# adobe-research/DiffusionHandles

Hardware: AMD Instinct MI355X
Metric: guided-denoise steps/sec at 512x512 (SD2-depth) (higher is better)
Workload: dtype f16; 1 GPU; single 512x512 edit per GPU, SD2-depth (865.9M params, seeded random weights), guided phase: 3 x (fwd + energy + bwd-to-latent) + CFG fwd (B=2) + DDIM step; resolution=512, edits_per_gpu=1, correspondences=24906, parallelism=independent edits, one process per GPU, no collectives

## Files before the change

### diffusionhandles_amd/_lib.py

```python
import ctypes
import os

import torch

_HERE = os.path.dirname(os.path.abspath(__file__))
LIB_PATH = os.environ.get("DIFFHANDLES_LIB") or os.path.join(_HERE, "libdiffhandles_hip.so")
_LIB = None

c_p = ctypes.c_void_p
c_i = ctypes.c_int
c_f = ctypes.c_float
c_d = ctypes.c_double
c_sz = ctypes.c_size_t


class UNetConfig(ctypes.Structure):
    _fields_ = [("in_channels", c_i), ("out_channels", c_i), ("n_levels", c_i),
                ("block_out_channels", c_i * 4), ("layers_per_block", c_i), ("heads", c_i * 4),
                ("cross_attention_dim", c_i), ("norm_groups", c_i), ("sample_size", c_i),
                ("text_len", c_i), ("max_batch", c_i), ("dtype", c_i), ("max_diff_batch", c_i)]


class VAEConfig(ctypes.Structure):
    _fields_ = [("latent_channels", c_i), ("out_channels", c_i), ("block_out_channels", c_i * 4),
# ... 40 lines not shown
    "dh_energy_fwd_bwd_planned": (c_i, [c_p, c_p, c_i, c_i, c_i, c_p, c_sz, c_i, c_p, c_i, c_p, c_i, c_f, c_f, c_f,
                                        c_p, c_p, c_i, c_p, c_sz, c_p]),
    "dh_energy_planned_batch_workspace_bytes": (c_i, [c_i, c_i, c_i, ctypes.POINTER(c_sz)]),
    "dh_energy_fwd_bwd_planned_batch": (c_i, [ctypes.POINTER(EnergyItem), c_i, c_i, c_i, c_i, c_i, c_p, c_sz, c_p]),
    "dh_energy_plan_objects_bytes": (c_i, [c_i, c_i, ctypes.POINTER(c_sz)]),
    "dh_energy_plan_build_objects": (c_i, [c_p, c_p, c_i, c_p, c_i, c_i, c_i, ctypes.POINTER(c_f), ctypes.POINTER(ctypes.c_int32),
                                           c_p, c_sz, c_p]),
    "dh_energy_fwd_bwd_planned_objects": (c_i, [c_p, c_p, c_i, c_i, c_i, c_p, c_sz, c_i, c_p, c_i, c_p, c_i, c_f, c_f, c_f,
                                                c_p, c_p, c_i, c_p, c_sz, c_p]),
    "dh_energy_planned_objects_batch_workspace_bytes": (c_i, [c_i, c_i, c_i, ctypes.POINTER(c_sz)]),
    "dh_energy_fwd_bwd_planned_objects_batch": (c_i, [ctypes.POINTER(EnergyItem), c_i, c_i, c_i, c_i, c_i, c_p, c_sz, c_p]),
    "dh_energy_fwd_bwd_planned_mixed_batch": (c_i, [ctypes.POINTER(EnergyItem), ctypes.POINTER(ctypes.c_uint8), c_i, c_i, c_i, c_i, c_i,
                                              c_p, c_sz, c_p]),
    "dh_unet_create": (c_i, [ctypes.POINTER(UNetConfig), ctypes.POINTER(c_p)]),
    "dh_unet_create_shared": (c_i, [c_p, c_i, c_p, ctypes.POINTER(c_p)]),
    "dh_unet_destroy": (None, [c_p]),
    "dh_unet_num_params": (c_i, [c_p]),
    "dh_unet_param_info": (c_i, [c_p, c_i, ctypes.POINTER(ctypes.c_char_p), ctypes.POINTER(c_i),
                                 ctypes.POINTER(ctypes.c_int64)]),
    "dh_unet_load_param": (c_i, [c_p, c_i, c_p, c_p]),
    "dh_unet_weight_bytes": (c_sz, [c_p]),
    "dh_unet_workspace_bytes": (c_sz, [c_p]),
    "dh_unet_forward": (c_i, [c_p, c_p, c_f, c_p, c_i, c_i, c_p, ctypes.POINTER(c_p), c_p]),
    "dh_unet_backward": (c_i, [c_p, ctypes.POINTER(c_p), c_p, c_p, c_p, c_p]),
    "dh_unet_set_text_key": (c_i, [c_p, ctypes.c_ulonglong]),
    "dh_unet_stats": (c_i, [c_p, ctypes.POINTER(c_d), ctypes.POINTER(c_d), ctypes.POINTER(ctypes.c_int64)]),
    "dh_vae_decoder_create": (c_i, [c_p, ctypes.POINTER(c_p)]),
    "dh_vae_decoder_destroy": (None, [c_p]),
    "dh_vae_decoder_num_params": (c_i, [c_p]),
    "dh_vae_decoder_param_info": (c_i, [c_p, c_i, ctypes.POINTER(ctypes.c_char_p), ctypes.POINTER(c_i),
                                        ctypes.POINTER(ctypes.c_int64)]),
    "dh_vae_decoder_load_param": (c_i, [c_p, c_i, c_p, c_p]),
    "dh_vae_decoder_bytes": (c_sz, [c_p]),
    "dh_vae_decoder_decode": (c_i, [c_p, c_p, c_i, c_p, c_p]),
    "dh_vae_encoder_create": (c_i, [c_p, ctypes.POINTER(c_p)]),
    "dh_vae_encoder_encode": (c_i, [c_p, c_p, c_i, c_p, c_p]),
    "dh_text_encoder_create": (c_i, [c_p, ctypes.POINTER(c_p)]),
    "dh_text_encoder_destroy": (None, [c_p]),
    "dh_text_encoder_num_params": (c_i, [c_p]),
    "dh_text_encoder_param_info": (c_i, [c_p, c_i, ctypes.POINTER(ctypes.c_char_p), ctypes.POINTER(c_i),
                                         ctypes.POINTER(ctypes.c_int64)]),
    "dh_text_encoder_load_param": (c_i, [c_p, c_i, c_p, c_p]),
    "dh_text_encoder_bytes": (c_sz, [c_p]),
    "dh_text_encoder_encode": (c_i, [c_p, c_p, c_i, c_i, c_p, c_p]),
    "dh_gemm_profile_begin": (c_i, []),
    "dh_gemm_profile_end": (c_i, [ctypes.POINTER(c_d), ctypes.POINTER(ctypes.c_int64), ctypes.POINTER(c_d)]),
    "dh_gemm_profile_bytes": (c_i, [ctypes.POINTER(c_d)]),
    "dh_ddim_cfg_step": (c_i, [c_p, c_p, c_p, c_p, c_f, c_f, c_f, c_i, c_p]),
    "dh_latent_update": (c_i, [c_p, c_p, c_p, c_f, c_f, c_i, c_p]),
    "dh_adam_step": (c_i, [c_p, c_p, c_p, c_p, c_f, c_f, c_f, c_f, c_i, c_i, c_p]),
    "dh_mse_fwd_bwd": (c_i, [c_p, c_p, c_i, c_p, c_p, c_p]),
    "dh_latent_update_strided": (c_i, [c_p, c_p, c_p, c_i, c_i, c_f, c_f, c_i, c_p]),
    "dh_pack_sample": (c_i, [c_p, c_p, c_i, c_i, c_p, c_i, c_i, c_i, c_i, c_p]),
    "dh_unet_io_ptr": (c_i, [c_p, c_i, c_i, ctypes.POINTER(c_p), ctypes.POINTER(c_sz)]),
    "dh_mse_cotangent": (c_i, [c_p, c_p, c_i, c_f, c_f, c_p, c_p, c_p, c_p]),
    "dh_adam_step_scaled": (c_i, [c_p, c_p, c_p, c_p, c_p, c_f, c_f, c_f, c_f, c_i, c_i, c_p]),
    "dh_mse_cotangent_batch": (c_i, [c_p, c_p, c_i, c_i, c_f, c_f, c_d, c_p, c_p, c_p, c_p, c_p, c_p]),
    "dh_adam_step_scaled_batch": (c_i, [c_p, c_p, c_p, c_p, c_p, c_p, c_f, c_f, c_f, c_f, c_i, c_i, c_i, c_p]),
    "dh_latent_update_guarded": (c_i, [c_p, c_p, c_p, c_i, c_i, c_f, c_i, c_i, c_p, c_i, c_i, c_p, c_p, c_i, c_i, c_p]),
    "dh_ddim_cfg_step_flagged": (c_i, [c_p, c_p, c_p, c_p, c_f, c_f, c_f, c_i, c_i, c_p, c_i, c_i, c_p]),
}

c_l = ctypes.c_long
DEBUG_SIGNATURES = {
    "dh_dbg_gemm": (c_i, [c_i, c_p, c_l, c_p, c_i, c_i, c_i, c_i, c_i, c_i, c_i, c_i, c_i, c_i, c_i, c_p, c_p, c_i, c_i,
                          c_p, c_l, c_p, c_l, c_i, c_p, c_sz, c_p]),
    "dh_dbg_gemm_groupnorm": (c_i, [c_i, c_p, c_l, c_p, c_i, c_i, c_i, c_i, c_i, c_i, c_i, c_p, c_p, c_p, c_sz, c_i, c_i, c_p, c_p, c_f, c_i,
                                    c_p, c_p, c_p, ctypes.POINTER(c_i), c_p]),
    "dh_dbg_gemm_groupnorm_bwd": (c_i, [c_i, c_p, c_l, c_p, c_i, c_i, c_i, c_i, c_i, c_i, c_i, c_p, c_p, c_sz, c_i, c_i, c_p, c_p, c_p, c_p, c_i,
                                        c_p, c_p, ctypes.POINTER(c_i), c_p]),
    "dh_dbg_gemm_groupnorm_res": (c_i, [c_i, c_p, c_l, c_p, c_i, c_i, c_i, c_i, c_i, c_i, c_i, c_p, c_p, c_l, c_p, c_p, c_sz, c_i, c_i, c_p, c_p,
                                    c_f, c_i, c_p, c_p, c_p, ctypes.POINTER(c_i), c_p]),
    "dh_dbg_gemm_groupnorm_bwd_res": (c_i, [c_i, c_p, c_l, c_p, c_i, c_i, c_i, c_i, c_i, c_i, c_i, c_p, c_l, c_p, c_p, c_sz, c_i, c_i, c_p, c_p, c_p,
                                        c_p, c_i, c_p, c_p, ctypes.POINTER(c_i), c_p]),
    "dh_dbg_concat_groupnorm": (c_i, [c_i, c_p, c_i, c_p, c_i, c_p, c_i, c_i, c_i, c_p, c_p, c_f, c_i, c_p, c_p, c_p, c_p]),
    "dh_dbg_gemm_last_tile": (c_i, [ctypes.POINTER(c_i)]),
    "dh_dbg_unet_concat_ops": (c_i, [ctypes.POINTER(UNetConfig), ctypes.POINTER(c_i), c_i, ctypes.POINTER(c_i)]),
    "dh_dbg_gemm_lnfold": (c_i, [c_i, c_p, c_l, c_p, c_i, c_i, c_i, c_p, c_p, c_p, c_f, c_p, c_l, c_p]),
    "dh_dbg_gemm_glu": (c_i, [c_i, c_i, c_p, c_l, c_p, c_i, c_i, c_i, c_p, c_p, c_p, c_p, c_p, c_p]),
    "dh_dbg_gemm_glub_split": (c_i, [c_i, c_p, c_l, c_p, c_i, c_i, c_i, c_i, c_p, c_l, c_i, c_p, c_p, ctypes.POINTER(c_i), c_p]),
    "dh_dbg_unet_ff_fold": (c_i, [c_p, c_i, ctypes.POINTER(c_i), ctypes.POINTER(c_i), c_p, c_p, c_p]),
    "dh_dbg_gemm_family": (c_i, [c_i]),
    "dh_dbg_gemm_stage": (c_i, [c_i]),
    "dh_dbg_gemm_pp_variant": (c_i, [c_i, c_p]),
    "dh_dbg_gemm_pp_ablate": (c_i, [c_i]),
    "dh_dbg_gemm_pp_persist": (c_i, [c_i]),
    "dh_dbg_gemm_pp_glu": (c_i, [c_i]),
    "dh_dbg_gemm_pp_plan": (c_i, [c_i, c_i, c_i, c_i, c_i, c_i, c_sz, ctypes.POINTER(c_i), ctypes.POINTER(c_i), ctypes.POINTER(c_i)]),
    "dh_dbg_touch_tiled": (c_i, [c_sz, c_p]),
    "dh_dbg_groupnorm": (c_i, [c_i, c_p, c_p, c_p, c_p, c_p, c_p, c_p, c_p, c_i, c_i, c_i, c_i, c_f, c_i, c_i, c_p]),
    "dh_dbg_layernorm": (c_i, [c_i, c_p, c_p, c_p, c_p, c_p, c_p, c_p, c_p, c_i, c_i, c_f, c_p]),
    "dh_dbg_geglu": (c_i, [c_i, c_p, c_p, c_p, c_p, c_i, c_i, c_p]),
    "dh_dbg_attention": (c_i, [c_i, c_p, c_l, c_p, c_p, c_l, c_p, c_l, c_p, c_p, c_p, c_p, c_p, c_p, c_i, c_i, c_i, c_i, c_p]),
    "dh_dbg_attention_bwd_pair": (c_i, [c_i, c_p, c_l, c_p, c_p, c_l, c_p, c_l, c_p, c_p, c_p, c_p, c_p, c_p, c_i, c_i, c_i, c_i, c_p, c_p]),
    "dh_dbg_pool2x2": (c_i, [c_i, c_p, c_p, c_i, c_i, c_i, c_i, c_i, c_p]),
    "dh_dbg_ellipse_offsets": (c_i, [c_i, ctypes.POINTER(ctypes.c_int32), c_i, ctypes.POINTER(c_i)]),
    "dh_dbg_lane_ops": (c_i, [c_p, c_p, c_p, c_p]),
}


def lib():
    global _LIB
    if _LIB is None:
        if not os.path.exists(LIB_PATH):
            raise RuntimeError(
                f"native HIP library not found at {LIB_PATH}; build it with "
                "`python -c 'import __graft_entry__ as g; g.build()'` (there is no CPU fallback)")
        handle = ctypes.CDLL(LIB_PATH)
        missing = []
        for name, (res, args) in list(SIGNATURES.items()) + list(DEBUG_SIGNATURES.items()):
            try:
                fn = getattr(handle, name)
            except AttributeError:
                missing.append(name)
                continue
            fn.restype = res
            fn.argtypes = args
        handle.dh_missing_symbols = missing
        for env, fn in (("DH_GEMM_FAMILY", "dh_dbg_gemm_family"), ("DH_PP_GLU", "dh_dbg_gemm_pp_glu"),
                        ("DH_PP_PERSIST", "dh_dbg_gemm_pp_persist"), ("DH_GEMM_STAGE", "dh_dbg_gemm_stage")):
            if os.environ.get(env) and fn not in missing:
                getattr(handle, fn)(int(os.environ[env]))
        _LIB = handle
    return _LIB


def check(rc, what=""):
    if rc != 0:
        raise RuntimeError(f"{what} failed ({rc}): {lib().dh_last_error().decode()}")


def require_gpu(t=None):
    if not torch.cuda.is_available():
        raise RuntimeError("diffusionhandles_amd needs a HIP device (MI355X); there is no CPU fallback")
    if t is not None and not t.is_cuda:
        raise RuntimeError("expected a device tensor")


def ptr(t):
    return c_p(t.data_ptr()) if t is not None else c_p(0)


def stream_ptr():
    return c_p(torch.cuda.current_stream().cuda_stream)


DTYPE_CODE = {torch.float16: 0, torch.bfloat16: 1, torch.float32: 2}
CODE_DTYPE = {v: k for k, v in DTYPE_CODE.items()}
```

### diffusionhandles_amd/csrc/attention.hip

```cpp
#include "unet_kernels.h"

namespace dh {

typedef _Float16 v8h __attribute__((ext_vector_type(8)));
typedef __bf16 v8b __attribute__((ext_vector_type(8)));
typedef float v16f __attribute__((ext_vector_type(16)));
typedef short v4s __attribute__((ext_vector_type(4)));

template <class T> struct Mma;
template <> struct Mma<f16> {
  static __device__ __forceinline__ v16f run(uint4 a, uint4 b, v16f c) {
    return __builtin_amdgcn_mfma_f32_32x32x16_f16(__builtin_bit_cast(v8h, a), __builtin_bit_cast(v8h, b), c, 0, 0, 0);
  }
};
template <> struct Mma<bf16> {
  static __device__ __forceinline__ v16f run(uint4 a, uint4 b, v16f c) {
    return __builtin_amdgcn_mfma_f32_32x32x16_bf16(__builtin_bit_cast(v8b, a), __builtin_bit_cast(v8b, b), c, 0, 0, 0);
  }
};

constexpr int HD = 64;
constexpr int TLD = 72;
constexpr int TILE = 64 * TLD;
constexpr float LOG2E = 1.4426950408889634f;
constexpr float LN2 = 0.6931471805599453f;
constexpr float SCALE = 0.125f;
constexpr float CEXP = SCALE * LOG2E;

__device__ __forceinline__ v16f zero16() {
  v16f z;
#pragma unroll
  for (int i = 0; i < 16; ++i) z[i] = 0.f;
  return z;
}
__device__ __forceinline__ float fast_exp2(float x) { return __builtin_amdgcn_exp2f(x); }
#ifndef DH_ATTN_ABL
#define DH_ATTN_ABL 0
#endif

template <class T>
__device__ __forceinline__ void load_row_frags(const T* base, long ld, long row, bool ok, int col0, int hi, uint4 (&f)[4]) {
#pragma unroll
  for (int kk = 0; kk < 4; ++kk)
    f[kk] = ok ? *reinterpret_cast<const uint4*>(base + row * ld + col0 + 16 * kk + 8 * hi) : make_uint4(0, 0, 0, 0);
}

typedef unsigned u4v __attribute__((ext_vector_type(4)));
template <int GT> struct TileRegs { u4v v[(512 + GT - 1) / GT]; };
template <class T, int GT>
__device__ __forceinline__ void fetch_tile(const T* base , long ld, long row0, long rows_total,
                                           TileRegs<GT>& t, int tid) {
#pragma unroll
  for (int j = 0; j < (512 + GT - 1) / GT; ++j) {
    int idx = tid + j * GT;
    idx = idx < 512 ? idx : 511;
    long r = row0 + (idx >> 3);
    r = r < rows_total ? r : rows_total - 1;
    const T* ptr = base + r * ld + (idx & 7) * 8;
    asm volatile("global_load_dwordx4 %0, %1, off" : "=&v"(t.v[j]) : "v"(ptr) : "memory");
  }
}
__device__ __forceinline__ void frags_ready(uint4 (&f)[4]) {
#pragma unroll
  for (int kk = 0; kk < 4; ++kk) asm volatile("" : "+v"(f[kk].x), "+v"(f[kk].y), "+v"(f[kk].z), "+v"(f[kk].w));
}
template <int GT>
__device__ __forceinline__ void tile_wait(TileRegs<GT>& a, TileRegs<GT>& b) {
  asm volatile("s_waitcnt vmcnt(0)" ::: "memory");
#pragma unroll
  for (int j = 0; j < (512 + GT - 1) / GT; ++j) { asm volatile("" : "+v"(a.v[j])); asm volatile("" : "+v"(b.v[j])); }
}
template <int GT>
__device__ __forceinline__ void commit_tile(const TileRegs<GT>& t, unsigned short* rm, int tid) {
#pragma unroll
  for (int j = 0; j < (512 + GT - 1) / GT; ++j) {
    const int idx = tid + j * GT;
    if (512 % GT == 0 || idx < 512) *reinterpret_cast<u4v*>(&rm[(idx >> 3) * TLD + (idx & 7) * 8]) = t.v[j];
  }
}

template <class T>
__device__ __forceinline__ v16f tile_times_frags(const unsigned short* tile, int rowbase, int ln, int hi, const uint4 (&f)[4]) {
  v16f acc = zero16();
#pragma unroll
  for (int kk = 0; kk < 4; ++kk) {
    const uint4 a = *reinterpret_cast<const uint4*>(&tile[(rowbase + ln) * TLD + 16 * kk + 8 * hi]);
    acc = Mma<T>::run(a, f[kk], acc);
  }
  return acc;
}

__device__ __forceinline__ uint4 tr_frag(const unsigned short* tptr, int cbase, int r0) {
  typedef __attribute__((address_space(3))) v4s* lp;
  const unsigned short* a = tptr + r0 * TLD + cbase;
  const v4s lo = __builtin_amdgcn_ds_read_tr16_b64_v4i16((lp)(a));
  const v4s up = __builtin_amdgcn_ds_read_tr16_b64_v4i16((lp)(a + 8 * TLD));
  const uint2 l2 = __builtin_bit_cast(uint2, lo), u2 = __builtin_bit_cast(uint2, up);
  return make_uint4(l2.x, l2.y, u2.x, u2.y);
}

constexpr int DTILE = 64 * 64;
__device__ uint4 g_attn_zero_page[8];
#ifdef DH_ATTN_STAMP
__device__ unsigned long long g_attn_ts_dkv[16];
#define DKV_STAMP(i) do { if (blockIdx.x == 0 && blockIdx.y == 0 && blockIdx.z == 0 && threadIdx.x == 0) g_attn_ts_dkv[i] = __builtin_amdgcn_s_memtime(); } while (0)
__device__ unsigned long long g_attn_ts[8];
#define ATTN_STAMP(i) do { if (blockIdx.x == 0 && blockIdx.y == 0 && blockIdx.z == 0 && threadIdx.x == 0) g_attn_ts[i] = __builtin_amdgcn_s_memtime(); } while (0)
#else
#define ATTN_STAMP(i) do { } while (0)
#define DKV_STAMP(i) do { } while (0)
#endif
#ifdef DH_ATTN_STAMP_DQ
#undef DKV_STAMP
#define DKV_STAMP(i) do { } while (0)
#define DQ_STAMP(i) do { if (blockIdx.x == 0 && blockIdx.y == 0 && blockIdx.z == 0 && threadIdx.x == 0) g_attn_ts_dkv[i] = __builtin_amdgcn_s_memtime(); } while (0)
#else
#define DQ_STAMP(i) do { } while (0)
#endif
__device__ __forceinline__ int dswz(int r) {
  const int y = r >> 1;
  return ((y & 1) << 2) | (y & 2) | ((y >> 2) & 1);
}
__device__ __forceinline__ void attn_dma16(const void* gsrc, unsigned lds_dst) {
  unsigned keep;
  asm volatile("s_mov_b32 %0, m0\n\ts_mov_b32 m0, %2\n\ts_nop 0\n\tglobal_load_lds_dwordx4 %1, off\n\ts_mov_b32 m0, %0"
               : "=&s"(keep) : "v"(gsrc), "s"(lds_dst) : "memory");
}
template <int QW> struct DmaPieces { unsigned voff[(16 + QW - 1) / QW]; };
template <int QW>
__device__ __forceinline__ void dma_pieces_init(DmaPieces<QW>& d, int wave_u, int lane, long ld_a, long ld_b) {
  const int d_row = lane >> 3;
  const int d_c0 = (lane & 7) ^ ((((lane >> 4) >> 1) & 1) << 1 | ((lane >> 4) & 1) << 2);
#pragma unroll
  for (int j = 0; j < (16 + QW - 1) / QW; ++j) {
    const int p = wave_u + j * QW, pp = p & 7;
    d.voff[j] = (unsigned)(((long)(8 * pp + d_row) * (p < 8 ? ld_a : ld_b) + ((d_c0 ^ (pp & 1)) << 3)) * 2);
  }
}
__device__ __forceinline__ void attn_dma16_s(const void* base, unsigned voff, unsigned lds) {
  const unsigned long long b64 = (unsigned long long)base;
  const unsigned long long sbase = (unsigned long long)(unsigned)__builtin_amdgcn_readfirstlane((int)(unsigned)b64) |
                                   ((unsigned long long)(unsigned)__builtin_amdgcn_readfirstlane((int)(unsigned)(b64 >> 32)) << 32);
  const unsigned lds_dst = (unsigned)__builtin_amdgcn_readfirstlane((int)lds);
  unsigned keep;
  asm volatile("s_mov_b32 %0, m0\n\ts_mov_b32 m0, %3\n\ts_nop 0\n\tglobal_load_lds_dwordx4 %2, %1\n\ts_mov_b32 m0, %0"
               : "=&s"(keep) : "s"(sbase), "v"(voff), "s"(lds_dst) : "memory");
}
template <int QW>
__device__ __forceinline__ void dma_tile_full(const DmaPieces<QW>& d, int wave_u, const void* base_a, const void* base_b,
                                              unsigned lds_tile) {
#pragma unroll
  for (int j = 0; j < (16 + QW - 1) / QW; ++j) {
    const int p = wave_u + j * QW;
    if (p < 16) attn_dma16_s(p < 8 ? base_a : base_b, d.voff[j], lds_tile + (unsigned)(p * 1024));
  }
}
template <class T>
__device__ __forceinline__ v16f dtile_times_frags(const unsigned short* tile, int rowbase, int ln, int xk, const uint4 (&f)[4]) {
  v16f acc = zero16();
#pragma unroll
  for (int kk = 0; kk < 4; ++kk) {
    const uint4 a = *reinterpret_cast<const uint4*>(&tile[(rowbase + ln) * 64 + ((xk ^ (2 * kk)) << 3)]);
    acc = Mma<T>::run(a, f[kk], acc);
  }
  return acc;
}
__device__ __forceinline__ uint4 dtr_frag(const unsigned short* trow, int lo_c, int up_c, int within, int dt, int r0) {
  typedef __attribute__((address_space(3))) v4s* lp;
  const unsigned short* a = trow + r0 * 64 + within;
  const v4s lo = __builtin_amdgcn_ds_read_tr16_b64_v4i16((lp)(a + ((lo_c ^ (4 * dt)) << 3)));
  const v4s up = __builtin_amdgcn_ds_read_tr16_b64_v4i16((lp)(a + 8 * 64 + ((up_c ^ (4 * dt)) << 3)));
  const uint2 l2 = __builtin_bit_cast(uint2, lo), u2 = __builtin_bit_cast(uint2, up);
  return make_uint4(l2.x, l2.y, u2.x, u2.y);
}

template <class T>
__device__ __forceinline__ uint4 pack8(const v16f& p, int s);
template <>
__device__ __forceinline__ uint4 pack8<f16>(const v16f& p, int s) {
  uint4 o;
  o.x = __builtin_bit_cast(unsigned, __builtin_amdgcn_cvt_pkrtz(p[8 * s + 0], p[8 * s + 1]));
  o.y = __builtin_bit_cast(unsigned, __builtin_amdgcn_cvt_pkrtz(p[8 * s + 2], p[8 * s + 3]));
  o.z = __builtin_bit_cast(unsigned, __builtin_amdgcn_cvt_pkrtz(p[8 * s + 4], p[8 * s + 5]));
  o.w = __builtin_bit_cast(unsigned, __builtin_amdgcn_cvt_pkrtz(p[8 * s + 6], p[8 * s + 7]));
  return o;
}
template <>
__device__ __forceinline__ uint4 pack8<bf16>(const v16f& p, int s) {
  bf16 o[8];
#pragma unroll
  for (int j = 0; j < 8; ++j) o[j] = (bf16)p[8 * s + j];
  return *reinterpret_cast<uint4*>(o);
}

template <class T>
__device__ __forceinline__ void store_rows_t(T* base, long ld, long row, int col0, int hi, const v16f (&acc)[2], float mul) {
#pragma unroll
  for (int dt = 0; dt < 2; ++dt) {
    uint2 w[4];
#pragma unroll
    for (int g = 0; g < 4; ++g) {
      T o[4];
#pragma unroll
      for (int i = 0; i < 4; ++i) o[i] = from_f32<T>(acc[dt][4 * g + i] * mul);
      w[g] = *reinterpret_cast<uint2*>(o);
    }
    const uint4 ca = half_exchange(w[0], w[1]), cb = half_exchange(w[2], w[3]);
    T* out = base + row * ld + col0 + dt * 32 + 8 * hi;
    *reinterpret_cast<uint4*>(out) = ca;
    *reinterpret_cast<uint4*>(out + 16) = cb;
  }
}

__device__ __forceinline__ int acc_row(int r, int hi) { return (r & 3) + 8 * (r >> 2) + 4 * hi; }

__device__ __forceinline__ void lds_barrier() {
  asm volatile("s_waitcnt lgkmcnt(0)" ::: "memory");
  __builtin_amdgcn_s_barrier();
  asm volatile("" ::: "memory");
}

template <class T, int KS, int QW, bool DB>
__global__ void __launch_bounds__(64 * QW * KS) k_attn_fwd(const T* q, long ldq, const T* k, const T* v, long ldk, T* o, long ldo,
                                                       float* lse, int H, int Nq, int Nk, int causal) {
  ATTN_STAMP(0);
  constexpr int NBUF = DB ? 2 : 1;
  constexpr int TSZ = DB ? DTILE : TILE;
  __shared__ __attribute__((aligned(1024))) unsigned short smem[KS * NBUF * 2 * TSZ];
  constexpr int GT = 64 * QW;
  const int ks = threadIdx.x / GT, tid = threadIdx.x - ks * GT;
  const int lane = tid & 63, wave = tid >> 6, ln = lane & 31, hi = lane >> 5, t16 = lane & 15;
  const int h = blockIdx.y, b = blockIdx.z;
  unsigned short* sK0 = smem + ks * NBUF * 2 * TSZ;
  const long qrow = (long)blockIdx.x * (32 * QW) + wave * 32 + ln;
  const bool qok = qrow < Nq;
  uint4 qf[4];
  load_row_frags<T>(q + (long)b * Nq * ldq, ldq, qrow, qok, h * HD, hi, qf);
  frags_ready(qf);
  v16f oacc[2] = {zero16(), zero16()};
  float m_run = -INFINITY, l_run = 0.f;
  const T* kp = k + (long)b * Nk * ldk + h * HD;
  const T* vp = v + (long)b * Nk * ldk + h * HD;
  const int vt_off = (4 * hi + (t16 >> 2)) * TLD + 16 * ((lane >> 4) & 1) + 4 * (t16 & 3);
  const int tiles = (Nk + 63) >> 6, tps = (tiles + KS - 1) / KS;
  const int t_begin = ks * tps, t_end = min(t_begin + tps, tiles);
  TileRegs<GT> rk, rv;
  const unsigned lds_grp = DB ? (unsigned)(size_t)((__attribute__((address_space(3))) unsigned char*)smem) + ks * NBUF * 2 * TSZ * 2 : 0u;
  const int d_row = lane >> 3;
  const int d_c0 = (lane & 7) ^ ((((lane >> 4) >> 1) & 1) << 1 | ((lane >> 4) & 1) << 2);
  const T* d_zero = reinterpret_cast<const T*>(g_attn_zero_page) + (lane & 7) * 8;
  const int wave_u = __builtin_amdgcn_readfirstlane(wave);
  DmaPieces<QW> dpc;
  if (DB) dma_pieces_init<QW>(dpc, wave_u, lane, ldk, ldk);
  auto dma_tile = [&](int key0, int buf) {
    if (key0 + 64 <= Nk) {
      dma_tile_full<QW>(dpc, wave_u, kp + (long)key0 * ldk, vp + (long)key0 * ldk, lds_grp + (unsigned)(buf * 2 * TSZ * 2));
      return;
    }
#pragma unroll
    for (int j = 0; j < (16 + QW - 1) / QW; ++j) {
      const int p = wave_u + j * QW;
      if (p < 16) {
        const int pp = p & 7;
        const long r = (long)key0 + 8 * pp + d_row;
        const T* src = (p < 8 ? kp : vp) + r * ldk + ((d_c0 ^ (pp & 1)) << 3);
        attn_dma16(r < Nk ? src : d_zero, __builtin_amdgcn_readfirstlane(lds_grp + (unsigned)(buf * 2 * TSZ * 2 + p * 1024)));
      }
    }
  };
  if (t_begin < t_end) {
    if (DB) {
      dma_tile(t_begin * 64, 0);
    } else {
      fetch_tile<T, GT>(kp, ldk, t_begin * 64, Nk, rk, tid);
      fetch_tile<T, GT>(vp, ldk, t_begin * 64, Nk, rv, tid);
    }
  }
  const int xk = hi ^ dswz(ln);
  const int d_rl = 4 * hi + (t16 >> 2), d_cl = 2 * ((lane >> 4) & 1) + ((t16 & 3) >> 1);
  const int d_lo = d_cl ^ dswz(d_rl), d_up = d_cl ^ dswz(d_rl + 8), d_within = 4 * (t16 & 1);
  ATTN_STAMP(1);
  for (int it = 0; it < tps; ++it) {
    if (it == 1) ATTN_STAMP(2);
    const int k0 = (t_begin + it) * 64;
    const bool act = t_begin + it < t_end;
    if (DB) {
      asm volatile("s_waitcnt vmcnt(0)" ::: "memory");
      __syncthreads();
    } else {
      lds_barrier();
    }
    if (DB && act && t_begin + it + 1 < t_end) dma_tile(k0 + 64, (it + 1) & 1);
    if (!DB) {
      if (act) {
        tile_wait<GT>(rk, rv);
        commit_tile<GT>(rk, sK0, tid);
        commit_tile<GT>(rv, sK0 + TILE, tid);
// ... 712 lines not shown
```

### diffusionhandles_amd/csrc/debug_api.cpp

```cpp
#include <stdlib.h>

#include "unet_kernels.h"
using namespace dh;

static void* g_dbg_tiled = nullptr;

__global__ void k_dbg_touch(const uint4* p, size_t n16, unsigned* sink) {
  unsigned acc = 0;
  for (size_t i = (size_t)blockIdx.x * blockDim.x + threadIdx.x; i < n16; i += (size_t)gridDim.x * blockDim.x) { const uint4 v = p[i]; acc ^= v.x ^ v.y ^ v.z ^ v.w; }
  if (acc == 0x9e3779b9u && sink) sink[0] = acc;
}
extern "C" int dh_dbg_touch_tiled(size_t bytes, void* stream) {
  DH_REQUIRE(g_dbg_tiled != nullptr, "no tiled weights yet (call dh_dbg_gemm first)");
  hipLaunchKernelGGL(k_dbg_touch, dim3(512), dim3(256), 0, (hipStream_t)stream, (const uint4*)g_dbg_tiled, bytes / 16, (unsigned*)nullptr);
  DH_LAUNCH_CHECK();
  return DH_OK;
}

extern "C" int dh_dbg_gemm(int dtype, const void* A, long lda, const void* W, int M, int N, int K, int mode, int Hin,
                           int Win, int Cin, int Hout, int Wout, int stride, int up, const float* bias,
                           const float* rowvec, int rowvec_ld, int rows_per_batch, const void* R, long ldr, void* C,
                           long ldc, int act_silu, float* partial, size_t partial_elems, void* stream) {
  DH_REQUIRE(A && W && C && K % 64 == 0 && N % 64 == 0, "bad arguments (N, K must be multiples of 64)");
  void*& tiled = g_dbg_tiled;
// ... 32 lines not shown
    cap = need;
  }
  launch_tile_weights(dtype, W, tiled, N, K, (hipStream_t)stream, mode != 0 ? Cin : 0);
  GemmArgs g;
  g.A = A; g.lda = lda; g.W = tiled; g.M = M; g.N = N; g.K = K; g.mode = mode; g.Hin = Hin; g.Win = Win; g.Cin = Cin;
  g.Hout = Hin; g.Wout = Win; g.stride = 1; g.up = 0; g.bias = bias; g.R = R; g.ldr = ldr; g.C = C; g.ldc = N;
  g.partial = partial; g.partial_elems = partial_elems;
  int have = 0;
  g.gn_part = scratch; g.gn_HW = HW; g.gn_G = G; g.gn_done = &have;
  launch_gemm(dtype, g, (hipStream_t)stream);
  launch_groupnorm_fwd(dtype, C, gamma, beta, Y, stats, scratch, M / HW, HW, N, G, eps, silu, (hipStream_t)stream, have);
  if (have_out) *have_out = have;
  DH_LAUNCH_CHECK();
  return DH_OK;
}
extern "C" int dh_dbg_gemm_groupnorm(int dtype, const void* A, long lda, const void* W, int M, int N, int K, int mode, int Hin, int Win,
                                     int Cin, const float* bias, void* C, float* partial, size_t partial_elems, int HW, int G,
                                     const float* gamma, const float* beta, float eps, int silu, void* Y, float* stats, float* scratch,
                                     int* have_out, void* stream) {
  return dh_dbg_gemm_groupnorm_res(dtype, A, lda, W, M, N, K, mode, Hin, Win, Cin, bias, nullptr, N, C, partial, partial_elems, HW, G,
                                   gamma, beta, eps, silu, Y, stats, scratch, have_out, stream);
}
extern "C" int dh_dbg_gemm_groupnorm_bwd_res(int dtype, const void* A, long lda, const void* W, int M, int N, int K, int mode, int Hin,
                                         int Win, int Cin, const void* R, long ldr, void* C, float* partial, size_t partial_elems, int HW, int G, const void* x,
                                         const float* gamma, const float* beta, const float* stats, int silu, void* dx,
                                         float* scratch, int* have_out, void* stream) {
  DH_REQUIRE(A && W && C && x && dx && stats && scratch && gamma && beta && K % 64 == 0 && N % 64 == 0 && HW > 0 && M % HW == 0, "bad arguments");
  static void* tiled = nullptr;
  static size_t cap = 0;
  const size_t need = (size_t)N * K * 2;
  if (need > cap) {
    if (tiled) (void)hipFree(tiled);
    DH_CHECK_HIP(hipMalloc(&tiled, need));
    cap = need;
  }
  launch_tile_weights(dtype, W, tiled, N, K, (hipStream_t)stream, mode != 0 ? Cin : 0);
  GemmArgs g;
  g.A = A; g.lda = lda; g.W = tiled; g.M = M; g.N = N; g.K = K; g.mode = mode; g.Hin = Hin; g.Win = Win; g.Cin = Cin;
  g.Hout = Hin; g.Wout = Win; g.stride = 1; g.up = 0; g.R = R; g.ldr = ldr; g.C = C; g.ldc = N;
  g.partial = partial; g.partial_elems = partial_elems;
  int have = 0;
  g.gnb_x = x; g.gnb_ldx = N; g.gnb_gamma = gamma; g.gnb_beta = beta; g.gnb_stats = stats; g.gnb_silu = silu;
  g.gn_part = scratch; g.gn_HW = HW; g.gn_G = G; g.gn_done = &have;
  launch_gemm(dtype, g, (hipStream_t)stream);
  launch_groupnorm_bwd(dtype, x, C, gamma, beta, stats, dx, scratch, M / HW, HW, N, G, silu, 0, (hipStream_t)stream, have, GnBwdSplit());
  if (have_out) *have_out = have;
  DH_LAUNCH_CHECK();
  return DH_OK;
}
extern "C" int dh_dbg_gemm_groupnorm_bwd(int dtype, const void* A, long lda, const void* W, int M, int N, int K, int mode, int Hin,
                                         int Win, int Cin, void* C, float* partial, size_t partial_elems, int HW, int G, const void* x,
                                         const float* gamma, const float* beta, const float* stats, int silu, void* dx,
                                         float* scratch, int* have_out, void* stream) {
  return dh_dbg_gemm_groupnorm_bwd_res(dtype, A, lda, W, M, N, K, mode, Hin, Win, Cin, nullptr, N, C, partial, partial_elems, HW, G, x,
                                       gamma, beta, stats, silu, dx, scratch, have_out, stream);
}
extern "C" int dh_dbg_concat_groupnorm(int dtype, const void* a, int Ca, const void* b, int Cb, void* out, int B, int HW, int G,
                                       const float* gamma, const float* beta, float eps, int silu, void* Y, float* stats,
                                       float* scratch, void* stream) {
  DH_REQUIRE(a && b && out && Y && stats && scratch && gamma && beta && B > 0 && HW > 0 && G > 0, "bad arguments");
  DH_REQUIRE(Ca % 8 == 0 && Cb % 8 == 0 && (Ca + Cb) % G == 0 && (GN_GB * ((Ca + Cb) / G)) % 8 == 0 && GN_GB * ((Ca + Cb) / G) <= 2048,
             "shape the fused concatenation does not take");
  launch_concat_gn(dtype, a, Ca, b, Cb, out, scratch, B, HW, G, (hipStream_t)stream);
  launch_groupnorm_fwd(dtype, out, gamma, beta, Y, stats, scratch, B, HW, Ca + Cb, G, eps, silu, (hipStream_t)stream, 1);
  DH_LAUNCH_CHECK();
  return DH_OK;
}
extern "C" int dh_dbg_gemm_lnfold(int dtype, const void* A, long lda, const void* W, int M, int N, int K, const float* ln_s,
                                  const float* ln_t, float* ln_stats, float ln_eps, void* C, long ldc, void* stream) {
  DH_REQUIRE(A && W && C && ln_s && ln_t && ln_stats && K % 64 == 0 && N % 64 == 0, "bad arguments (N, K must be multiples of 64)");
  static void* tiled = nullptr;
  static size_t tiled_cap = 0;
  const size_t need = (size_t)N * K * 2;
  if (need > tiled_cap) {
    if (tiled) (void)hipFree(tiled);
    DH_CHECK_HIP(hipMalloc(&tiled, need));
    tiled_cap = need;
  }
  launch_tile_weights(dtype, W, tiled, N, K, (hipStream_t)stream);
  GemmArgs g;
  g.A = A; g.lda = lda; g.W = tiled; g.M = M; g.N = N; g.K = K; g.mode = A_DENSE; g.C = C; g.ldc = ldc;
  g.ln_s = ln_s; g.ln_t = ln_t; g.ln_stats = ln_stats; g.ln_eps = ln_eps;
  launch_gemm(dtype, g, (hipStream_t)stream);
  DH_LAUNCH_CHECK();
  return DH_OK;
}
extern "C" int dh_dbg_gemm_glu(int dtype, int bwd, const void* A, long lda, const void* W, int M, int N, int K, const float* bias,
                               void* C, void* y, const void* x, void* dx, void* stream) {
  DH_REQUIRE(A && W && K % 64 == 0 && N % 128 == 0, "bad arguments (K % 64, N % 128)");
  DH_REQUIRE(bwd ? (x && dx) : (y != nullptr), "missing output");
  static void* tiled = nullptr;
  static size_t tiled_cap = 0;
  const size_t need = (size_t)N * K * 2;
  if (need > tiled_cap) {
    if (tiled) (void)hipFree(tiled);
    DH_CHECK_HIP(hipMalloc(&tiled, need));
    tiled_cap = need;
  }
  launch_tile_weights(dtype, W, tiled, N, K, (hipStream_t)stream);
  GemmArgs g;
  g.A = A; g.lda = lda; g.W = tiled; g.M = M; g.N = N; g.K = K; g.mode = A_DENSE; g.bias = bias;
  if (bwd) { g.glub_x = x; g.glub_dx = dx; }
  else { g.C = C; g.ldc = N; g.glu_y = y; g.glu_ldy = N / 2; }
  launch_gemm(dtype, g, (hipStream_t)stream);
  DH_LAUNCH_CHECK();
  return DH_OK;
}
extern "C" int dh_dbg_gemm_last_tile(int* out);
extern "C" int dh_dbg_gemm_glub_split(int dtype, const void* A, long lda, const void* W, int M, int N, int K, int F, void* C,
                                      long ldc, int accumulate, const void* x, void* dx, int* tile, void* stream) {
  DH_REQUIRE(A && W && C && x && dx && K % 64 == 0 && N % 64 == 0 && F % 64 == 0 && F > 0 && F < N, "bad arguments (K, N, F % 64; 0 < F < N)");
  static void* tiled = nullptr;
  static size_t tiled_cap = 0;
  const int Np = (int)align_up((size_t)N, 128);
  const size_t need = (size_t)Np * K * 2;
  if (need > tiled_cap) {
    if (tiled) (void)hipFree(tiled);
    DH_CHECK_HIP(hipMalloc(&tiled, need));
    tiled_cap = need;
  }
  DH_CHECK_HIP(hipMemsetAsync(tiled, 0, need, (hipStream_t)stream));
  launch_tile_weights(dtype, W, tiled, N, K, (hipStream_t)stream);
  GemmArgs g;
  g.A = A; g.lda = lda; g.W = tiled; g.M = M; g.N = N; g.K = K; g.mode = A_DENSE;
  g.glub_x = x; g.glub_dx = dx; g.glub_f = F;
  g.C = C; g.ldc = ldc;
  if (accumulate) { g.R = C; g.ldr = ldc; }
  launch_gemm(dtype, g, (hipStream_t)stream);
  if (tile) dh_dbg_gemm_last_tile(tile);
  DH_LAUNCH_CHECK();
  return DH_OK;
}
extern "C" int dh_dbg_groupnorm(int dtype, const void* x, const float* gamma, const float* beta, void* y, float* stats,
                                const void* dy, void* dx, float* scratch, int B, int HW, int C, int G, float eps,
                                int silu, int accumulate, void* stream) {
  launch_groupnorm_fwd(dtype, x, gamma, beta, y, stats, scratch, B, HW, C, G, eps, silu, (hipStream_t)stream);
  if (dy && dx)
    launch_groupnorm_bwd(dtype, x, dy, gamma, beta, stats, dx, scratch, B, HW, C, G, silu, accumulate, (hipStream_t)stream);
  DH_LAUNCH_CHECK();
  return DH_OK;
}
extern "C" int dh_dbg_layernorm(int dtype, const void* x, const float* gamma, const float* beta, void* y, float* stats,
                                const void* dy, const void* add, void* dx, int rows, int C, float eps, void* stream) {
  launch_layernorm_fwd(dtype, x, gamma, beta, y, stats, rows, C, eps, (hipStream_t)stream);
  if (dy && dx) launch_layernorm_bwd(dtype, x, dy, gamma, stats, add, dx, rows, C, (hipStream_t)stream);
  DH_LAUNCH_CHECK();
  return DH_OK;
}
extern "C" int dh_dbg_geglu(int dtype, const void* x, void* y, const void* dy, void* dx, int rows, int F, void* stream) {
  launch_geglu_fwd(dtype, x, y, rows, F, (hipStream_t)stream);
  if (dy && dx) launch_geglu_bwd(dtype, x, dy, dx, rows, F, (hipStream_t)stream);
  DH_LAUNCH_CHECK();
  return DH_OK;
}
extern "C" int dh_dbg_attention(int dtype, const void* q, long ldq, const void* k, const void* v, long ldk, void* o,
                                long ldo, float* lse, const void* d_o, float* delta, void* dq, void* dk, void* dv,
                                int B, int H, int Nq, int Nk, void* stream) {
  hipStream_t st = (hipStream_t)stream;
  launch_attention_fwd(dtype, q, ldq, k, v, ldk, o, ldo, lse, B, H, Nq, Nk, st);
  if (d_o) {
    if (dq) launch_attention_bwd_dq(dtype, q, ldq, k, v, ldk, o, ldo, d_o, ldo, lse, delta, dq, ldq, B, H, Nq, Nk, st);
    else launch_attention_delta(dtype, o, ldo, d_o, ldo, delta, B, H, Nq, st);
    if (dk && dv) {
      static float* scratch = nullptr;
      constexpr size_t kScratch = (size_t)16 << 20;
      if (!scratch && hipMalloc((void**)&scratch, kScratch * sizeof(float)) != hipSuccess) scratch = nullptr;
// ... 39 lines not shown
```

### diffusionhandles_amd/csrc/gemm.hip

```cpp
#include <stdlib.h>

#include <vector>

#include <hip/hip_ext.h>

#include "gemm_k.h"

namespace dh {

struct GemmProf {
  bool on = false;
  std::vector<hipEvent_t> ev;
  size_t used = 0;
  double flops = 0;
  double bytes = 0;
  hipEvent_t e0 = nullptr, e1 = nullptr;
};
static GemmProf g_prof;
static int g_buf_stage = 1;
static int g_pp_force = 0;
struct GemmTileReport {
  int bm, bn, kg, stages, mw, splits, pp, gn_epi, reduce_gn;
};
static thread_local GemmTileReport g_last_tile;
#ifdef DH_TUNING
static unsigned long long* g_gemm_ts = nullptr;
#endif
bool gemm_profiling_on() { return g_prof.on; }

constexpr int BK = 64;
#ifdef DH_EXP_SETPRIO
#define DH_PRIO(x) __builtin_amdgcn_s_setprio(x)
#else
#define DH_PRIO(x) do { } while (0)
#endif


template <class T>
__device__ __forceinline__ uint2 epilogue_pack(const GemmK& p, int m, int n, float v0, float v1, float v2, float v3,
                                               bool have_r, uint2 rpre, bool have_b, float4 bpre) {
  float v[4] = {v0, v1, v2, v3};
  if (p.bias) {
    float4 b = bpre;
    if (!have_b) b = *reinterpret_cast<const float4*>(p.bias + n);
    v[0] += b.x; v[1] += b.y; v[2] += b.z; v[3] += b.w;
  }
  if (p.rowvec) {
    const float4 b = *reinterpret_cast<const float4*>(p.rowvec + (size_t)div_small(m, p.inv_rows_per_batch) * p.rowvec_ld + n);
    v[0] += b.x; v[1] += b.y; v[2] += b.z; v[3] += b.w;
  }
  if (p.act_silu) {
#pragma unroll
    for (int i = 0; i < 4; ++i) v[i] = v[i] / (1.f + __expf(-v[i]));
  }
  typedef T T4 __attribute__((ext_vector_type(4)));
  if (p.R) {
    const T* r = reinterpret_cast<const T*>(p.R) + (size_t)m * p.ldr + n;
    uint2 raw = rpre;
    if (!have_r) raw = *reinterpret_cast<const uint2*>(r);
    const T4 rv = __builtin_bit_cast(T4, raw);
#pragma unroll
    for (int i = 0; i < 4; ++i) v[i] += to_f32<T>(rv[i]);
  }
  T4 o;
#pragma unroll
  for (int i = 0; i < 4; ++i) o[i] = from_f32<T>(v[i]);
  return __builtin_bit_cast(uint2, o);
}
template <class T>
__device__ __forceinline__ void epilogue_store(const GemmK& p, int m, int n, float v0, float v1, float v2, float v3,
                                               bool have_r = false, uint2 rpre = make_uint2(0, 0), bool have_b = false,
                                               float4 bpre = make_float4(0.f, 0.f, 0.f, 0.f)) {
  *reinterpret_cast<uint2*>(reinterpret_cast<T*>(p.C) + (size_t)m * p.ldc + n) =
      epilogue_pack<T>(p, m, n, v0, v1, v2, v3, have_r, rpre, have_b, bpre);
}

template <class T>
__device__ __forceinline__ float epilogue_scalar(const GemmK& p, int m, int n, float v) {
  if (p.bias) v += p.bias[n];
  if (p.rowvec) v += p.rowvec[(size_t)div_small(m, p.inv_rows_per_batch) * p.rowvec_ld + n];
  if (p.act_silu) v = v / (1.f + __expf(-v));
  if (p.R) v += to_f32<T>(reinterpret_cast<const T*>(p.R)[(size_t)m * p.ldr + n]);
  return to_f32<T>(from_f32<T>(v));
}

__device__ uint4 g_zero_page[8];

__device__ __forceinline__ void dma16(const void* gsrc, unsigned lds_dst) {
  unsigned keep;
  asm volatile("s_mov_b32 %0, m0\n\ts_mov_b32 m0, %2\n\ts_nop 0\n\tglobal_load_lds_dwordx4 %1, off\n\ts_mov_b32 m0, %0"
               : "=&s"(keep) : "v"(gsrc), "s"(lds_dst) : "memory");
}

__device__ __forceinline__ void dma16_nt(const void* gsrc, unsigned lds_dst) {
  unsigned keep;
  asm volatile("s_mov_b32 %0, m0\n\ts_mov_b32 m0, %2\n\ts_nop 0\n\tglobal_load_lds_dwordx4 %1, off nt\n\ts_mov_b32 m0, %0"
               : "=&s"(keep) : "v"(gsrc), "s"(lds_dst) : "memory");
}

typedef int buf_v4i __attribute__((ext_vector_type(4)));
__device__ __forceinline__ void buf_dma16(unsigned voff, buf_v4i rsrc, unsigned soff, unsigned lds_dst) {
  unsigned tmp;
  soff = __builtin_amdgcn_readfirstlane(soff);
  lds_dst = __builtin_amdgcn_readfirstlane(lds_dst);
  asm volatile("s_mov_b32 m0, %4\n\ts_mov_b32 %0, %3\n\tbuffer_load_dwordx4 %1, %2, %0 offen lds"
               : "=&s"(tmp) : "v"(voff), "s"(rsrc), "s"(soff), "s"(lds_dst) : "memory");
}
// ... 235 lines not shown
      bs_sh = 31u - (unsigned)tap;
      return;
    }
    if (MODE != GM_DENSE) { if (++tap == 9) { tap = 0; c0 += BK; } }
  };
  auto issue = [&](int kt, int stage) {
#pragma unroll
    for (int q = 0; q < NP; ++q) issue_piece(kt, stage, q);
    next_tile();
  };

  v16f acc[TM][TN];
#pragma unroll
  for (int i = 0; i < TM; ++i)
#pragma unroll
    for (int j = 0; j < TN; ++j)
#pragma unroll
      for (int r = 0; r < 16; ++r) acc[i][j][r] = 0.f;

  const int wn_u = __builtin_amdgcn_readfirstlane(wn);
  float ln1[TM], ln2[TM];
#pragma unroll
  for (int i = 0; i < TM; ++i) { ln1[i] = 0.f; ln2[i] = 0.f; }

#pragma unroll
  for (int s = 0; s < ST - 1; ++s)
    if (s < ntiles) issue(s, s);
  DH_STAMP(1);

  constexpr bool PRE = TM * TN <= 8;
  const bool pre_r = PRE && p.R != nullptr && p.pre_r && p.splits == 1 && (WG == 1 || grp == 0) && (KG == 1 || kg == 0) &&
                     (GLU != 2 || !glub_tile_is_glu(n0, p.glub_f));
  constexpr bool PRE_B = PRE && !(MW == 2 && BN == 320) && WNS == 2;
  const bool pre_b = PRE_B && p.bias != nullptr && p.pre_r && p.splits == 1;
  float4 bpre[PRE_B ? TN : 1][4];
  if (pre_b) {
#pragma unroll
    for (int j = 0; j < TN; ++j)
#pragma unroll
      for (int g = 0; g < 4; ++g) {
        const int n = n0 + wn * CPW + j * 32 + 8 * g + 4 * hi;
        bpre[PRE_B ? j : 0][g] = n < p.N ? *reinterpret_cast<const float4*>(p.bias + n) : make_float4(0.f, 0.f, 0.f, 0.f);
      }
  }
  constexpr bool PRE_LN = LNF && PRE && !(MW == 2 && BM == 256);
  float4 lsp[PRE_LN ? TN : 1][4], ltp[PRE_LN ? TN : 1][4];
  if (PRE_LN) {
#pragma unroll
    for (int j = 0; j < TN; ++j)
#pragma unroll
      for (int g = 0; g < 4; ++g) {
        const int n = n0 + wn * CPW + j * 32 + 8 * g + 4 * hi;
        lsp[PRE_LN ? j : 0][g] = n < p.N ? *reinterpret_cast<const float4*>(p.ln_s + n) : make_float4(0.f, 0.f, 0.f, 0.f);
        ltp[PRE_LN ? j : 0][g] = n < p.N ? *reinterpret_cast<const float4*>(p.ln_t + n) : make_float4(0.f, 0.f, 0.f, 0.f);
      }
  }
  constexpr bool GNB = gn_epi_bwd_tile(BM, BN, WG, GLU, LNF);
  static_assert(!GNB || (PRE && WNS == 2), "the backward form carries the GroupNorm input tile in the residual's prefetch registers");
  const bool gnb = GNB && p.gn_epi == 2 && p.splits == 1;
  const bool pre_x = gnb && (KG == 1 || kg == 0);
  float4 gnb_col = make_float4(0.f, 0.f, 0.f, 0.f);
  if (GNB && pre_x && tid < BN) {
    const int n = n0 + tid, grp_n = (int)(((float)n + 0.5f) / (float)p.gn_cpg);
    const float2 st2 = *reinterpret_cast<const float2*>(p.gnb_stats + 2 * ((m0 / p.gn_HW) * p.gn_G + grp_n));
    gnb_col = make_float4(p.gnb_gamma[n], p.gnb_beta[n], st2.x, st2.y);
  }
  uint2 rpre[TM][TN][4];
  if (pre_r || pre_x) {
    const T* rsrc = reinterpret_cast<const T*>(pre_x ? p.gnb_x : p.R);
    const long rld = pre_x ? p.gnb_ldx : p.ldr;
#pragma unroll
    for (int i = 0; i < TM; ++i) {
      const int m = m0 + wm * RPW + i * 32 + ln;
#pragma unroll
      for (int j = 0; j < TN; ++j)
#pragma unroll
        for (int g = 0; g < 4; ++g) {
          const int n = n0 + wn * CPW + j * 32 + 8 * g + 4 * hi;
          rpre[i][j][g] = (m < p.M && n < p.N) ? *reinterpret_cast<const uint2*>(rsrc + (size_t)m * rld + n) : make_uint2(0, 0);
        }
    }
  }

  constexpr int KK = BK / 16 / WG;
  const int kk0 = grp * KK;
  unsigned fa_off[BK / 16], fb_off[BK / 16];
#pragma unroll
  for (int kk = 0; kk < BK / 16; ++kk) {
    const unsigned pc = (unsigned)(((2 * kk + hi) ^ ((ln >> 1) & 7)) << 4);
    fa_off[kk] = (unsigned)((wm * RPW + ln) * 128) + pc;
    fb_off[kk] = (unsigned)(BM * 128 + (wn * CPW + ln) * 128) + pc;
  }
  int stg = 0;
  DH_STAMP(2);
  for (int kt = 0; kt < loop_tiles; ++kt) {
    DH_STAMP_T(kt, 0);
    if (ntiles - 1 - kt >= ST - 2) wait_vmcnt<NP * (ST - 2)>(); else wait_vmcnt<0>();
    __builtin_amdgcn_s_barrier();
    DH_STAMP_T(kt, 1);
    if (kt == 0) DH_STAMP(3);
    if (KG > 1 && kt >= ntiles) continue;
    const bool more = ABL != 2 && kt + ST - 1 < ntiles;
    const int cur = __builtin_amdgcn_readfirstlane(stg);
    const int nkt = kt + ST - 1, nstage = cur == 0 ? ST - 1 : cur - 1;
    stg = cur + 1 == ST ? 0 : cur + 1;
    if (ABL == 1) { if (more) issue(nkt, nstage); continue; }
    const unsigned char* st_base = smem + cur * STAGE;
    uint4 fw[2][TN], fx[2][TM];
    auto load_frags = [&](int kk, int buf) {
      const unsigned char* pb = st_base + fb_off[kk];
      const unsigned char* pa = st_base + fa_off[kk];
#pragma unroll
      for (int j = 0; j < TN; ++j) fw[buf][j] = *reinterpret_cast<const uint4*>(pb + j * (32 * 128));
#pragma unroll
      for (int i = 0; i < TM; ++i) fx[buf][i] = *reinterpret_cast<const uint4*>(pa + i * (32 * 128));
    };
    load_frags(kk0, 0);
#pragma unroll
    for (int kk = 0; kk < KK; ++kk) {
      if (kk + 1 < KK) load_frags(kk0 + kk + 1, (kk + 1) & 1);
      DH_PRIO(1);
#pragma unroll
      for (int i = 0; i < TM; ++i)
#pragma unroll
        for (int j = 0; j < TN; ++j) acc[i][j] = Mfma<T>::run(fw[kk & 1][j], fx[kk & 1][i], acc[i][j]);
      DH_PRIO(0);
      if (LNF && (kk & 1) == wn_u LNF_ABL(1)) {
#pragma unroll
        for (int i = 0; i < TM; ++i) frag_sums<T>(fx[kk & 1][i], ln1[i], ln2[i]);
      }
      if (more) {
        constexpr int EK = ST == 2 ? 2 : KK;
        if (kk < EK) {
#pragma unroll
          for (int q = kk * NP / EK; q < (kk + 1) * NP / EK; ++q) issue_piece(nkt, nstage, q);
        }
      }
    }
    if (more) next_tile();
    DH_STAMP_T(kt, 2);
  }
  DH_STAMP(4);

  if (LNF LNF_ABL(2)) {
    float* xb = reinterpret_cast<float*>(smem_all);
    const int wid = tid >> 6;
    __syncthreads();
#pragma unroll
    for (int i = 0; i < TM; ++i) { xb[(wid * 2 * TM + 2 * i) * 64 + lane] = ln1[i]; xb[(wid * 2 * TM + 2 * i + 1) * 64 + lane] = ln2[i]; }
    __syncthreads();
#pragma unroll
    for (int i = 0; i < TM; ++i) {
      ln1[i] += xb[((wid ^ 1) * 2 * TM + 2 * i) * 64 + lane];
      ln2[i] += xb[((wid ^ 1) * 2 * TM + 2 * i + 1) * 64 + lane];
    }
  }

  if (WG > 1 || KG > 1) {
    constexpr int NG = WG * KG;
    constexpr int SLOT = (TM * TN * 16 + (LNF ? 2 * TM : 0)) * 64;
    static_assert((NG - 1) * 4 * SLOT * 4 <= KG * ST * STAGE, "merge buffer does not fit the stage rings");
    const int g = WG > 1 ? grp : kg;
    float* cb = reinterpret_cast<float*>(smem_all);
    __syncthreads();
    if (g > 0) {
      float* slot = cb + ((g - 1) * 4 + wave) * SLOT + lane;
#pragma unroll
      for (int i = 0; i < TM; ++i)
#pragma unroll
        for (int j = 0; j < TN; ++j)
#pragma unroll
          for (int r = 0; r < 16; ++r) slot[((i * TN + j) * 16 + r) * 64] = acc[i][j][r];
      if (LNF) {
#pragma unroll
        for (int i = 0; i < TM; ++i) { slot[(TM * TN * 16 + 2 * i) * 64] = ln1[i]; slot[(TM * TN * 16 + 2 * i + 1) * 64] = ln2[i]; }
      }
    }
    __syncthreads();
    if (g > 0) return;
#pragma unroll
    for (int og = 1; og < NG; ++og) {
      const float* slot = cb + ((og - 1) * 4 + wave) * SLOT + lane;
#pragma unroll
      for (int i = 0; i < TM; ++i)
#pragma unroll
        for (int j = 0; j < TN; ++j)
#pragma unroll
          for (int r = 0; r < 16; ++r) acc[i][j][r] += slot[((i * TN + j) * 16 + r) * 64];
      if (LNF) {
#pragma unroll
        for (int i = 0; i < TM; ++i) { ln1[i] += slot[(TM * TN * 16 + 2 * i) * 64]; ln2[i] += slot[(TM * TN * 16 + 2 * i + 1) * 64]; }
      }
    }
  }

  if (LNF LNF_ABL(4)) {
    const float inv_k = 1.f / (float)p.K;
#pragma unroll
    for (int i = 0; i < TM; ++i) {
      const float a = xor32_sum(ln1[i]), q = xor32_sum(ln2[i]);
      const float mean = a * inv_k;
      float var = q * inv_k - mean * mean;
      var = var > 0.f ? var : 0.f;
      const float rstd = rsqrtf(var + p.ln_eps);
      const int m = m0 + wm * RPW + i * 32 + ln;
      if (blockIdx.y == 0 && wn == 0 && hi == 0 && m < p.M) { p.ln_stats[2 * (size_t)m] = mean; p.ln_stats[2 * (size_t)m + 1] = rstd; }
#pragma unroll
      for (int j = 0; j < TN; ++j)
#pragma unroll
        for (int g = 0; g < 4; ++g) {
          const int n = n0 + wn * CPW + j * 32 + 8 * g + 4 * hi;
          if (n >= p.N) continue;
          float4 sv, tv;
          if (PRE_LN) { sv = lsp[PRE_LN ? j : 0][g]; tv = ltp[PRE_LN ? j : 0][g]; }
          else { sv = *reinterpret_cast<const float4*>(p.ln_s + n); tv = *reinterpret_cast<const float4*>(p.ln_t + n); }
          acc[i][j][4 * g] = rstd * (acc[i][j][4 * g] - mean * sv.x) + tv.x;
          acc[i][j][4 * g + 1] = rstd * (acc[i][j][4 * g + 1] - mean * sv.y) + tv.y;
          acc[i][j][4 * g + 2] = rstd * (acc[i][j][4 * g + 2] - mean * sv.z) + tv.z;
          acc[i][j][4 * g + 3] = rstd * (acc[i][j][4 * g + 3] - mean * sv.w) + tv.w;
        }
    }
  }


  if constexpr (GLU == 1) {
    typedef T T4 __attribute__((ext_vector_type(4)));
    const bool hb = p.bias != nullptr;
    T* Y = reinterpret_cast<T*>(p.glu_y);
#pragma unroll
    for (int i = 0; i < TM; ++i) {
      const int m = m0 + wm * RPW + i * 32 + ln;
      if (m >= p.M) continue;
#pragma unroll
      for (int j = 0; j < TN; ++j) {
        const int nb = n0 + wn * CPW + j * 32;
        if (nb >= p.N) continue;
        uint2 w[4];
        float pv[4][4];
#pragma unroll
        for (int g = 0; g < 4; ++g) {
          float v0 = acc[i][j][4 * g], v1 = acc[i][j][4 * g + 1], v2 = acc[i][j][4 * g + 2], v3 = acc[i][j][4 * g + 3];
          if (hb) {
            float4 b = bpre[PRE_B ? j : 0][g];
            if (!pre_b) b = *reinterpret_cast<const float4*>(p.bias + nb + 8 * g + 4 * hi);
            v0 += b.x; v1 += b.y; v2 += b.z; v3 += b.w;
          }
          T4 o;
          o[0] = from_f32<T>(v0); o[1] = from_f32<T>(v1); o[2] = from_f32<T>(v2); o[3] = from_f32<T>(v3);
          w[g] = __builtin_bit_cast(uint2, o);
#pragma unroll
          for (int c = 0; c < 4; ++c) pv[g][c] = to_f32<T>(o[c]);
        }
        if (p.C) {
          T* out = reinterpret_cast<T*>(p.C) + (size_t)m * p.ldc + nb + 8 * hi;
          *reinterpret_cast<uint4*>(out) = half_exchange(w[0], w[1]);
          *reinterpret_cast<uint4*>(out + 16) = half_exchange(w[2], w[3]);
        }
        uint2 y[2];
#pragma unroll
        for (int q = 0; q < 2; ++q) {
          T4 o;
#pragma unroll
          for (int c = 0; c < 4; ++c) o[c] = from_f32<T>(pv[q][c] * gelu_f(pv[q + 2][c]));
          y[q] = __builtin_bit_cast(uint2, o);
        }
        *reinterpret_cast<uint4*>(Y + (size_t)m * p.glu_ldy + (nb >> 1) + 8 * hi) = half_exchange(y[0], y[1]);
      }
    }
    return;
  }
  if (GLU == 2 && glub_tile_is_glu(n0, p.glub_f)) {
    typedef T T4 __attribute__((ext_vector_type(4)));
    const T* X = reinterpret_cast<const T*>(p.glub_x);
    T* DX = reinterpret_cast<T*>(p.glub_dx);
    const size_t ldx = 2 * (size_t)p.glub_f;
    uint4 Hc[TM][TN][2], Gc[TM][TN][2];
#pragma unroll
    for (int i = 0; i < TM; ++i) {
      const int m = m0 + wm * RPW + i * 32 + ln;
      const int mc = m < p.M ? m : p.M - 1;
#pragma unroll
      for (int j = 0; j < TN; ++j) {
        int nb = n0 + wn * CPW + j * 32;
        if (nb >= p.glub_f) nb = 0;
#pragma unroll
        for (int q = 0; q < 2; ++q) {
          const T* src = X + (size_t)mc * ldx + 2 * nb + 32 * q + 8 * hi;
          Hc[i][j][q] = *reinterpret_cast<const uint4*>(src);
          Gc[i][j][q] = *reinterpret_cast<const uint4*>(src + 16);
        }
      }
    }
#pragma unroll
    for (int i = 0; i < TM; ++i) {
      const int m = m0 + wm * RPW + i * 32 + ln;
      if (m >= p.M) continue;
#pragma unroll
      for (int j = 0; j < TN; ++j) {
        const int nb = n0 + wn * CPW + j * 32;
        if (nb >= p.glub_f) continue;
#pragma unroll
        for (int q = 0; q < 2; ++q) {
          const uint4 hc = Hc[i][j][q], gc = Gc[i][j][q];
          const uint4 hx = half_exchange(make_uint2(hc.x, hc.y), make_uint2(hc.z, hc.w));
          const uint4 gx = half_exchange(make_uint2(gc.x, gc.y), make_uint2(gc.z, gc.w));
          uint2 dh[2], dg[2];
// ... 381 lines not shown
      const uint4 rawx = *reinterpret_cast<const uint4*>(reinterpret_cast<const T*>(p.gnb_x) + (size_t)m * p.gnb_ldx + n);
      const T* xv = reinterpret_cast<const T*>(&rawx);
#pragma unroll
      for (int i = 0; i < 8; ++i) {
        o[i] = from_f32<T>(v[i]);
        const float xh = (to_f32<T>(xv[i]) - mu[i]) * rs[i];
        float d = to_f32<T>(o[i]);
        if (p.gnb_silu) d *= silu_grad(xh * gm[i] + bt[i]);
        d *= gm[i];
        av[i] += d; qv[i] += d * xh;
      }
    }
    *reinterpret_cast<uint4*>(reinterpret_cast<T*>(p.C) + (size_t)m * p.ldc + n) = *reinterpret_cast<uint4*>(o);
  };
  auto acc = [&](const float* f) {
#pragma unroll
    for (int i = 0; i < 8; ++i) { const float d = f[i] - pv[i]; av[i] += d; qv[i] += d * d; }
  };
  float f[8];
  if (BWD) {
    if (live)
      for (int r = r0 + rr; r < r1; r += RP) row(r, f);
  } else {
    const bool first = live && r0 + rr < r1;
    if (first) row(r0 + rr, f);
    if (first && rr == 0) {
#pragma unroll
      for (int i = 0; i < 8; ++i)
        if (ch * 8 + i == gi[i] * cpg) sm_piv[gi[i]] = f[i];
    }
    __syncthreads();
#pragma unroll
    for (int i = 0; i < 8; ++i) pv[i] = g0 + gi[i] < G ? sm_piv[gi[i]] : 0.f;
    if (first) {
      acc(f);
      for (int r = r0 + rr + RP; r < r1; r += RP) { row(r, f); acc(f); }
    }
  }
  if (live) {
#pragma unroll
    for (int i = 0; i < 8; ++i)
#pragma unroll
      for (int gl = 0; gl < GN_GB; ++gl) {
        ga[gl] += gi[i] == gl ? av[i] : 0.f;
        gq[gl] += gi[i] == gl ? qv[i] : 0.f;
      }
  }
#pragma unroll
  for (int gl = 0; gl < GN_GB; ++gl) { ga[gl] = wave_sum(ga[gl]); gq[gl] = wave_sum(gq[gl]); }
  if ((threadIdx.x & 63) == 0) {
#pragma unroll
    for (int gl = 0; gl < GN_GB; ++gl) { sm_red[threadIdx.x >> 6][2 * gl] = ga[gl]; sm_red[threadIdx.x >> 6][2 * gl + 1] = gq[gl]; }
  }
  __syncthreads();
  if ((int)threadIdx.x < GN_GB && g0 + (int)threadIdx.x < G) {
    const int gl = threadIdx.x, g = g0 + gl;
    float sa = 0.f, sq = 0.f;
    for (int w = 0; w < 4; ++w) { sa += sm_red[w][2 * gl]; sq += sm_red[w][2 * gl + 1]; }
    if (BWD) {
      p.gn_part[((size_t)(b * G + g) * S + s) * 2] = sa;
      p.gn_part[((size_t)(b * G + g) * S + s) * 2 + 1] = sq;
    } else {
      const float cnt = (float)(r1 - r0) * (float)cpg;
      float* o = p.gn_part + ((size_t)(b * G + g) * 3) * S + s;
      o[0] = cnt; o[S] = sm_piv[gl] + sa / cnt; o[2 * S] = sq - sa * sa / cnt;
    }
  }
}

#define DH_GEMM_LAUNCH(KERNEL)                                                                              \
  do {                                                                                                      \
    if (g_prof.e0) hipExtLaunchKernelGGL(KERNEL, grid, dim3(TH), 0, st, g_prof.e0, g_prof.e1, 0, k);        \
    else hipLaunchKernelGGL(KERNEL, grid, dim3(TH), 0, st, k);                                              \
  } while (0)
template <class T, int BM, int BN, int ST, int WG, int KG, int MW, bool BUF>
static void launch_tile_b(int gm, bool lnf, dim3 grid, hipStream_t st, const GemmK& k, int glu) {
  constexpr int TH = 256 * WG * KG * MW;
  constexpr bool GLUOK = WG == 1 && KG == 1 && ((BM == 256 && BN == 128 && MW == 2) || (BM == 128 && BN == 128 && MW == 2 && ST == 4) || (BM == 64 && BN == 64));
  if constexpr (GLUOK) {
    if (glu == 1 && lnf) { DH_GEMM_LAUNCH((k_gemm_dma<T, BM, BN, ST, GM_DENSE, 0, WG, KG, MW, true, 1, BUF>)); return; }
    if (glu == 1) { DH_GEMM_LAUNCH((k_gemm_dma<T, BM, BN, ST, GM_DENSE, 0, WG, KG, MW, false, 1, BUF>)); return; }
    if (glu == 2) { DH_GEMM_LAUNCH((k_gemm_dma<T, BM, BN, ST, GM_DENSE, 0, WG, KG, MW, false, 2, BUF>)); return; }
  }
  if (gm == GM_DENSE) {
    if constexpr (WG == 1 && BN != 320 && BN != 160) {
      if (lnf) { DH_GEMM_LAUNCH((k_gemm_dma<T, BM, BN, ST, GM_DENSE, 0, WG, KG, MW, true, 0, BUF>)); return; }
    }
    DH_GEMM_LAUNCH((k_gemm_dma<T, BM, BN, ST, GM_DENSE, 0, WG, KG, MW, false, 0, BUF>));
  } else if (gm == GM_CONV_S1) {
    DH_GEMM_LAUNCH((k_gemm_dma<T, BM, BN, ST, GM_CONV_S1, 0, WG, KG, MW, false, 0, BUF>));
  } else {
    DH_GEMM_LAUNCH((k_gemm_dma<T, BM, BN, ST, GM_GENERIC, 0, WG, KG, MW>));
  }
}
template <class T, int BM, int BN, int ST, int WG, int KG, int MW>
static void launch_tile(int gm, bool lnf, dim3 grid, hipStream_t st, const GemmK& k, int glu = 0) {
  g_last_tile.bm = BM; g_last_tile.bn = BN; g_last_tile.kg = KG; g_last_tile.stages = ST; g_last_tile.mw = MW;
  if (k.pp_a_bytes != 0 && gm != GM_GENERIC) launch_tile_b<T, BM, BN, ST, WG, KG, MW, true>(gm, lnf, grid, st, k, glu);
  else launch_tile_b<T, BM, BN, ST, WG, KG, MW, false>(gm, lnf, grid, st, k, glu);
}
#undef DH_GEMM_LAUNCH

#ifdef DH_TUNING
#define DH_KNOB(name, env, dflt) static const int name = getenv(env) ? atoi(getenv(env)) : (dflt)
#else
#define DH_KNOB(name, env, dflt) constexpr int name = (dflt)
#endif

template <class T>
static void gemm_dispatch(GemmK k, size_t partial_elems, hipStream_t st, int* gn_done, int* lnb_done, int dtype) {
  DH_KNOB(kSplitTiles, "DH_SPLITK_TILES", 200);
  DH_KNOB(kSplitMinK, "DH_SPLITK_MINKT", 32);
  DH_KNOB(kSplitTarget, "DH_SPLITK_TARGET", 256);
  DH_KNOB(kBigTiles, "DH_BIG_TILES", 128);
  DH_KNOB(kNarrowTiles, "DH_NARROW_TILES", 40);
  DH_KNOB(kN320, "DH_GEMM_N320", 224);
  DH_KNOB(kMwBlocks, "DH_GEMM_MW", 64);
  DH_KNOB(kKg2MinKt, "DH_KG2_MINKT", 4);
  DH_KNOB(kManyBlocks, "DH_GEMM_MANY", 512);
  DH_KNOB(kMw128, "DH_GEMM_MW128", 1);
  DH_KNOB(kTwoPerCu, "DH_GEMM_TWO_PER_CU", 1);
#ifdef DH_TUNING
  DH_KNOB(kWnt, "DH_W_NT", 0);
#endif
  const bool lnf = k.ln_s != nullptr;
  g_last_tile = GemmTileReport{};
  int BM = 128, BN = (k.N % 128 == 0) ? 128 : 64;
  const int ktiles = k.K / BK;
  PpPlan pp;
  const bool use_pp = gemm_pp_plan(k, partial_elems, g_pp_force, &pp);
  if (BN == 128 && ktiles >= 16 && cdiv(k.M, 128) * cdiv(k.N, 128) <= kNarrowTiles) BN = 64;
  if (k.M <= 64 || (cdiv(k.M, 128) * cdiv(k.N, BN) < kBigTiles && ktiles < kSplitMinK)) { BM = 64; BN = 64; }
  const bool n320 = kN320 > 0 && k.N % 320 == 0 && k.N <= 960 && !lnf && BM == 128 && BN == 64 && cdiv(k.M, 128) >= kN320;
  if (n320) BN = 320;
  DH_KNOB(kMwShortK, "DH_GEMM_MW_SHORTK", 128);
  const long tiles256 = (long)cdiv(k.M, 256) * cdiv(k.N, 128);
  const bool mw2 = kMwBlocks > 0 && k.N % 128 == 0 && tiles256 >= kMwBlocks &&
                   !(k.M <= 256 && k.M > 128 && cdiv(k.N, 128) < 128) && (tiles256 >= kMwShortK || ktiles >= kSplitMinK);
  if (mw2) { BM = 256; BN = 128; }
  const int glu = k.glu_y ? 1 : (k.glub_x ? 2 : 0);
  if (glu && !(BM == 64 && BN == 64)) { BM = mw2 ? 256 : 128; BN = 128; }
  if (glu == 2 && !glub_split_ok(BN, k.glub_f)) { BM = 64; BN = 64; }
  DH_KNOB(kT160, "DH_GEMM_T160", 224);
  const long tiles160 = (long)cdiv(k.M, 128) * (k.N / 160);
  const bool t160 = kT160 > 0 && k.N % 160 == 0 && !lnf && !glu && !n320 && BM != 64 && tiles160 >= kT160 && tiles160 <= 256;
  if (t160) { BM = 128; BN = 160; }
  if (use_pp) { BM = pp.bm; BN = pp.bn; }
  const int tm = cdiv(k.M, BM), tn = cdiv(k.N, BN), tiles = tm * tn;
  int splits = 1;
  if (use_pp) splits = pp.splits;
  else if (k.partial && !lnf && !glu && tiles < kSplitTiles && ktiles >= kSplitMinK) {
    splits = kSplitTarget / tiles;
    if (splits > ktiles / 4) splits = ktiles / 4;
    if (splits > 32) splits = 32;
    const size_t fit = partial_elems / ((size_t)k.M * k.N);
    if ((size_t)splits > fit) splits = (int)fit;
    if (splits < 1) splits = 1;
  }
#ifdef DH_TUNING
  static const int kLog = getenv("DH_GEMM_LOG") ? atoi(getenv("DH_GEMM_LOG")) : 0;
  const int kForceTile = getenv("DH_FORCE_TILE") ? atoi(getenv("DH_FORCE_TILE")) : 0;
  const int kForceSplits = getenv("DH_FORCE_SPLITS") ? atoi(getenv("DH_FORCE_SPLITS")) : 0;
  int force_tile = 0;
  if (kForceTile && !use_pp && !(k.glu_y || k.glub_x)) {
    const int fbm = kForceTile == 1 ? 64 : (kForceTile == 6 ? 256 : 128), fbn = kForceTile == 7 ? 160 : ((kForceTile <= 3) ? 64 : 128);
    if ((k.N % fbn == 0 || fbn == 64) && !(fbn == 160 && lnf)) { BM = fbm; BN = fbn; force_tile = kForceTile; }
  }
  if (kForceSplits && !use_pp && k.partial && !lnf) {
    splits = kForceSplits;
    if (splits > ktiles / 2) splits = ktiles / 2 > 0 ? ktiles / 2 : 1;
    const size_t fit = partial_elems / ((size_t)k.M * k.N);
    if ((size_t)splits > fit) splits = (int)fit;
    if (splits < 1) splits = 1;
  }
  if (kLog) fprintf(stderr, "GEMMLOG M=%d N=%d K=%d mode=%d lnf=%d gn=%d gnb=%d bias=%d R=%d rowvec=%d | pp=%d BM=%d BN=%d splits=%d\n", k.M, k.N, k.K,
                    k.mode == A_DENSE ? 0 : (k.mode == A_CONV3 && k.stride == 1 && k.up == 0 ? 1 : 2), (int)lnf, k.gn_part != nullptr,
                    k.gnb_x != nullptr, k.bias != nullptr, k.R != nullptr, k.rowvec != nullptr, (int)use_pp, BM, BN, splits);
#endif
  const int tiles_per_split = cdiv(ktiles, splits);
  splits = cdiv(ktiles, tiles_per_split);
  k.splits = splits;
  k.k_per_split = tiles_per_split * BK;
  k.gn_epi = 0; k.gn_cpg = 0;
  if ((g_buf_stage & 4) == 0 && splits == 1 && !use_pp && gn_epi_fwd_tile(BN, glu, lnf) && k.gn_part && !k.gnb_x && gn_done && k.gn_G > 0 &&
      k.gn_HW > 0 && k.C && k.wide_store && k.M % k.gn_HW == 0 && k.gn_HW % BM == 0 && k.N % k.gn_G == 0 && k.N % BN == 0) {
    const int cpg = k.N / k.gn_G, sx = 2 * (k.gn_HW / BM);
    if (cpg >= 8 && cpg <= BN && sx <= 64) { k.gn_epi = 1; k.gn_cpg = cpg; k.gn_S = sx; }
  }
  if ((g_buf_stage & 8) == 0 && splits == 1 && !use_pp && gn_epi_bwd_tile(BM, BN, 1, glu, lnf) && k.gn_part && k.gnb_x && gn_done && k.gn_G > 0 &&
      k.gn_HW > 0 && k.C && k.wide_store && k.pre_r && !k.R && !k.bias && !k.rowvec && !k.act_silu && k.M % k.gn_HW == 0 && k.gn_HW % BM == 0 &&
      k.N % k.gn_G == 0 && k.N % BN == 0 && (((size_t)k.gnb_x | (size_t)(k.gnb_ldx * 2)) & 7) == 0) {
    const int cpg = k.N / k.gn_G, sx = 2 * (k.gn_HW / BM);
    if (cpg >= 8 && cpg <= BN && sx <= 64) { k.gn_epi = 2; k.gn_cpg = cpg; k.gn_S = sx; }
  }
#ifdef DH_TUNING
  k.w_nt = kWnt > 0 && tm <= kWnt;
  static const int kLnfAbl = getenv("DH_LNF_ABL") ? atoi(getenv("DH_LNF_ABL")) : 0;
  k.lnf_abl = kLnfAbl;
  k.ts = g_gemm_ts;
#endif
#ifdef DH_TUNING
  dim3 grid(force_tile ? cdiv(k.M, BM) : tm, force_tile ? cdiv(k.N, BN) : tn, splits);
#else
  dim3 grid(tm, tn, splits);
#endif
  hipEvent_t e0 = nullptr, e1 = nullptr;
  if (g_prof.on) {
    if (g_prof.used + 2 > g_prof.ev.size()) {
      const size_t old = g_prof.ev.size();
      g_prof.ev.resize(old + 4096);
      for (size_t i = old; i < g_prof.ev.size(); ++i) (void)hipEventCreate(&g_prof.ev[i]);
    }
    e0 = g_prof.ev[g_prof.used++];
    e1 = g_prof.ev[g_prof.used++];
    g_prof.flops += 2.0 * (double)k.M * (double)k.N * (double)k.K;
    const double esz = 2.0;
    double a_elems = (double)k.M * k.K;
    if (k.mode != A_DENSE && k.Hout > 0 && k.Wout > 0) a_elems = (double)k.M / ((double)k.Hout * k.Wout) * k.Hin * k.Win * k.Cin;
    double c_elems = (double)k.M * k.N * (k.C ? 1.0 : 0.0) + (k.R ? (double)k.M * k.N : 0.0);
    if (k.glu_y) c_elems += 0.5 * (double)k.M * k.N;
    if (k.glub_x) c_elems += 4.0 * (double)k.M * k.glub_f - (k.C ? (double)k.M * k.glub_f : 0.0);
    if (k.gn_epi == 2) c_elems += (double)k.M * k.N;
    g_prof.bytes += esz * (a_elems + (double)k.N * k.K + c_elems);
    g_prof.e0 = e0; g_prof.e1 = e1;
  }
  int gm = GM_GENERIC;
  if (k.mode == A_DENSE) gm = GM_DENSE;
  else if (k.mode == A_CONV3 && k.stride == 1 && k.up == 0 && k.pad == 1) gm = GM_CONV_S1;
  if (!use_pp) {
    k.pp_a_bytes = 0; k.pp_w_bytes = 0;
    size_t ab = 0;
    if (k.mode == A_DENSE) ab = ((size_t)(k.M - 1) * k.lda + k.K) * 2;
    else if (k.Hout > 0 && k.Wout > 0 && k.M % (k.Hout * k.Wout) == 0)
      ab = (size_t)(k.M / (k.Hout * k.Wout)) * k.Hin * k.Win * (size_t)k.lda * 2;
    const size_t wb = (size_t)align_up((size_t)k.N, 64) * k.K * 2;
    const bool conv_ok = k.mode == A_DENSE || (k.Cin % 64 == 0 && k.K == 9 * k.Cin);
    if ((g_buf_stage & 1) && ab > 0 && conv_ok && ab + (size_t)(k.Win + 1) * k.lda * 2 < 0x7ff00000ull && wb < 0x7ff00000ull && k.lda % 8 == 0 &&
        ((size_t)k.A & 15) == 0 && ((size_t)k.W & 15) == 0) {
      k.pp_a_bytes = (unsigned)ab; k.pp_w_bytes = (unsigned)wb;
    }
  }
#ifdef DH_TUNING
  static const int kAbl = getenv("DH_GEMM_ABLATE") ? atoi(getenv("DH_GEMM_ABLATE")) : 0;
  if (kAbl == 1 && BM == 128 && BN == 128) { hipLaunchKernelGGL((k_gemm_dma<T, 128, 128, 4, GM_CONV_S1, 1>), grid, dim3(256), 0, st, k); }
  else if (kAbl == 2 && BM == 128 && BN == 128) { hipLaunchKernelGGL((k_gemm_dma<T, 128, 128, 4, GM_CONV_S1, 2>), grid, dim3(256), 0, st, k); }
  else if (kAbl == 3 && BM == 128 && BN == 128) { hipLaunchKernelGGL((k_gemm_dma<T, 128, 128, 4, GM_DENSE, 1>), grid, dim3(256), 0, st, k); }
  else if (kAbl == 1 && mw2 && gm == GM_CONV_S1) { hipLaunchKernelGGL((k_gemm_dma<T, 256, 128, 3, GM_CONV_S1, 1, 1, 1, 2>), grid, dim3(512), 0, st, k); }
  else if (kAbl == 2 && mw2 && gm == GM_CONV_S1) { hipLaunchKernelGGL((k_gemm_dma<T, 256, 128, 3, GM_CONV_S1, 2, 1, 1, 2>), grid, dim3(512), 0, st, k); }
  else if (kAbl == 1 && mw2 && gm == GM_DENSE && !lnf) { hipLaunchKernelGGL((k_gemm_dma<T, 256, 128, 3, GM_DENSE, 1, 1, 1, 2>), grid, dim3(512), 0, st, k); }
  else if (kAbl == 2 && mw2 && gm == GM_DENSE && !lnf) { hipLaunchKernelGGL((k_gemm_dma<T, 256, 128, 3, GM_DENSE, 2, 1, 1, 2>), grid, dim3(512), 0, st, k); }
  else if (force_tile == 1) launch_tile<T, 64, 64, 4, 1, 1, 1>(gm, lnf, grid, st, k);
  else if (force_tile == 2) launch_tile<T, 128, 64, 3, 1, 2, 1>(gm, lnf, grid, st, k);
  else if (force_tile == 3) launch_tile<T, 128, 64, 5, 1, 1, 1>(gm, lnf, grid, st, k);
  else if (force_tile == 4) launch_tile<T, 128, 128, 4, 1, 1, 2>(gm, lnf, grid, st, k);
  else if (force_tile == 5) launch_tile<T, 128, 128, 4, 1, 1, 1>(gm, lnf, grid, st, k);
  else if (force_tile == 6) launch_tile<T, 256, 128, 3, 1, 1, 2>(gm, lnf, grid, st, k);
  else if (force_tile == 7) launch_tile<T, 128, 160, 4, 1, 1, 1>(gm, false, grid, st, k);
  else
#endif
  if (use_pp) { pp.splits = splits; g_last_tile.bm = pp.bm; g_last_tile.bn = pp.bn; launch_gemm_pp(dtype, k, pp, st, g_prof.e0, g_prof.e1); }
  else if (t160) launch_tile<T, 128, 160, 4, 1, 1, 1>(gm, false, grid, st, k);
  else if (mw2) launch_tile<T, 256, 128, 3, 1, 1, 2>(gm, lnf, grid, st, k, glu);
  else if (BM == 128 && BN == 128 && (glu || (kMw128 && tiles_per_split >= kMw128))) launch_tile<T, 128, 128, 4, 1, 1, 2>(gm, lnf, grid, st, k, glu);
  else if (kTwoPerCu && BM == 128 && BN == 64 && tiles * splits > 256 && tiles * splits <= 512)
    launch_tile<T, 128, 64, 3, 1, 1, 1>(gm, lnf, grid, st, k);
  else if (BM == 128 && BN == 64 && tiles_per_split >= kKg2MinKt) launch_tile<T, 128, 64, 3, 1, 2, 1>(gm, lnf, grid, st, k);
  else if (BN == 320) launch_tile<T, 128, 320, 2, 1, 1, 2>(gm, false, grid, st, k);
  else if (BM == 64) launch_tile<T, 64, 64, 4, 1, 1, 1>(gm, lnf, grid, st, k, glu);
  else if (BN == 128 && kManyBlocks > 0 && tiles * splits >= kManyBlocks) launch_tile<T, 128, 128, 2, 1, 1, 1>(gm, lnf, grid, st, k);
  else if (BN == 128) launch_tile<T, 128, 128, 4, 1, 1, 1>(gm, lnf, grid, st, k);
  else launch_tile<T, 128, 64, 5, 1, 1, 1>(gm, lnf, grid, st, k);
  g_prof.e0 = g_prof.e1 = nullptr;
  g_last_tile.splits = splits; g_last_tile.pp = use_pp ? 1 : 0; g_last_tile.gn_epi = k.gn_epi;
  if (k.gn_epi) *gn_done = k.gn_S;
  if (splits > 1) {
    if (k.gn_part && k.gn_G > 0 && k.gn_HW > 0 && k.N % k.gn_G == 0 && (GN_GB * (k.N / k.gn_G)) % 8 == 0 &&
        GN_GB * (k.N / k.gn_G) <= 2048 && k.M % k.gn_HW == 0) {
      k.gn_S = gn_slices(k.gn_HW, k.M / k.gn_HW);
      if (k.gnb_x) hipLaunchKernelGGL((k_splitk_reduce_gn<T, true>), dim3(k.gn_S, cdiv(k.gn_G, GN_GB), k.M / k.gn_HW), dim3(256), 0, st, k);
      else hipLaunchKernelGGL((k_splitk_reduce_gn<T, false>), dim3(k.gn_S, cdiv(k.gn_G, GN_GB), k.M / k.gn_HW), dim3(256), 0, st, k);
      g_last_tile.reduce_gn = 1;
      if (gn_done) *gn_done = 1;
    } else if (k.lnb_x && lnb_done && !k.bias && !k.rowvec && !k.R && !k.act_silu && k.N % 8 == 0 && k.ldc == k.N) {
      launch_splitk_reduce_ln_bwd(dtype, k.partial, splits, k.lnb_x, k.lnb_gamma, k.lnb_stats, k.lnb_add, k.lnb_dx, k.M, k.N, st, k.lnb_ldx);
      *lnb_done = 1;
    } else {
      const size_t groups = (size_t)k.M * k.N / 4;
      hipLaunchKernelGGL((k_splitk_reduce<T>), dim3((unsigned)((groups + 255) / 256)), dim3(256), 0, st, k);
    }
  }
}
#undef DH_KNOB

double launch_gemm(int dtype, const GemmArgs& a, hipStream_t st) {
  GemmK k;
  k.A = a.A; k.lda = a.lda; k.W = a.W; k.M = a.M; k.N = a.N; k.K = a.K;
  k.mode = a.mode; k.Hin = a.Hin; k.Win = a.Win; k.Cin = a.Cin; k.Hout = a.Hout; k.Wout = a.Wout;
  k.stride = a.stride; k.up = a.up; k.pad = a.pad;
  k.bias = a.bias; k.rowvec = a.rowvec; k.rowvec_ld = a.rowvec_ld;
  k.rows_per_batch = a.rows_per_batch > 0 ? a.rows_per_batch : 1;
  k.inv_rows_per_batch = 1.f / (float)k.rows_per_batch;
  k.R = a.R; k.ldr = a.ldr; k.C = a.C; k.ldc = a.ldc; k.act_silu = a.act_silu;
  k.partial = a.partial; k.splits = 1; k.k_per_split = a.K;
  k.pre_r = 1;
  k.wide_store = a.N % 32 == 0 && a.ldc % 8 == 0 && ((size_t)a.C & 15) == 0;
  k.ln_s = a.ln_s; k.ln_t = a.ln_t; k.ln_stats = a.ln_stats; k.ln_eps = a.ln_eps;
  k.gn_part = a.gn_part; k.gn_HW = a.gn_HW; k.gn_G = a.gn_G; k.gn_S = 0;
  k.gnb_x = a.gnb_x; k.gnb_ldx = a.gnb_ldx; k.gnb_gamma = a.gnb_gamma; k.gnb_beta = a.gnb_beta; k.gnb_stats = a.gnb_stats;
  k.gnb_silu = a.gnb_silu;
  k.lnb_x = a.lnb_x; k.lnb_ldx = a.lnb_ldx > 0 ? a.lnb_ldx : a.N;
  k.lnb_gamma = a.lnb_gamma; k.lnb_stats = a.lnb_stats; k.lnb_add = a.lnb_add; k.lnb_dx = a.lnb_dx;
  k.glu_y = a.glu_y; k.glu_ldy = a.glu_ldy; k.glub_x = a.glub_x; k.glub_dx = a.glub_dx;
  k.glub_f = a.glub_x && a.glub_f > 0 && a.glub_f < a.N ? a.glub_f : a.N;
  if (k.glub_f < a.N) {
    if (k.C) k.C = reinterpret_cast<unsigned short*>(k.C) - k.glub_f;
    if (k.R) k.R = reinterpret_cast<const unsigned short*>(k.R) - k.glub_f;
  } else if (a.glub_x) {
    k.C = nullptr;
  }
  if (a.gn_done) *a.gn_done = 0;
  if (a.lnb_done) *a.lnb_done = 0;
  if (dtype == DH_DTYPE_F16) gemm_dispatch<f16>(k, a.partial_elems, st, a.gn_done, a.lnb_done, dtype);
  else gemm_dispatch<bf16>(k, a.partial_elems, st, a.gn_done, a.lnb_done, dtype);
  return 2.0 * (double)a.M * (double)a.N * (double)a.K;
}

}

#ifdef DH_TUNING
extern "C" int dh_dbg_gemm_timeline(unsigned long long* ts) { dh::g_gemm_ts = ts; return DH_OK; }
#endif

extern "C" int dh_dbg_gemm_family(int force) {
  DH_REQUIRE(force >= 0 && force <= 2, "family: 0 policy, 1 k_gemm_dma, 2 k_gemm_pp");
  dh::g_pp_force = force;
  return DH_OK;
}

extern "C" int dh_dbg_gemm_stage(int buf) {
  dh::g_buf_stage = buf;
  return DH_OK;
}

extern "C" int dh_dbg_gemm_last_tile(int* out) {
  DH_REQUIRE(out != nullptr, "null pointer");
  const dh::GemmTileReport& r = dh::g_last_tile;
  const int v[9] = {r.bm, r.bn, r.kg, r.stages, r.mw, r.splits, r.pp, r.gn_epi, r.reduce_gn};
  for (int i = 0; i < 9; ++i) out[i] = v[i];
  return DH_OK;
}

extern "C" int dh_gemm_profile_begin(void) {
  dh::g_prof.on = true;
  dh::g_prof.used = 0;
  dh::g_prof.flops = 0;
  dh::g_prof.bytes = 0;
  return DH_OK;
}
extern "C" int dh_gemm_profile_bytes(double* bytes) {
  if (bytes) *bytes = dh::g_prof.bytes;
  return DH_OK;
}
extern "C" int dh_gemm_profile_end(double* ms_total, int64_t* launches, double* flops) {
  using namespace dh;
  g_prof.on = false;
  double ms = 0;
  if (g_prof.used >= 2) DH_CHECK_HIP(hipEventSynchronize(g_prof.ev[g_prof.used - 1]));
  for (size_t i = 0; i + 1 < g_prof.used; i += 2) {
    float t = 0;
    DH_CHECK_HIP(hipEventElapsedTime(&t, g_prof.ev[i], g_prof.ev[i + 1]));
    ms += t;
  }
  if (ms_total) *ms_total = ms;
  if (launches) *launches = (int64_t)(g_prof.used / 2);
  if (flops) *flops = g_prof.flops;
  return DH_OK;
}
```

### diffusionhandles_amd/csrc/gemm_k.h

```cpp
#pragma once
#include "unet_kernels.h"

namespace dh {

typedef _Float16 v8h __attribute__((ext_vector_type(8)));
typedef __bf16 v8b __attribute__((ext_vector_type(8)));
typedef float v16f __attribute__((ext_vector_type(16)));

template <class T> struct Mfma;
template <> struct Mfma<f16> {
  static __device__ __forceinline__ v16f run(uint4 a, uint4 b, v16f c) {
    return __builtin_amdgcn_mfma_f32_32x32x16_f16(__builtin_bit_cast(v8h, a), __builtin_bit_cast(v8h, b), c, 0, 0, 0);
  }
};
template <> struct Mfma<bf16> {
  static __device__ __forceinline__ v16f run(uint4 a, uint4 b, v16f c) {
    return __builtin_amdgcn_mfma_f32_32x32x16_bf16(__builtin_bit_cast(v8b, a), __builtin_bit_cast(v8b, b), c, 0, 0, 0);
  }
};

struct GemmK {
  const void* A; long lda;
  const void* W;
  int M, N, K;
  int mode, Hin, Win, Cin, Hout, Wout, stride, up, pad;
  const float* bias;
  const float* rowvec; int rowvec_ld; int rows_per_batch; float inv_rows_per_batch;
  const void* R; long ldr;
  void* C; long ldc;
  int act_silu;
  int pre_r;
  int wide_store;
#ifdef DH_TUNING
  int w_nt;
  unsigned long long* ts;
  int lnf_abl;
#endif
  const float* ln_s; const float* ln_t; float* ln_stats; float ln_eps;
  float* partial;
  int splits, k_per_split;
  float* gn_part; int gn_HW, gn_G, gn_S;
  int gn_epi, gn_cpg;
  const void* gnb_x; long gnb_ldx; const float *gnb_gamma, *gnb_beta, *gnb_stats; int gnb_silu;
  const void* lnb_x; long lnb_ldx; const float *lnb_gamma, *lnb_stats; const void* lnb_add; void* lnb_dx;
  void* glu_y; long glu_ldy; const void* glub_x; void* glub_dx;
  int glub_f;
  int pp_tm, pp_tn, pp_order, pp_nwork; unsigned pp_a_bytes, pp_w_bytes;
  unsigned long long* pp_ts;
};


__host__ __device__ constexpr bool glub_tile_is_glu(int n0, int glub_f) { return n0 < glub_f; }
__host__ __device__ constexpr bool glub_split_ok(int BN, int glub_f) { return BN > 0 && glub_f % BN == 0; }

struct PpPlan { int bm = 0, bn = 0, splits = 1; };
bool gemm_pp_plan(const GemmK& k, size_t partial_elems, int force, PpPlan* plan);
void launch_gemm_pp(int dtype, const GemmK& k, const PpPlan& plan, hipStream_t st, hipEvent_t e0, hipEvent_t e1);

}
```

### diffusionhandles_amd/csrc/unet_engine.cpp

```cpp
#include <stdlib.h>

#include <algorithm>
#include <map>
#include <numeric>
#include <vector>

#include "unet_kernels.h"

namespace dh {

enum OpType { OP_CONV_IN, OP_CONV_OUT, OP_GEMM, OP_GN, OP_LN, OP_ATTN, OP_GEGLU, OP_CONCAT, OP_TIMESTEP, OP_T2F };
enum ParamKind { PK_F32, PK_MAT };

struct Ten {
  size_t off = 0, goff = 0;
  size_t off_fo = 0;
  int rows = 0, C = 0;
  int ld = 0;
  int view = -1, col = 0;
  bool req_grad = true;
  bool persistent = false;
};

struct Wt {
  size_t fwd_off = 0, bwd_off = 0;
  int N = 0, K = 0, taps = 1;
  bool has_bwd = true, f32 = false;
  int glu_F = 0;
};

struct ParamInfo {
  std::string name;
  int ndim = 0;
  int64_t shape[4] = {0, 0, 0, 0};
  int kind = PK_F32;
  size_t f32_off = 0;
  int wt = -1;
  int row_off = 0;
  int glu_F = 0;
};

struct Op {
  int type = OP_GEMM;
  int in0 = -1, in1 = -1, out = -1, res = -1;
  int wt = -1;
  long bias_off = -1;
  long gamma_off = -1, beta_off = -1;
  int mode = A_DENSE, Hin = 0, Win = 0, Cin = 0, Hout = 0, Wout = 0, stride = 1, up = 0;
  int in_col = 0, in_cols = 0;
  long rowvec_off = -1; int rowvec_ld = 0;
  int act_silu = 0;
  float eps = 1e-5f; int silu = 0; int groups = 32; size_t stats_off = 0;
  int heads = 0, Nq = 0, Nk = 0, cross = 0, kv_col = 0; size_t lse_off = 0;
  int gn_next = -1;
  int ln_fold = -1, folded = 0;
  long ln_s_off = -1, ln_t_off = -1;
  int glu_op = -1, glub_op = -1;
};

struct FfFold {
  int wt_po = -1, wt_ffo = -1, wt = -1;
  long b_po = -1, b_ffo = -1, bias = -1;
};

}

using namespace dh;

struct dh_unet {
  dh_unet_config cfg;
  int dtype = DH_DTYPE_F16;
  std::vector<Ten> tens;
  std::vector<Wt> wts;
  std::vector<ParamInfo> params;
  std::vector<Op> ops;
  std::vector<FfFold> ffolds;
  std::map<std::string, int> pindex;
  size_t w16_elems = 0, pf_elems = 0, act_elems = 0, grad_elems = 0, f32_elems = 0;
  size_t fo_elems = 0;
  size_t partial_elems = 0, scratch_elems = 0, small_elems = 0;
  unsigned short *w16 = nullptr, *act = nullptr, *grad = nullptr, *scratch = nullptr;
  float *pf = nullptr, *f32a = nullptr, *partial = nullptr, *small = nullptr;
  int t_text = -1, t_kv = -1, t_conv_in_out = -1, t_final = -1, act_ids[3] = {-1, -1, -1};
  int act_op_end[3] = {0, 0, 0};
  int first_cross_op = 0;
  int saved_ops = 0;
  int temb_ops = 0, temb_rows = 0;
  float temb_t = 0.f;
  hipStream_t temb_stream = nullptr;
  uint64_t text_key = 0, kv_key = 0;
  int kv_rows = 0;
  hipStream_t kv_stream = nullptr;
  long temb_f32_off = -1;
  int temb_total = 0, kv_total = 0;
  float *in_sample = nullptr, *in_text = nullptr, *io_eps = nullptr, *out_dsample = nullptr, *out_dtext = nullptr, *t_dev = nullptr;
  std::map<uint64_t, hipGraphExec_t> graphs;
  std::map<uint64_t, double> graph_flops;
  bool use_graphs = true;
  long ones_off = -1, zeros_off = -1;
  bool fold_dirty = true;
  bool owns_weights = true;
  int n_shared = 0;
  int saved_batch = 0;
  const float* saved_sample = nullptr;
  std::vector<char> gready;
  double flops_fwd = 0, flops_bwd = 0;
  int64_t launches = 0;

  bool fo_mode = false;
  unsigned short* aptr(int t, int B_unused = 0) { return act + (fo_mode && !tens[t].persistent ? tens[t].off_fo : tens[t].off); }
  std::vector<int> galias;
  unsigned short* gptr(int t) {
    while (galias[t] != t) t = galias[t];
    return grad + tens[t].goff;
  }
};

namespace {

struct Builder {
  dh_unet& u;
  int maxB, maxBd;
  explicit Builder(dh_unet& uu) : u(uu), maxB(uu.cfg.max_batch), maxBd(uu.cfg.max_diff_batch) {}

  int tensor(int rows, int C, bool req_grad = true) {
    Ten t;
    t.rows = rows; t.C = C; t.ld = C; t.req_grad = req_grad;
    u.tens.push_back(t);
    return (int)u.tens.size() - 1;
  }
  void set_view(int t, int root, int col) {
    Ten& tt = u.tens[t];
    tt.view = root; tt.col = col; tt.ld = u.tens[root].C;
  }
  size_t f32_slot(size_t n) { size_t o = u.f32_elems; u.f32_elems += align_up(n, 64); return o; }

  long param_f32(const std::string& name, int n) {
    ParamInfo p;
    p.name = name; p.ndim = 1; p.shape[0] = n; p.kind = PK_F32;
    p.f32_off = u.pf_elems;
// ... 72 lines not shown
               bool req_grad = true) {
    const Ten tx = u.tens[x];
    Op o;
    o.type = OP_GEMM; o.mode = A_DENSE; o.in0 = x; o.res = res; o.wt = wt; o.bias_off = bias_off;
    o.in_col = in_col; o.in_cols = in_cols ? in_cols : tx.C; o.act_silu = silu;
    o.out = tensor(tx.rows, u.wts[wt].N, req_grad);
    u.ops.push_back(o);
    return o.out;
  }
  int linear(int x, const std::string& pre, int N, bool bias, int res, bool as_conv1x1 = false) {
    const int K = u.tens[x].C;
    const int wt = weight(N, K);
    if (as_conv1x1) bind_conv1x1(pre + ".weight", wt, N, K); else bind_mat(pre + ".weight", wt, N, 0, K, 1);
    const long b = bias ? param_f32(pre + ".bias", N) : -1;
    return linear_w(x, wt, b, res);
  }
  int concat(int a, int b) {
    Op o;
    o.type = OP_CONCAT; o.in0 = a; o.in1 = b;
    o.out = tensor(u.tens[a].rows, u.tens[a].C + u.tens[b].C);
    u.ops.push_back(o);
    return o.out;
  }

  void fold_ln_into_last_gemm() {
    const int gi = (int)u.ops.size() - 1, li = gi - 1;
    Op& g = u.ops[gi];
    Op& l = u.ops[li];
    if (g.type != OP_GEMM || l.type != OP_LN || g.in0 != l.out || g.mode != A_DENSE || g.in_col != 0) return;
    const int N = u.wts[g.wt].N;
    g.ln_fold = li; l.folded = 1;
    g.ln_s_off = (long)u.pf_elems; u.pf_elems += align_up((size_t)N, 64);
    g.ln_t_off = (long)u.pf_elems; u.pf_elems += align_up((size_t)N, 64);
  }

  int temb_cursor = 0, kv_cursor = 0;
  int wt_temb = -1, wt_kv = -1;
  size_t temb_bias_off = 0;

  int resnet(int x, const std::string& pre, int Cout, int H) {
    const int Cin = u.tens[x].C;
    int h = gn(x, pre + ".norm1", 1e-5f, true);
    bind_mat(pre + ".time_emb_proj.weight", wt_temb, Cout, temb_cursor, u.cfg.block_out_channels[0] * 4, 1);
    param_f32_at(pre + ".time_emb_proj.bias", Cout, temb_bias_off + temb_cursor);
    const long toff = temb_cursor;
    temb_cursor += Cout;
    h = conv3(h, pre + ".conv1", Cout, H, 1, 0, toff, -1);
    h = gn(h, pre + ".norm2", 1e-5f, true);
    int sc = x;
    if (Cin != Cout) sc = linear(x, pre + ".conv_shortcut", Cout, true, -1, true);
    return conv3(h, pre + ".conv2", Cout, H, 1, 0, -1, sc);
  }

  int transformer(int x, const std::string& pre, int heads, int H) {
    const int C = u.tens[x].C, N = H * H;
    int h = gn(x, pre + ".norm", 1e-6f, false);
    int t0 = linear(h, pre + ".proj_in", C, true, -1);
    const std::string b = pre + ".transformer_blocks.0";
    int n1 = ln(t0, b + ".norm1");
    const int wqkv = weight(3 * C, C);
    bind_mat(b + ".attn1.to_q.weight", wqkv, C, 0, C, 1);
    bind_mat(b + ".attn1.to_k.weight", wqkv, C, C, C, 1);
    bind_mat(b + ".attn1.to_v.weight", wqkv, C, 2 * C, C, 1);
    int qkv = linear_w(n1, wqkv, -1, -1);
    fold_ln_into_last_gemm();
    Op a;
    a.type = OP_ATTN; a.in0 = qkv; a.heads = heads; a.Nq = N; a.Nk = N; a.cross = 0;
    a.out = tensor(N, C);
    a.lse_off = f32_slot((size_t)maxB * heads * N);
    u.ops.push_back(a);
    int t1 = linear(a.out, b + ".attn1.to_out.0", C, true, t0);
    int n2 = ln(t1, b + ".norm2");
    int q2 = linear(n2, b + ".attn2.to_q", C, false, -1);
    fold_ln_into_last_gemm();
    bind_mat(b + ".attn2.to_k.weight", wt_kv, C, kv_cursor, u.cfg.cross_attention_dim, 1);
    bind_mat(b + ".attn2.to_v.weight", wt_kv, C, kv_cursor + C, u.cfg.cross_attention_dim, 1);
    Op c;
    c.type = OP_ATTN; c.in0 = q2; c.in1 = u.t_kv; c.heads = heads; c.Nq = N; c.Nk = u.cfg.text_len; c.cross = 1;
    c.kv_col = kv_cursor;
    kv_cursor += 2 * C;
    c.out = tensor(N, C);
    c.lse_off = f32_slot((size_t)maxB * heads * N);
    u.ops.push_back(c);
    const int tg = tensor(N, 5 * C, false);
    int t2 = linear(c.out, b + ".attn2.to_out.0", C, true, t1);
    set_view(t2, tg, 4 * C);
    int n3 = ln(t2, b + ".norm3");
    int gg = linear(n3, b + ".ff.net.0.proj", 8 * C, true, -1);
    fold_ln_into_last_gemm();
    const int ff1 = (int)u.ops.size() - 1;
    u.wts[u.ops[ff1].wt].glu_F = 4 * C;
    u.params[u.pindex[b + ".ff.net.0.proj.weight"]].glu_F = 4 * C;
    u.params[u.pindex[b + ".ff.net.0.proj.bias"]].glu_F = 4 * C;
    Op g;
    g.type = OP_GEGLU; g.in0 = gg; g.out = tensor(N, 4 * C);
    set_view(g.out, tg, 0);
    u.ops.push_back(g);
    u.ops[ff1].glu_op = (int)u.ops.size() - 1;
    FfFold f;
    f.wt_ffo = weight(C, 4 * C);
    bind_mat(b + ".ff.net.2.weight", f.wt_ffo, C, 0, 4 * C, 1);
    f.b_ffo = param_f32(b + ".ff.net.2.bias", C);
    f.wt_po = weight(C, C, 1, false);
    bind_mat(pre + ".proj_out.weight", f.wt_po, C, 0, C, 1);
    f.b_po = param_f32(pre + ".proj_out.bias", C);
    f.wt = weight(C, 5 * C, 1, true, false, true);
    f.bias = (long)u.pf_elems; u.pf_elems += align_up((size_t)C, 64);
    u.ffolds.push_back(f);
    const int out = linear_w(tg, f.wt, f.bias, x);
    u.ops.back().glub_op = u.ops[ff1].glu_op;
    u.ops.back().in1 = t2;
    return out;
  }
};

void count_fused(const dh_unet_config& c, int& temb_total, int& kv_total) {
  const int L = c.n_levels, n = c.layers_per_block;
  temb_total = 0; kv_total = 0;
  for (int i = 0; i < L; ++i) {
    temb_total += n * c.block_out_channels[i];
    if (i < L - 1) kv_total += n * 2 * c.block_out_channels[i];
  }
  temb_total += 2 * c.block_out_channels[L - 1];
  kv_total += 2 * c.block_out_channels[L - 1];
  for (int i = 0; i < L; ++i) {
    const int ch = c.block_out_channels[L - 1 - i];
    temb_total += (n + 1) * ch;
    if (i > 0) kv_total += (n + 1) * 2 * ch;
  }
}

static void layout_tensors(dh_unet& u);
static size_t ff_fold_scratch(int C);

int build(dh_unet& u) {
  const dh_unet_config& c = u.cfg;
  Builder b(u);
  const int L = c.n_levels, n = c.layers_per_block, S = c.sample_size;
  const int* ch = c.block_out_channels;
  const int temb_dim = ch[0] * 4;
  count_fused(c, u.temb_total, u.kv_total);

  int t_sin = b.tensor(1, ch[0], false);
  { Op o; o.type = OP_TIMESTEP; o.out = t_sin; u.ops.push_back(o); }
  const int w1 = b.weight(temb_dim, ch[0], 1, false);
  b.bind_mat("time_embedding.linear_1.weight", w1, temb_dim, 0, ch[0], 1);
  int e1 = b.linear_w(t_sin, w1, b.param_f32("time_embedding.linear_1.bias", temb_dim), -1, 0, 0, true, false);
  const int w2 = b.weight(temb_dim, temb_dim, 1, false);
  b.bind_mat("time_embedding.linear_2.weight", w2, temb_dim, 0, temb_dim, 1);
  int e2 = b.linear_w(e1, w2, b.param_f32("time_embedding.linear_2.bias", temb_dim), -1, 0, 0, true, false);
  b.wt_temb = b.weight(u.temb_total, temb_dim, 1, false);
  b.temb_bias_off = u.pf_elems;
  u.pf_elems += align_up((size_t)u.temb_total, 64);
  int t_temb = b.linear_w(e2, b.wt_temb, (long)b.temb_bias_off, -1, 0, 0, false, false);
  u.temb_f32_off = (long)b.f32_slot((size_t)c.max_batch * u.temb_total);
  { Op o; o.type = OP_T2F; o.in0 = t_temb; u.ops.push_back(o); }
  u.temb_ops = (int)u.ops.size();

  u.t_text = b.tensor(c.text_len, c.cross_attention_dim, true);
  b.wt_kv = b.weight(u.kv_total, c.cross_attention_dim);
  u.t_kv = b.linear_w(u.t_text, b.wt_kv, -1, -1);

  { Op o;
    o.type = OP_CONV_IN;
    o.wt = b.weight(ch[0], 9 * c.in_channels, 9, true, true);
    b.bind_mat("conv_in.weight", o.wt, ch[0], 0, c.in_channels, 9);
    o.bias_off = b.param_f32("conv_in.bias", ch[0]);
    o.Hin = S; o.Cin = c.in_channels;
// ... 13 lines not shown
    }
    if (down) {
      x = b.conv3(x, pre + ".downsamplers.0.conv", ch[i], H, 2, 0, -1, -1);
      H /= 2;
      skips.push_back(x);
    }
  }
  x = b.resnet(x, "mid_block.resnets.0", ch[L - 1], H);
  x = b.transformer(x, "mid_block.attentions.0", c.heads[L - 1], H);
  x = b.resnet(x, "mid_block.resnets.1", ch[L - 1], H);
  int n_act = 0;
  for (int i = 0; i < L; ++i) {
    const std::string pre = "up_blocks." + std::to_string(i);
    const int co = ch[L - 1 - i];
    const bool attn = i > 0, up = i < L - 1;
    for (int j = 0; j < n + 1; ++j) {
      const int sk = skips.back();
      skips.pop_back();
      x = b.concat(x, sk);
      x = b.resnet(x, pre + ".resnets." + std::to_string(j), co, H);
      if (attn) x = b.transformer(x, pre + ".attentions." + std::to_string(j), c.heads[L - 1 - i], H);
    }
    if (up) {
      x = b.conv3(x, pre + ".upsamplers.0.conv", co, H, 1, 1, -1, -1);
      H *= 2;
    }
    if (attn && n_act < 3) {
      u.act_op_end[n_act] = (int)u.ops.size();
      u.act_ids[n_act++] = x;
    }
  }
  x = b.gn(x, "conv_norm_out", 1e-5f, true);
  u.t_final = x;
  { Op o;
    o.type = OP_CONV_OUT; o.in0 = x;
    o.wt = b.weight(c.out_channels, 9 * ch[0], 9, true, true);
    b.bind_mat("conv_out.weight", o.wt, c.out_channels, 0, ch[0], 9);
    o.bias_off = b.param_f32("conv_out.bias", c.out_channels);
    o.Hin = S; o.Cin = ch[0];
    u.ops.push_back(o); }
  if (b.temb_cursor != u.temb_total || b.kv_cursor != u.kv_total) {
    set_error("internal: fused projection sizes do not match");
    return DH_ERR_STATE;
  }
  u.first_cross_op = 0;
  for (size_t i = 0; i < u.ops.size(); ++i)
    if (u.ops[i].type == OP_ATTN && u.ops[i].cross) { u.first_cross_op = (int)i; break; }
  for (size_t i = 0; i + 1 < u.ops.size(); ++i) {
    Op& o = u.ops[i];
    const Op& nx = u.ops[i + 1];
    if (nx.type == OP_GN && nx.in0 == o.out && (o.type == OP_GEMM || o.type == OP_CONCAT)) o.gn_next = (int)(i + 1);
  }
  { int cmax = 0;
    for (const Op& o : u.ops) if (o.type == OP_LN) cmax = std::max(cmax, u.tens[o.in0].C);
    u.ones_off = (long)u.pf_elems; u.pf_elems += align_up((size_t)cmax, 64);
    u.zeros_off = (long)u.pf_elems; u.pf_elems += align_up((size_t)cmax, 64); }
  layout_tensors(u);
  size_t biggest = 0;
  for (const Ten& t : u.tens) biggest = std::max(biggest, (size_t)t.rows * t.C * c.max_diff_batch);
  u.scratch_elems = biggest * 4 + 1024;
  for (const FfFold& f : u.ffolds) u.scratch_elems = std::max(u.scratch_elems, ff_fold_scratch(u.wts[f.wt_po].N));
  u.partial_elems = std::max<size_t>((size_t)48 << 20, biggest * 2);
  u.small_elems = (size_t)c.max_batch * 64 * 4096 + (size_t)c.max_batch * c.norm_groups * 4 + 4096;
  return DH_OK;
}


static void layout_tensors(dh_unet& u) {
  const size_t maxB = (size_t)u.cfg.max_batch, maxBd = (size_t)u.cfg.max_diff_batch;
  const int nt = (int)u.tens.size(), nops = (int)u.ops.size();
  u.tens[u.t_text].persistent = true;
  u.tens[u.t_kv].persistent = true;
  for (int i = 0; i < 3; ++i)
    if (u.act_ids[i] >= 0) u.tens[u.act_ids[i]].persistent = true;
  auto root = [&](int t) { return t >= 0 && u.tens[t].view >= 0 ? u.tens[t].view : t; };
  std::vector<int> first(nt, nops), last(nt, -1);
  auto rd = [&](int t, int oi) { t = root(t); if (t >= 0) { last[t] = std::max(last[t], oi); first[t] = std::min(first[t], oi); } };
  auto wr = [&](int t, int oi) { t = root(t); if (t >= 0) { first[t] = std::min(first[t], oi); last[t] = std::max(last[t], oi); } };
  for (int oi = 0; oi < nops; ++oi) {
    const Op& o = u.ops[oi];
    rd(o.in0, oi); rd(o.in1, oi); rd(o.res, oi); wr(o.out, oi);
    if (o.ln_fold >= 0) rd(u.ops[o.ln_fold].in0, oi);
    if (o.glu_op >= 0) wr(u.ops[o.glu_op].out, oi);
  }
  std::vector<char> written(nt, 0);
  for (const Op& o : u.ops) { if (o.out >= 0) written[root(o.out)] = 1; if (o.glu_op >= 0) written[root(u.ops[o.glu_op].out)] = 1; }
  for (int t = 0; t < nt; ++t)
    if (u.tens[t].view < 0 && (!written[t] || t == u.t_final)) {
      first[t] = 0; last[t] = nops; u.tens[t].persistent = u.tens[t].persistent || !written[t];
    }
  u.act_elems = 0; u.grad_elems = 0;
  for (Ten& t : u.tens) {
    if (t.view < 0) {
      t.off = u.act_elems;
      u.act_elems += align_up((size_t)t.rows * t.C * (t.persistent ? maxB : maxBd), 128);
    }
    if (t.req_grad) { t.goff = u.grad_elems; u.grad_elems += align_up((size_t)t.rows * t.C * maxBd, 128); }
  }
  struct Live { size_t off, end; int last; };
  std::vector<Live> live;
  for (const Ten& t : u.tens)
    if (t.persistent) live.push_back({t.off, t.off + align_up((size_t)t.rows * t.C * maxB, 128), nops + 1});
  std::vector<int> order(nt);
  std::iota(order.begin(), order.end(), 0);
  std::stable_sort(order.begin(), order.end(), [&](int a, int b) { return first[a] < first[b]; });
  size_t fo_end = 0;
  for (const Live& l : live) fo_end = std::max(fo_end, l.end);
  for (int t : order) {
    Ten& tt = u.tens[t];
    if (tt.view >= 0) continue;
    if (tt.persistent) { tt.off_fo = tt.off; continue; }
    if (last[t] < 0) { tt.off_fo = 0; continue; }
    const size_t size = align_up((size_t)tt.rows * tt.C * maxB, 128);
    live.erase(std::remove_if(live.begin(), live.end(), [&](const Live& l) { return l.last < first[t]; }), live.end());
    std::sort(live.begin(), live.end(), [](const Live& a, const Live& b) { return a.off < b.off; });
    size_t pos = 0;
    for (const Live& l : live) {
      if (pos + size <= l.off) break;
      pos = std::max(pos, l.end);
    }
    tt.off_fo = pos;
    live.push_back({pos, pos + size, last[t]});
    fo_end = std::max(fo_end, pos + size);
  }
  u.fo_elems = fo_end;
  u.act_elems = std::max(u.act_elems, fo_end);
  for (Ten& t : u.tens)
    if (t.view >= 0) {
      const Ten& r = u.tens[t.view];
      t.off = r.off + t.col; t.off_fo = r.off_fo + t.col; t.persistent = r.persistent;
    }
}

template <class D, bool TILED>
__global__ void k_load_weight(const float* src, int N, int C, int taps, D* fwd, long fwd_K, long row_off, D* bwd,
                              long bwd_K, long col_off, int Nb, float scale = 1.f, int glu_F = 0) {
  const size_t idx = (size_t)blockIdx.x * blockDim.x + threadIdx.x;
  if (idx >= (size_t)N * C * taps) return;
  const int tap = (int)(idx % taps);
  const int cc = (int)((idx / taps) % C);
  int nn = (int)(idx / ((size_t)taps * C));
  if (glu_F) nn = glu_col(nn >= glu_F ? nn - glu_F : nn, nn >= glu_F ? 1 : 0);
  const D v = from_f32<D>(src[idx] * scale);
  int fk = tap * C + cc, bk = (taps - 1 - tap) * Nb + (int)col_off + nn;
  if (TILED && taps == 9) { fk = conv_k_index(tap, cc); bk = conv_k_index(taps - 1 - tap, (int)col_off + nn); }
  const int fr = (int)row_off + nn;
  if (TILED) {
    fwd[wt_index(fr, fk, (int)fwd_K)] = v;
    if (bwd) bwd[wt_index(cc, bk, (int)bwd_K)] = v;
  } else {
    fwd[(size_t)fr * fwd_K + fk] = v;
    if (bwd) bwd[(size_t)cc * bwd_K + bk] = v;
  }
}

}
namespace dh {
void launch_load_weight(int dtype, const float* src, int N, int C, int taps, void* fwd, long fwd_K, long row_off, void* bwd,
                        long bwd_K, long col_off, int Nb, float scale, hipStream_t st) {
  const size_t total = (size_t)N * C * taps;
  const unsigned nb = (unsigned)((total + 255) / 256);
  if (dtype == DH_DTYPE_F32)
    hipLaunchKernelGGL((k_load_weight<float, false>), dim3(nb), dim3(256), 0, st, src, N, C, taps, (float*)fwd, fwd_K, row_off, (float*)bwd, bwd_K, col_off, Nb, scale);
  else if (dtype == DH_DTYPE_F16)
    hipLaunchKernelGGL((k_load_weight<f16, true>), dim3(nb), dim3(256), 0, st, src, N, C, taps, (f16*)fwd, fwd_K, row_off, (f16*)bwd, bwd_K, col_off, Nb, scale);
  else
// ... 230 lines not shown
}

extern "C" int dh_unet_load_param(dh_unet* u, int i, const float* src, void* stream) {
  DH_REQUIRE(u && src && i >= 0 && i < (int)u->params.size(), "bad arguments");
  if (!u->owns_weights || u->n_shared > 0) {
    set_error("dh_unet_load_param: the weights are shared (dh_unet_create_shared): load every parameter before sharing");
    return DH_ERR_STATE;
  }
  u->temb_rows = 0; u->fold_dirty = true; u->kv_key = 0;
  hipStream_t st = (hipStream_t)stream;
  const ParamInfo& p = u->params[i];
  if (p.kind == PK_F32) {
    if (p.glu_F) {
      hipLaunchKernelGGL(k_load_glu_bias, dim3(cdiv((int)p.shape[0], 256)), dim3(256), 0, st, src, u->pf + p.f32_off, p.glu_F);
      DH_LAUNCH_CHECK();
      return DH_OK;
    }
    DH_CHECK_HIP(hipMemcpyAsync(u->pf + p.f32_off, src, (size_t)p.shape[0] * 4, hipMemcpyDeviceToDevice, st));
    return DH_OK;
  }
  const Wt& w = u->wts[p.wt];
  const int N = (int)p.shape[0], C = (int)p.shape[1], taps = w.taps;
  const size_t total = (size_t)N * C * taps;
  const unsigned nb = (unsigned)((total + 255) / 256);
  const long fwd_ld = w.K;
  const long bwd_ld = (long)taps * w.N;
  if (w.f32) {
    float* f = u->pf + w.fwd_off;
    float* b = w.has_bwd ? u->pf + w.bwd_off : nullptr;
    hipLaunchKernelGGL((k_load_weight<float, false>), dim3(nb), dim3(256), 0, st, src, N, C, taps, f, fwd_ld, (long)p.row_off,
                       b, bwd_ld, (long)p.row_off, w.N);
  } else if (u->dtype == DH_DTYPE_F16) {
    f16* f = (f16*)(u->w16 + w.fwd_off);
    f16* b = w.has_bwd ? (f16*)(u->w16 + w.bwd_off) : nullptr;
    hipLaunchKernelGGL((k_load_weight<f16, true>), dim3(nb), dim3(256), 0, st, src, N, C, taps, f, fwd_ld, (long)p.row_off, b,
                       bwd_ld, (long)p.row_off, w.N, 1.f, w.glu_F);
  } else {
    bf16* f = (bf16*)(u->w16 + w.fwd_off);
    bf16* b = w.has_bwd ? (bf16*)(u->w16 + w.bwd_off) : nullptr;
    hipLaunchKernelGGL((k_load_weight<bf16, true>), dim3(nb), dim3(256), 0, st, src, N, C, taps, f, fwd_ld, (long)p.row_off, b,
                       bwd_ld, (long)p.row_off, w.N, 1.f, w.glu_F);
  }
  DH_LAUNCH_CHECK();
  return DH_OK;
}

extern "C" size_t dh_unet_weight_bytes(const dh_unet* u) { return u && u->owns_weights ? u->w16_elems * 2 + u->pf_elems * 4 : 0; }
extern "C" size_t dh_unet_workspace_bytes(const dh_unet* u) {
  return u ? (u->act_elems + u->grad_elems + u->scratch_elems) * 2 + (u->f32_elems + u->partial_elems + u->small_elems) * 4 : 0;
}

static void fill_gemm(dh_unet* u, const Op& o, int B, GemmArgs& g) {
  const Wt& w = u->wts[o.wt];
  const Ten& ti = u->tens[o.in0];
  const Ten& to = u->tens[o.out];
  g.A = u->aptr(o.in0) + o.in_col; g.lda = ti.ld;
  g.W = u->w16 + w.fwd_off;
  g.M = B * to.rows; g.N = w.N; g.K = w.K;
  g.mode = o.mode; g.Hin = o.Hin; g.Win = o.Win; g.Cin = o.Cin; g.Hout = o.Hout; g.Wout = o.Wout;
  g.stride = o.stride; g.up = o.up;
  g.bias = o.bias_off >= 0 ? u->pf + o.bias_off : nullptr;
  if (o.rowvec_off >= 0) { g.rowvec = u->f32a + o.rowvec_off; g.rowvec_ld = o.rowvec_ld; g.rows_per_batch = to.rows; }
  if (o.res >= 0) { g.R = u->aptr(o.res); g.ldr = u->tens[o.res].ld; }
  g.C = u->aptr(o.out); g.ldc = to.ld;
  g.act_silu = o.act_silu;
  g.partial = u->partial; g.partial_elems = u->partial_elems;
  if (o.ln_fold >= 0) {
    const Op& l = u->ops[o.ln_fold];
    if (use_ln_fold(u, B)) {
      g.A = u->aptr(l.in0); g.lda = u->tens[l.in0].ld;
      g.bias = nullptr;
      g.ln_s = u->pf + o.ln_s_off; g.ln_t = u->pf + o.ln_t_off; g.ln_stats = u->f32a + l.stats_off; g.ln_eps = l.eps;
    } else {
      g.bias = u->pf + o.ln_t_off;
    }
  }
}

static void forward_ops(dh_unet* u, int B, int n_ops, int first_op, bool kv_hit, bool save, hipStream_t st) {
  const int dt = u->dtype;
  const dh_unet_config& c = u->cfg;
  u->flops_fwd = 0;
  int gn_have = 0;
  if (!kv_hit) launch_f32_to_t(dt, u->in_text, u->aptr(u->t_text), (size_t)B * c.text_len * c.cross_attention_dim, st);
  for (int oi = first_op; oi < n_ops; ++oi) {
    const Op& o = u->ops[oi];
    if (kv_hit && oi == u->temb_ops) continue;
    switch (o.type) {
      case OP_TIMESTEP:
        launch_timestep_embedding(dt, u->t_dev, c.block_out_channels[0], B, u->aptr(o.out), st);
        break;
      case OP_T2F:
        launch_t_to_f32(dt, u->aptr(o.in0), u->f32a + u->temb_f32_off, (size_t)B * u->temb_total, 0, st);
        break;
      case OP_CONV_IN: {
        const Wt& w = u->wts[o.wt];
        launch_conv_small_fwd(dt, u->in_sample, 1, u->pf + w.fwd_off, u->pf + o.bias_off, u->aptr(o.out), 0, B, o.Hin, o.Hin,
                              o.Cin, w.N, st);
        u->flops_fwd += 2.0 * B * o.Hin * o.Hin * w.N * w.K;
        break;
      }
      case OP_CONV_OUT: {
        const Wt& w = u->wts[o.wt];
        launch_conv_small_fwd(dt, u->aptr(o.in0), 0, u->pf + w.fwd_off, u->pf + o.bias_off, u->io_eps, 1, B, o.Hin, o.Hin,
                              o.Cin, w.N, st);
        u->flops_fwd += 2.0 * B * o.Hin * o.Hin * w.N * w.K;
        break;
      }
      case OP_GEMM: {
        GemmArgs g;
        fill_gemm(u, o, B, g);
        gn_have = 0;
        if (o.gn_next >= 0 && oi + 1 < n_ops) {
          const Ten& to = u->tens[o.out];
          g.gn_part = u->small; g.gn_HW = to.rows; g.gn_G = u->ops[o.gn_next].groups; g.gn_done = &gn_have;
        }
        if (o.glu_op >= 0 && o.glu_op < n_ops) {
          const Op& ge = u->ops[o.glu_op];
          g.glu_y = u->aptr(ge.out); g.glu_ldy = u->tens[ge.out].ld;
          if (!save) g.C = nullptr;
        }
        u->flops_fwd += launch_gemm(dt, g, st);
        break;
      }
      case OP_GN: {
        const Ten& t = u->tens[o.in0];
        const int have = (oi > 0 && u->ops[oi - 1].gn_next == oi) ? gn_have : 0;
        launch_groupnorm_fwd(dt, u->aptr(o.in0), u->pf + o.gamma_off, u->pf + o.beta_off, u->aptr(o.out),
                             u->f32a + o.stats_off, u->small, B, t.rows, t.C, o.groups, o.eps, o.silu, st, have);
        gn_have = 0;
        break;
      }
      case OP_LN: {
        if (o.folded && use_ln_fold(u, B)) break;
        const Ten& t = u->tens[o.in0];
        launch_layernorm_fwd(dt, u->aptr(o.in0), u->pf + (o.folded ? u->ones_off : o.gamma_off),
                             u->pf + (o.folded ? u->zeros_off : o.beta_off), u->aptr(o.out),
                             u->f32a + o.stats_off, B * t.rows, t.C, o.eps, st, t.ld);
        break;
      }
      case OP_ATTN: {
        const Ten& tq = u->tens[o.in0];
        const int C = u->tens[o.out].C;
        if (!o.cross) {
          const unsigned short* qkv = u->aptr(o.in0);
          launch_attention_fwd(dt, qkv, tq.C, qkv + C, qkv + 2 * C, tq.C, u->aptr(o.out), C, u->f32a + o.lse_off, B,
                               o.heads, o.Nq, o.Nk, st);
        } else {
          const Ten& tkv = u->tens[o.in1];
          const unsigned short* kv = u->aptr(o.in1) + o.kv_col;
          launch_attention_fwd(dt, u->aptr(o.in0), tq.C, kv, kv + C, tkv.C, u->aptr(o.out), C, u->f32a + o.lse_off, B,
                               o.heads, o.Nq, o.Nk, st);
        }
        u->flops_fwd += 4.0 * B * o.heads * (double)o.Nq * o.Nk * 64;
        break;
      }
      case OP_GEGLU: {
        if (oi > 0 && u->ops[oi - 1].glu_op == oi) break;
        const Ten& t = u->tens[o.out];
        launch_geglu_fwd(dt, u->aptr(o.in0), u->aptr(o.out), B * t.rows, t.C, st);
        break;
      }
      case OP_CONCAT: {
        const Ten &a = u->tens[o.in0], &b2 = u->tens[o.in1], &t = u->tens[o.out];
        gn_have = 0;
        const int G = o.gn_next >= 0 ? u->ops[o.gn_next].groups : 0;
        if (o.gn_next >= 0 && oi + 1 < n_ops && a.C % 8 == 0 && b2.C % 8 == 0 && t.C % G == 0 &&
            (GN_GB * (t.C / G)) % 8 == 0 && GN_GB * (t.C / G) <= 2048) {
          launch_concat_gn(dt, u->aptr(o.in0), a.C, u->aptr(o.in1), b2.C, u->aptr(o.out), u->small, B, t.rows, G, st);
          gn_have = 1;
        } else {
          launch_copy_cols(dt, u->aptr(o.in0), a.C, u->aptr(o.out), t.C, B * t.rows, a.C, 0, st);
          launch_copy_cols(dt, u->aptr(o.in1), b2.C, u->aptr(o.out) + a.C, t.C, B * t.rows, b2.C, 0, st);
        }
        break;
      }
    }
  }
}

static uint64_t graph_key_fwd(int B, int n_ops, bool temb_hit, bool kv_hit, bool save) {
  return (uint64_t)B | ((uint64_t)n_ops << 12) | ((uint64_t)(temb_hit ? 1 : 0) << 34) | ((uint64_t)(kv_hit ? 1 : 0) << 36) |
         ((uint64_t)(save ? 1 : 0) << 37);
}
static uint64_t graph_key_bwd(int B, unsigned mask, bool eps, bool sample, bool text) {
  return (uint64_t)B | ((uint64_t)(mask & 7u) << 28) | ((uint64_t)(eps ? 1 : 0) << 31) | ((uint64_t)(sample ? 1 : 0) << 32) |
         ((uint64_t)(text ? 1 : 0) << 33) | (1ull << 35);
}

template <class F>
static int run_graphed(dh_unet* u, uint64_t key, hipStream_t st, double* flops_slot, F body) {
  if (!u->use_graphs || st == nullptr || gemm_profiling_on()) { body(); return DH_OK; }
  auto it = u->graphs.find(key);
  if (it == u->graphs.end()) {
    hipGraph_t graph = nullptr;
    DH_CHECK_HIP(hipStreamBeginCapture(st, hipStreamCaptureModeThreadLocal));
    body();
    DH_CHECK_HIP(hipStreamEndCapture(st, &graph));
    hipGraphExec_t exec = nullptr;
    DH_CHECK_HIP(hipGraphInstantiate(&exec, graph, nullptr, nullptr, 0));
    (void)hipGraphDestroy(graph);
    u->graphs[key] = exec;
    u->graph_flops[key] = *flops_slot;
    it = u->graphs.find(key);
  }
  *flops_slot = u->graph_flops[key];
  DH_CHECK_HIP(hipGraphLaunch(it->second, st));
  return DH_OK;
}

extern "C" int dh_unet_forward(dh_unet* u, const float* sample, float timestep, const float* text, int batch,
                               int save_for_backward, float* eps_out, void* const* act_out, void* stream) {
  DH_REQUIRE(u && sample && text, "null pointer");
  DH_REQUIRE(batch >= 1 && batch <= u->cfg.max_batch, "batch exceeds max_batch");
  DH_REQUIRE(!save_for_backward || batch <= u->cfg.max_diff_batch, "a forward saved for a backward pass exceeds max_diff_batch");
  hipStream_t st = (hipStream_t)stream;
  const int B = batch;
  const dh_unet_config& c = u->cfg;
  const size_t ns = (size_t)B * c.sample_size * c.sample_size;
  if (sample != u->in_sample) DH_CHECK_HIP(hipMemcpyAsync(u->in_sample, sample, ns * c.in_channels * 4, hipMemcpyDeviceToDevice, st));
  int n_ops = (int)u->ops.size();
  if (!eps_out) {
    n_ops = 0;
    for (int i = 0; i < 3; ++i)
      if (act_out && act_out[i]) n_ops = std::max(n_ops, u->act_op_end[i]);
    DH_REQUIRE(n_ops > 0, "nothing requested: eps_out and every act_out are null");
  }
  if (u->fold_dirty) fold_layernorms(u, st);
  const bool temb_hit = u->temb_rows >= B && u->temb_t == timestep && u->temb_stream == st;
  const bool kv_hit = u->text_key != 0 && u->text_key == u->kv_key && u->kv_rows == B && u->kv_stream == st;
  const int first_op = temb_hit ? u->temb_ops : 0;
  if (!kv_hit && text != u->in_text)
    DH_CHECK_HIP(hipMemcpyAsync(u->in_text, text, (size_t)B * c.text_len * c.cross_attention_dim * 4, hipMemcpyDeviceToDevice, st));
  if (!temb_hit) launch_set_scalar(u->t_dev, timestep, st);
  const bool save = save_for_backward != 0;
  u->fo_mode = !save;
  int rc = run_graphed(u, graph_key_fwd(B, n_ops, temb_hit, kv_hit, save), st, &u->flops_fwd,
                       [&]() { forward_ops(u, B, n_ops, first_op, kv_hit, save, st); });
  u->fo_mode = false;
  if (rc != DH_OK) { u->temb_rows = 0; u->kv_key = 0; return rc; }
  if (!temb_hit) { u->temb_t = timestep; u->temb_rows = B; u->temb_stream = st; }
  if (!kv_hit) { u->kv_key = u->text_key; u->kv_rows = B; u->kv_stream = st; }
  if (eps_out && eps_out != u->io_eps)
    DH_CHECK_HIP(hipMemcpyAsync(eps_out, u->io_eps, ns * c.out_channels * 4, hipMemcpyDeviceToDevice, st));
  if (act_out) {
    for (int i = 0; i < 3; ++i)
      if (act_out[i]) {
        DH_REQUIRE(u->act_op_end[i] <= n_ops, "activation requested beyond the truncated tape");
        const Ten& t = u->tens[u->act_ids[i]];
        if (act_out[i] != (void*)u->aptr(u->act_ids[i]))
          DH_CHECK_HIP(hipMemcpyAsync(act_out[i], u->aptr(u->act_ids[i]), (size_t)B * t.rows * t.C * 2,
                                      hipMemcpyDeviceToDevice, st));
      }
  }
  u->saved_batch = save_for_backward ? B : 0;
  u->saved_ops = n_ops;
  DH_LAUNCH_CHECK();
  return DH_OK;
}

namespace {
struct Bwd {
  dh_unet* u;
  int B, dt;
  hipStream_t st;
  bool need_text;
  void add_into(int t, const unsigned short* src, long lds_, int cols, int col_off = 0) {
    const Ten& tt = u->tens[t];
    launch_copy_cols(dt, src, lds_, u->gptr(t) + col_off, tt.C, B * tt.rows, cols, u->gready[t] ? 1 : 0, st);
  }
};
}

static void backward_ops(dh_unet* u, int B, unsigned act_mask, bool has_eps, bool want_sample, bool want_text,
                         hipStream_t st) {
  const int dt = u->dtype;
  const dh_unet_config& c = u->cfg;
  const float* d_eps = has_eps ? u->io_eps : nullptr;
  float* d_sample = want_sample ? u->out_dsample : nullptr;
  float* d_text = want_text ? u->out_dtext : nullptr;
  u->flops_bwd = 0;
  std::fill(u->gready.begin(), u->gready.end(), 0);
  for (int i = 0; i < 3; ++i)
    if (act_mask & (1u << i)) u->gready[u->act_ids[i]] = 1;
  Bwd bw{u, B, dt, st, d_text != nullptr};
  bool text_grad_written = false;
  int gnb_have = 0, gnb_for = -1;
  int lnb_have = 0, lnb_for = -1;
  int cat_done = -1;
  int glub_done = -1;
  for (int oi = (int)u->ops.size() - 1; oi >= 0; --oi) {
    const Op& o = u->ops[oi];
    if (!want_sample && oi < u->first_cross_op && o.out != u->t_kv) continue;
    switch (o.type) {
      case OP_CONV_OUT: {
        if (!d_eps) break;
        const Wt& w = u->wts[o.wt];
        launch_conv_small_bwd(dt, d_eps, 1, u->pf + w.bwd_off, u->gptr(o.in0), 0, 0, B, o.Hin, o.Hin, w.N, o.Cin, st);
        u->gready[o.in0] = 1;
        u->flops_bwd += 2.0 * B * o.Hin * o.Hin * w.N * w.K;
        break;
      }
      case OP_CONV_IN: {
        if (!d_sample || !u->gready[o.out]) break;
        const Wt& w = u->wts[o.wt];
        launch_conv_small_bwd(dt, u->gptr(o.out), 0, u->pf + w.bwd_off, d_sample, 1, 0, B, o.Hin, o.Hin, w.N, o.Cin, st);
        u->flops_bwd += 2.0 * B * o.Hin * o.Hin * w.N * w.K;
        break;
      }
      case OP_GEMM: {
        if (!u->tens[o.out].req_grad || !u->gready[o.out]) break;
        const Ten& to = u->tens[o.out];
        const Ten& ti = u->tens[o.in0];
        const Wt& w = u->wts[o.wt];
        if (o.res >= 0 && u->tens[o.res].req_grad) {
          if (u->gready[o.res]) bw.add_into(o.res, u->gptr(o.out), to.C, to.C);
          else u->galias[o.res] = o.out;
          u->gready[o.res] = 1;
        }
        if (o.glub_op >= 0 && o.in1 >= 0) {
          const Op& ge = u->ops[o.glub_op];
          const int t2 = o.in1;
          GemmArgs g;
          g.A = u->gptr(o.out); g.lda = to.C;
          g.W = u->w16 + w.bwd_off;
          g.mode = A_DENSE; g.M = B * to.rows; g.N = w.K; g.K = w.N;
          g.partial = u->partial; g.partial_elems = u->partial_elems;
          g.glub_x = u->aptr(ge.in0); g.glub_dx = u->gptr(ge.in0); g.glub_f = u->tens[ge.out].C;
          g.C = u->gptr(t2); g.ldc = u->tens[t2].C;
          if (u->gready[t2]) { g.R = g.C; g.ldr = g.ldc; }
          u->flops_bwd += launch_gemm(dt, g, st);
          u->gready[ge.in0] = 1; u->gready[ge.out] = 1; u->gready[t2] = 1;
          glub_done = o.glub_op;
          break;
        }
        if (!ti.req_grad || !w.has_bwd) break;
        if (o.in0 == u->t_text && !bw.need_text) break;
        GemmArgs g;
        g.A = u->gptr(o.out); g.lda = to.C;
        g.W = u->w16 + w.bwd_off;
        g.partial = u->partial; g.partial_elems = u->partial_elems;
        if (o.mode == A_DENSE) {
          g.mode = A_DENSE;
          g.M = B * to.rows; g.N = w.K; g.K = w.N;
          g.C = u->gptr(o.in0) + o.in_col; g.ldc = ti.C;
          if (u->gready[o.in0]) { g.R = g.C; g.ldr = ti.C; }
          lnb_have = 0;
          if (oi > 0 && u->ops[oi - 1].type == OP_LN && u->ops[oi - 1].out == o.in0 && !u->gready[o.in0] && o.in_col == 0 &&
              w.K == ti.C) {
            const Op& ln = u->ops[oi - 1];
            g.lnb_x = u->aptr(ln.in0); g.lnb_ldx = u->tens[ln.in0].ld; g.lnb_gamma = u->pf + ln.gamma_off; g.lnb_stats = u->f32a + ln.stats_off;
            g.lnb_add = u->gready[ln.in0] ? u->gptr(ln.in0) : nullptr; g.lnb_dx = u->gptr(ln.in0);
            g.lnb_done = &lnb_have;
            lnb_for = oi - 1;
          }
          if (oi > 0 && u->ops[oi - 1].type == OP_GN && u->ops[oi - 1].out == o.in0 && !u->gready[o.in0] && o.in_col == 0 &&
              w.K == ti.C) {
            const Op& gn = u->ops[oi - 1];
            const Ten& tx = u->tens[gn.in0];
            g.gnb_x = u->aptr(gn.in0); g.gnb_ldx = tx.ld;
            g.gnb_gamma = u->pf + gn.gamma_off; g.gnb_beta = u->pf + gn.beta_off; g.gnb_stats = u->f32a + gn.stats_off;
            g.gnb_silu = gn.silu;
            g.gn_part = u->small; g.gn_HW = tx.rows; g.gn_G = gn.groups; g.gn_done = &gnb_have;
            gnb_have = 0;
            gnb_for = oi - 1;
          }
          u->flops_bwd += launch_gemm(dt, g, st);
          u->gready[o.in0] = 1;
        } else if (o.up) {
          g.mode = A_CONV3; g.stride = 1; g.up = 0;
          g.Hin = o.Hout; g.Win = o.Wout; g.Cin = w.N; g.Hout = o.Hout; g.Wout = o.Wout;
          g.M = B * o.Hout * o.Wout; g.N = o.Cin; g.K = 9 * w.N;
          g.C = u->scratch; g.ldc = o.Cin;
          u->flops_bwd += launch_gemm(dt, g, st);
          launch_pool2x2_sum(dt, u->scratch, u->gptr(o.in0), B, o.Hin, o.Win, o.Cin, u->gready[o.in0] ? 1 : 0, st);
          u->gready[o.in0] = 1;
        } else {
          g.mode = o.stride == 2 ? A_CONVT2 : A_CONV3;
          g.stride = 1; g.up = 0;
          g.Hin = o.Hout; g.Win = o.Wout; g.Cin = w.N;
          g.Hout = o.Hin; g.Wout = o.Win;
          g.M = B * o.Hin * o.Win; g.N = o.Cin; g.K = 9 * w.N;
          g.C = u->gptr(o.in0); g.ldc = ti.C;
          if (u->gready[o.in0]) { g.R = g.C; g.ldr = ti.C; }
          gnb_have = 0;
          int gi = -1;
          if (oi > 0 && u->ops[oi - 1].type == OP_GN && u->ops[oi - 1].out == o.in0) gi = oi - 1;
          else if (oi > 1 && u->ops[oi - 1].type == OP_GEMM && u->ops[oi - 1].mode == A_DENSE && u->ops[oi - 1].out == o.res &&
                   u->ops[oi - 1].in0 != o.in0 && u->ops[oi - 2].type == OP_GN && u->ops[oi - 2].out == o.in0)
            gi = oi - 2;
          if (gi >= 0) {
            const Op& gn = u->ops[gi];
            const Ten& tx = u->tens[gn.in0];
            g.gnb_x = u->aptr(gn.in0); g.gnb_ldx = tx.ld;
            g.gnb_gamma = u->pf + gn.gamma_off; g.gnb_beta = u->pf + gn.beta_off; g.gnb_stats = u->f32a + gn.stats_off;
            g.gnb_silu = gn.silu;
            g.gn_part = u->small; g.gn_HW = tx.rows; g.gn_G = gn.groups; g.gn_done = &gnb_have;
            gnb_for = gi;
          }
          u->flops_bwd += launch_gemm(dt, g, st);
          u->gready[o.in0] = 1;
        }
        if (o.in0 == u->t_text) text_grad_written = true;
        break;
      }
      case OP_GN: {
        if (!u->gready[o.out]) break;
        const Ten& t = u->tens[o.in0];
        GnBwdSplit split;
        if (oi > 0 && u->ops[oi - 1].type == OP_CONCAT && u->ops[oi - 1].out == o.in0) {
          const Op& cat = u->ops[oi - 1];
          const int ca = u->tens[cat.in0].C;
          if (!u->gready[cat.in0] && !u->gready[cat.in1] && ca % 8 == 0 && ca + u->tens[cat.in1].C == t.C) {
            split.out0 = u->gptr(cat.in0); split.out1 = u->gptr(cat.in1); split.split_c = ca;
            cat_done = oi - 1;
          }
        }
        launch_groupnorm_bwd(dt, u->aptr(o.in0), u->gptr(o.out), u->pf + o.gamma_off, u->pf + o.beta_off,
                             u->f32a + o.stats_off, u->gptr(o.in0), u->small, B, t.rows, t.C, o.groups, o.silu,
                             u->gready[o.in0] ? 1 : 0, st, gnb_for == oi ? gnb_have : 0, split);
        gnb_have = 0;
        u->gready[o.in0] = 1;
        if (split.out0) { u->gready[u->ops[oi - 1].in0] = 1; u->gready[u->ops[oi - 1].in1] = 1; }
        break;
      }
      case OP_LN: {
        if (!u->gready[o.out]) break;
        if (lnb_have && lnb_for == oi) {
          lnb_have = 0;
          u->gready[o.in0] = 1;
          break;
        }
        const Ten& t = u->tens[o.in0];
        launch_layernorm_bwd(dt, u->aptr(o.in0), u->gptr(o.out), u->pf + o.gamma_off, u->f32a + o.stats_off,
                             u->gready[o.in0] ? u->gptr(o.in0) : nullptr, u->gptr(o.in0), B * t.rows, t.C, st, t.ld);
        u->gready[o.in0] = 1;
        break;
      }
      case OP_GEGLU: {
        if (!u->gready[o.out]) break;
        if (glub_done == oi) { glub_done = -1; break; }
        const Ten& t = u->tens[o.out];
        launch_geglu_bwd(dt, u->aptr(o.in0), u->gptr(o.out), u->gptr(o.in0), B * t.rows, t.C, st);
        u->gready[o.in0] = 1;
        break;
      }
      case OP_ATTN: {
        if (!u->gready[o.out]) break;
        const Ten& tq = u->tens[o.in0];
        const int C = u->tens[o.out].C;
        float* delta = u->small;
        if (!o.cross) {
          const unsigned short* qkv = u->aptr(o.in0);
          unsigned short* dqkv = u->gptr(o.in0);
          launch_attention_bwd_dq(dt, qkv, tq.C, qkv + C, qkv + 2 * C, tq.C, u->aptr(o.out), C, u->gptr(o.out), C,
                                  u->f32a + o.lse_off, delta, dqkv, tq.C, B, o.heads, o.Nq, o.Nk, st);
          launch_attention_bwd_dkv(dt, qkv, tq.C, qkv + C, qkv + 2 * C, tq.C, u->gptr(o.out), C, u->f32a + o.lse_off,
                                   delta, dqkv + C, dqkv + 2 * C, tq.C, B, o.heads, o.Nq, o.Nk, st);
          u->flops_bwd += 14.0 * B * o.heads * (double)o.Nq * o.Nk * 64;
        } else {
          const Ten& tkv = u->tens[o.in1];
          const unsigned short* kv = u->aptr(o.in1) + o.kv_col;
          launch_attention_bwd_dq(dt, u->aptr(o.in0), tq.C, kv, kv + C, tkv.C, u->aptr(o.out), C, u->gptr(o.out), C,
                                  u->f32a + o.lse_off, delta, u->gptr(o.in0), tq.C, B, o.heads, o.Nq, o.Nk, st);
          u->flops_bwd += 6.0 * B * o.heads * (double)o.Nq * o.Nk * 64;
          if (bw.need_text) {
            unsigned short* dkv = u->gptr(o.in1) + o.kv_col;
            launch_attention_bwd_dkv(dt, u->aptr(o.in0), tq.C, kv, kv + C, tkv.C, u->gptr(o.out), C,
                                     u->f32a + o.lse_off, delta, dkv, dkv + C, tkv.C, B, o.heads, o.Nq, o.Nk, st, u->partial,
                                     u->partial_elems);
            u->gready[o.in1] = 1;
            u->flops_bwd += 8.0 * B * o.heads * (double)o.Nq * o.Nk * 64;
          }
        }
        u->gready[o.in0] = 1;
        break;
      }
      case OP_CONCAT: {
        if (!u->gready[o.out]) break;
        if (cat_done == oi) { cat_done = -1; break; }
        const Ten &a = u->tens[o.in0], &b2 = u->tens[o.in1], &t = u->tens[o.out];
        launch_split_cols(dt, u->gptr(o.out), t.C, u->gptr(o.in0), a.C, a.C, u->gready[o.in0] ? 1 : 0, u->gptr(o.in1), b2.C,
                          b2.C, u->gready[o.in1] ? 1 : 0, B * t.rows, st);
        u->gready[o.in0] = 1;
        u->gready[o.in1] = 1;
        break;
      }
      default: break;
    }
  }
  if (d_text) {
    const size_t n = (size_t)B * c.text_len * c.cross_attention_dim;
    if (text_grad_written) launch_t_to_f32(dt, u->gptr(u->t_text), d_text, n, 0, st);
    else (void)hipMemsetAsync(d_text, 0, n * 4, st);
  }
}

extern "C" int dh_unet_backward(dh_unet* u, void* const* d_act, const float* d_eps, float* d_sample, float* d_text,
                                void* stream) {
  DH_REQUIRE(u, "null engine");
  DH_REQUIRE(u->saved_batch > 0, "no saved forward: call dh_unet_forward(save_for_backward=1) first");
  hipStream_t st = (hipStream_t)stream;
  const int B = u->saved_batch;
  const dh_unet_config& c = u->cfg;
  const size_t ns = (size_t)B * c.sample_size * c.sample_size;
  const size_t nt = (size_t)B * c.text_len * c.cross_attention_dim;
  unsigned mask = 0;
  std::iota(u->galias.begin(), u->galias.end(), 0);
  DH_REQUIRE(!d_eps || u->saved_ops == (int)u->ops.size(), "d_eps given but the saved forward did not compute eps");
  if (d_act)
    for (int i = 0; i < 3; ++i)
      if (d_act[i]) {
        DH_REQUIRE(u->act_op_end[i] <= u->saved_ops, "d_act given for an activation the saved forward did not compute");
        const Ten& t = u->tens[u->act_ids[i]];
        if (d_act[i] != (void*)u->gptr(u->act_ids[i]))
          DH_CHECK_HIP(hipMemcpyAsync(u->gptr(u->act_ids[i]), d_act[i], (size_t)B * t.rows * t.C * 2,
                                      hipMemcpyDeviceToDevice, st));
        mask |= 1u << i;
      }
  if (d_eps && d_eps != u->io_eps) DH_CHECK_HIP(hipMemcpyAsync(u->io_eps, d_eps, ns * c.out_channels * 4, hipMemcpyDeviceToDevice, st));
  const uint64_t key = graph_key_bwd(B, mask, d_eps != nullptr, d_sample != nullptr, d_text != nullptr);
  int rc = run_graphed(u, key, st, &u->flops_bwd,
                       [&]() { backward_ops(u, B, mask, d_eps != nullptr, d_sample != nullptr, d_text != nullptr, st); });
  if (rc != DH_OK) return rc;
  if (d_sample && d_sample != u->out_dsample)
    DH_CHECK_HIP(hipMemcpyAsync(d_sample, u->out_dsample, ns * c.in_channels * 4, hipMemcpyDeviceToDevice, st));
  if (d_text && d_text != u->out_dtext) DH_CHECK_HIP(hipMemcpyAsync(d_text, u->out_dtext, nt * 4, hipMemcpyDeviceToDevice, st));
  DH_LAUNCH_CHECK();
  return DH_OK;
}

extern "C" int dh_unet_io_ptr(dh_unet* u, int which, int index, void** ptr, size_t* bytes) {
  DH_REQUIRE(u && ptr, "null pointer");
  const dh_unet_config& c = u->cfg;
  const size_t ns = (size_t)c.max_batch * c.sample_size * c.sample_size;
  const size_t nt = (size_t)c.max_batch * c.text_len * c.cross_attention_dim;
  size_t n = 0;
  switch (which) {
    case DH_IO_SAMPLE: *ptr = u->in_sample; n = ns * c.in_channels * 4; break;
    case DH_IO_TEXT: *ptr = u->in_text; n = nt * 4; break;
    case DH_IO_EPS: *ptr = u->io_eps; n = ns * c.out_channels * 4; break;
    case DH_IO_DSAMPLE: *ptr = u->out_dsample; n = ns * c.in_channels * 4; break;
// ... 71 lines not shown
```

### diffusionhandles_amd/csrc/unet_kernels.h

```cpp
#pragma once
#include "common.h"

namespace dh {

__device__ inline float silu_grad(float z) {
  const float s = 1.f / (1.f + __expf(-z));
  return s * (1.f + z * (1.f - s));
}

struct GeluParts { float Phi, pdf; };
__device__ __forceinline__ GeluParts gelu_parts(float g) {
  const float x = fabsf(g) * 0.70710678118654752f;
  const float t = __builtin_amdgcn_rcpf(fmaf(0.3275911f, x, 1.f));
  const float e = __expf(-x * x);
  const float poly = t * (0.254829592f + t * (-0.284496736f + t * (1.421413741f + t * (-1.453152027f + t * 1.061405429f))));
  const float q = 0.5f * poly * e;
  return {g < 0.f ? q : 1.f - q, e * 0.3989422804014327f};
}
__device__ __forceinline__ float gelu_f(float g) { return g * gelu_parts(g).Phi; }
__device__ __forceinline__ float gelu_grad(float g) { const GeluParts p = gelu_parts(g); return fmaf(g, p.pdf, p.Phi); }
__host__ __device__ inline int glu_col(int o, int gate) { return 32 * (o >> 4) + 16 * gate + (o & 15); }
__host__ __device__ inline int glu_src_row(int n, int F) { return ((n >> 4) & 1) * F + 16 * (n >> 5) + (n & 15); }

enum { A_DENSE = 0, A_CONV3 = 1, A_CONVT2 = 2 };

struct GemmArgs {
  const void* A = nullptr; long lda = 0;
  const void* W = nullptr;
  int M = 0, N = 0, K = 0;
  int mode = A_DENSE;
  int Hin = 0, Win = 0, Cin = 0;
  int Hout = 0, Wout = 0;
  int stride = 1, up = 0;
  int pad = 1;
  const float* bias = nullptr;
  const float* rowvec = nullptr; int rowvec_ld = 0; int rows_per_batch = 1;
  const void* R = nullptr; long ldr = 0;
  void* C = nullptr; long ldc = 0;
  int act_silu = 0;
  float* partial = nullptr; size_t partial_elems = 0;
  float* gn_part = nullptr; int gn_HW = 0, gn_G = 0; int* gn_done = nullptr;
  const void* gnb_x = nullptr; long gnb_ldx = 0; const float *gnb_gamma = nullptr, *gnb_beta = nullptr, *gnb_stats = nullptr;
  int gnb_silu = 0;
  const float* ln_s = nullptr; const float* ln_t = nullptr; float* ln_stats = nullptr; float ln_eps = 1e-5f;
  const void* lnb_x = nullptr; long lnb_ldx = 0; const float *lnb_gamma = nullptr, *lnb_stats = nullptr; const void* lnb_add = nullptr;
  void* lnb_dx = nullptr; int* lnb_done = nullptr;
  void* glu_y = nullptr; long glu_ldy = 0;
  const void* glub_x = nullptr; void* glub_dx = nullptr; int glub_f = 0;
};
void launch_splitk_reduce_ln_bwd(int dtype, const float* partial, int splits, const void* x, const float* gamma,
                                 const float* stats, const void* add, void* dx, int rows, int C, hipStream_t st, long ldx = 0);
double launch_gemm(int dtype, const GemmArgs& a, hipStream_t st);
bool gemm_profiling_on();
void launch_tile_weights(int dtype, const void* src, void* dst, int N, int K, hipStream_t st, int conv_cin = 0);
__host__ __device__ inline size_t wt_index(int n, int k, int K) {
  const int r = n & 63, c = (k & 63) >> 3;
  return ((size_t)(n >> 6) * (K >> 6) + (k >> 6)) * 4096 + (size_t)r * 64 + (size_t)((c ^ ((r >> 1) & 7)) << 3) + (k & 7);
}

__host__ __device__ inline int conv_k_index(int tap, int c) { return (c >> 6) * 576 + tap * 64 + (c & 63); }

void launch_load_weight(int dtype, const float* src, int N, int C, int taps, void* fwd, long fwd_K, long row_off, void* bwd,
                        long bwd_K, long col_off, int Nb, float scale, hipStream_t st);

void launch_conv_small_fwd(int dtype, const void* x, int x_is_f32, const float* w, const float* bias, void* y,
                           int y_is_f32, int B, int H, int W, int Cin, int Cout, hipStream_t st);
void launch_conv_small_bwd(int dtype, const void* dy, int dy_is_f32, const float* w, void* dx, int dx_is_f32,
                           int accumulate, int B, int H, int W, int Cin, int Cout, hipStream_t st);

void launch_groupnorm_fwd(int dtype, const void* x, const float* gamma, const float* beta, void* y, float* stats,
                          float* scratch, int B, int HW, int C, int G, float eps, int silu, hipStream_t st,
                          int have_partials = 0);
int gn_slices(int HW, int B);
constexpr int GN_GB = 4;
void launch_concat_gn(int dtype, const void* a, int Ca, const void* b, int Cb, void* out, float* gn_part, int B, int HW,
                      int G, hipStream_t st);
struct GnBwdSplit { void* out0 = nullptr; void* out1 = nullptr; int split_c = 0; };
void launch_groupnorm_bwd(int dtype, const void* x, const void* dy, const float* gamma, const float* beta,
                          const float* stats, void* dx, float* scratch, int B, int HW, int C, int G, int silu,
                          int accumulate, hipStream_t st, int have_partials = 0, GnBwdSplit split = GnBwdSplit());
void launch_gelu(int dtype, const void* x, void* y, size_t n, hipStream_t st);
void launch_layernorm_fwd(int dtype, const void* x, const float* gamma, const float* beta, void* y, float* stats,
                          int rows, int C, float eps, hipStream_t st, long ldx = 0);
void launch_layernorm_bwd(int dtype, const void* x, const void* dy, const float* gamma, const float* stats,
                          const void* add, void* dx, int rows, int C, hipStream_t st, long ldx = 0);
void launch_geglu_fwd(int dtype, const void* x, void* y, int rows, int F, hipStream_t st);
void launch_geglu_bwd(int dtype, const void* x, const void* dy, void* dx, int rows, int F, hipStream_t st);
void launch_copy_cols(int dtype, const void* src, long lds, void* dst, long ldd, int rows, int cols, int accumulate,
                      hipStream_t st);
void launch_split_cols(int dtype, const void* src, long lds, void* dstA, long ldA, int colsA, int accA, void* dstB, long ldB,
                       int colsB, int accB, int rows, hipStream_t st);
void launch_lane_ops_probe(const float* in, float* out, unsigned* ex, hipStream_t st);
void launch_pool2x2_sum(int dtype, const void* src, void* dst, int B, int h, int w, int C, int accumulate,
                        hipStream_t st);
void launch_f32_to_t(int dtype, const float* src, void* dst, size_t n, hipStream_t st);
void launch_t_to_f32(int dtype, const void* src, float* dst, size_t n, int accumulate, hipStream_t st);
void launch_timestep_embedding(int dtype, const float* t_dev, int dim, int B, void* out, hipStream_t st);
void launch_set_scalar(float* p, float v, hipStream_t st);

void launch_attention_fwd(int dtype, const void* q, long ldq, const void* k, const void* v, long ldk, void* o,
                          long ldo, float* lse, int B, int H, int Nq, int Nk, hipStream_t st, int causal = 0);
void launch_attention_delta(int dtype, const void* o, long ldo, const void* d_o, long lddo, float* delta, int B,
                            int H, int Nq, hipStream_t st);
void launch_attention_bwd_dq(int dtype, const void* q, long ldq, const void* k, const void* v, long ldk, const void* o,
                             long ldo, const void* d_o, long lddo, const float* lse, float* delta, void* dq, long lddq,
                             int B, int H, int Nq, int Nk, hipStream_t st);
void launch_attention_bwd_dkv(int dtype, const void* q, long ldq, const void* k, const void* v, long ldk,
                              const void* d_o, long lddo, const float* lse, const float* delta, void* dk, void* dv,
                              long lddk, int B, int H, int Nq, int Nk, hipStream_t st, float* scratch = nullptr,
                              size_t scratch_elems = 0);

}
```

Measured before the change: 37.69 steps/s.

## Fuse cross-attention forward and dQ backward into Q-projection GEMM epilogues

```diff
diff --git a/diffusionhandles_amd/_lib.py b/diffusionhandles_amd/_lib.py
--- a/diffusionhandles_amd/_lib.py
+++ b/diffusionhandles_amd/_lib.py
@@ -146,6 +146,10 @@
     "dh_dbg_unet_ff_fold": (c_i, [c_p, c_i, ctypes.POINTER(c_i), ctypes.POINTER(c_i), c_p, c_p, c_p]),
     "dh_dbg_gemm_family": (c_i, [c_i]),
     "dh_dbg_gemm_stage": (c_i, [c_i]),
+    "dh_dbg_gemm_xattn": (c_i, [c_i, c_p, c_l, c_p, c_i, c_i, c_i, c_p, c_p, c_p, c_p, c_f, c_p, c_p, c_p, c_l, c_p, c_p, c_i, c_i, c_i,
+                                ctypes.POINTER(c_i), c_p]),
+    "dh_dbg_gemm_xattn_dq": (c_i, [c_i, c_p, c_l, c_p, c_i, c_i, c_i, c_p, c_p, c_p, c_p, c_l, c_p, c_p, c_p, c_i, c_i, ctypes.POINTER(c_i), c_p]),
+    "dh_dbg_gemm_xattn_carried": (c_i, [ctypes.POINTER(c_i), ctypes.POINTER(ctypes.c_longlong)]),
     "dh_dbg_gemm_pp_variant": (c_i, [c_i, c_p]),
     "dh_dbg_gemm_pp_ablate": (c_i, [c_i]),
     "dh_dbg_gemm_pp_persist": (c_i, [c_i]),
diff --git a/diffusionhandles_amd/csrc/attention.hip b/diffusionhandles_amd/csrc/attention.hip
--- a/diffusionhandles_amd/csrc/attention.hip
+++ b/diffusionhandles_amd/csrc/attention.hip
@@ -1,39 +1,7 @@
-#include "unet_kernels.h"
+#include "attn_tile.h"
 
 namespace dh {
 
-typedef _Float16 v8h __attribute__((ext_vector_type(8)));
-typedef __bf16 v8b __attribute__((ext_vector_type(8)));
-typedef float v16f __attribute__((ext_vector_type(16)));
-typedef short v4s __attribute__((ext_vector_type(4)));
-
-template <class T> struct Mma;
-template <> struct Mma<f16> {
-  static __device__ __forceinline__ v16f run(uint4 a, uint4 b, v16f c) {
-    return __builtin_amdgcn_mfma_f32_32x32x16_f16(__builtin_bit_cast(v8h, a), __builtin_bit_cast(v8h, b), c, 0, 0, 0);
-  }
-};
-template <> struct Mma<bf16> {
-  static __device__ __forceinline__ v16f run(uint4 a, uint4 b, v16f c) {
-    return __builtin_amdgcn_mfma_f32_32x32x16_bf16(__builtin_bit_cast(v8b, a), __builtin_bit_cast(v8b, b), c, 0, 0, 0);
-  }
-};
-
-constexpr int HD = 64;
-constexpr int TLD = 72;
-constexpr int TILE = 64 * TLD;
-constexpr float LOG2E = 1.4426950408889634f;
-constexpr float LN2 = 0.6931471805599453f;
-constexpr float SCALE = 0.125f;
-constexpr float CEXP = SCALE * LOG2E;
-
-__device__ __forceinline__ v16f zero16() {
-  v16f z;
-#pragma unroll
-  for (int i = 0; i < 16; ++i) z[i] = 0.f;
-  return z;
-}
-__device__ __forceinline__ float fast_exp2(float x) { return __builtin_amdgcn_exp2f(x); }
 #ifndef DH_ATTN_ABL
 #define DH_ATTN_ABL 0
 #endif
@@ -77,26 +45,6 @@
     const int idx = tid + j * GT;
     if (512 % GT == 0 || idx < 512) *reinterpret_cast<u4v*>(&rm[(idx >> 3) * TLD + (idx & 7) * 8]) = t.v[j];
   }
-}
-
-template <class T>
-__device__ __forceinline__ v16f tile_times_frags(const unsigned short* tile, int rowbase, int ln, int hi, const uint4 (&f)[4]) {
-  v16f acc = zero16();
-#pragma unroll
-  for (int kk = 0; kk < 4; ++kk) {
-    const uint4 a = *reinterpret_cast<const uint4*>(&tile[(rowbase + ln) * TLD + 16 * kk + 8 * hi]);
-    acc = Mma<T>::run(a, f[kk], acc);
-  }
-  return acc;
-}
-
-__device__ __forceinline__ uint4 tr_frag(const unsigned short* tptr, int cbase, int r0) {
-  typedef __attribute__((address_space(3))) v4s* lp;
-  const unsigned short* a = tptr + r0 * TLD + cbase;
-  const v4s lo = __builtin_amdgcn_ds_read_tr16_b64_v4i16((lp)(a));
-  const v4s up = __builtin_amdgcn_ds_read_tr16_b64_v4i16((lp)(a + 8 * TLD));
-  const uint2 l2 = __builtin_bit_cast(uint2, lo), u2 = __builtin_bit_cast(uint2, up);
-  return make_uint4(l2.x, l2.y, u2.x, u2.y);
 }
 
 constexpr int DTILE = 64 * 64;
@@ -175,25 +123,6 @@
 }
 
 template <class T>
-__device__ __forceinline__ uint4 pack8(const v16f& p, int s);
-template <>
-__device__ __forceinline__ uint4 pack8<f16>(const v16f& p, int s) {
-  uint4 o;
-  o.x = __builtin_bit_cast(unsigned, __builtin_amdgcn_cvt_pkrtz(p[8 * s + 0], p[8 * s + 1]));
-  o.y = __builtin_bit_cast(unsigned, __builtin_amdgcn_cvt_pkrtz(p[8 * s + 2], p[8 * s + 3]));
-  o.z = __builtin_bit_cast(unsigned, __builtin_amdgcn_cvt_pkrtz(p[8 * s + 4], p[8 * s + 5]));
-  o.w = __builtin_bit_cast(unsigned, __builtin_amdgcn_cvt_pkrtz(p[8 * s + 6], p[8 * s + 7]));
-  return o;
-}
-template <>
-__device__ __forceinline__ uint4 pack8<bf16>(const v16f& p, int s) {
-  bf16 o[8];
-#pragma unroll
-  for (int j = 0; j < 8; ++j) o[j] = (bf16)p[8 * s + j];
-  return *reinterpret_cast<uint4*>(o);
-}
-
-template <class T>
 __device__ __forceinline__ void store_rows_t(T* base, long ld, long row, int col0, int hi, const v16f (&acc)[2], float mul) {
 #pragma unroll
   for (int dt = 0; dt < 2; ++dt) {
@@ -211,8 +140,6 @@
     *reinterpret_cast<uint4*>(out + 16) = cb;
   }
 }
-
-__device__ __forceinline__ int acc_row(int r, int hi) { return (r & 3) + 8 * (r >> 2) + 4 * hi; }
 
 __device__ __forceinline__ void lds_barrier() {
   asm volatile("s_waitcnt lgkmcnt(0)" ::: "memory");
diff --git a/diffusionhandles_amd/csrc/attn_tile.h b/diffusionhandles_amd/csrc/attn_tile.h
--- /dev/null
+++ b/diffusionhandles_amd/csrc/attn_tile.h
@@ -0,0 +1,67 @@
+#pragma once
+#include "gemm_k.h"
+
+namespace dh {
+
+typedef short v4s __attribute__((ext_vector_type(4)));
+
+template <class T> using Mma = Mfma<T>;
+
+constexpr int HD = 64;
+constexpr int TLD = 72;
+constexpr int TILE = 64 * TLD;
+constexpr float LOG2E = 1.4426950408889634f;
+constexpr float LN2 = 0.6931471805599453f;
+constexpr float SCALE = 0.125f;
+constexpr float CEXP = SCALE * LOG2E;
+
+__device__ __forceinline__ v16f zero16() {
+  v16f z;
+#pragma unroll
+  for (int i = 0; i < 16; ++i) z[i] = 0.f;
+  return z;
+}
+__device__ __forceinline__ float fast_exp2(float x) { return __builtin_amdgcn_exp2f(x); }
+template <class T>
+__device__ __forceinline__ v16f tile_times_frags(const unsigned short* tile, int rowbase, int ln, int hi, const uint4 (&f)[4]) {
+  v16f acc = zero16();
+#pragma unroll
+  for (int kk = 0; kk < 4; ++kk) {
+    const uint4 a = *reinterpret_cast<const uint4*>(&tile[(rowbase + ln) * TLD + 16 * kk + 8 * hi]);
+    acc = Mma<T>::run(a, f[kk], acc);
+  }
+  return acc;
+}
+
+__device__ __forceinline__ uint4 tr_frag(const unsigned short* tptr, int cbase, int r0) {
+  typedef __attribute__((address_space(3))) v4s* lp;
+  const unsigned short* a = tptr + r0 * TLD + cbase;
+  const v4s lo = __builtin_amdgcn_ds_read_tr16_b64_v4i16((lp)(a));
+  const v4s up = __builtin_amdgcn_ds_read_tr16_b64_v4i16((lp)(a + 8 * TLD));
+  const uint2 l2 = __builtin_bit_cast(uint2, lo), u2 = __builtin_bit_cast(uint2, up);
+  return make_uint4(l2.x, l2.y, u2.x, u2.y);
+}
+
+template <class T>
+__device__ __forceinline__ uint4 pack8(const v16f& p, int s);
+template <>
+__device__ __forceinline__ uint4 pack8<f16>(const v16f& p, int s) {
+  uint4 o;
+  o.x = __builtin_bit_cast(unsigned, __builtin_amdgcn_cvt_pkrtz(p[8 * s + 0], p[8 * s + 1]));
+  o.y = __builtin_bit_cast(unsigned, __builtin_amdgcn_cvt_pkrtz(p[8 * s + 2], p[8 * s + 3]));
+  o.z = __builtin_bit_cast(unsigned, __builtin_amdgcn_cvt_pkrtz(p[8 * s + 4], p[8 * s + 5]));
+  o.w = __builtin_bit_cast(unsigned, __builtin_amdgcn_cvt_pkrtz(p[8 * s + 6], p[8 * s + 7]));
+  return o;
+}
+template <>
+__device__ __forceinline__ uint4 pack8<bf16>(const v16f& p, int s) {
+  bf16 o[8];
+#pragma unroll
+  for (int j = 0; j < 8; ++j) o[j] = (bf16)p[8 * s + j];
+  return *reinterpret_cast<uint4*>(o);
+}
+
+__device__ __forceinline__ int acc_row(int r, int hi) { return (r & 3) + 8 * (r >> 2) + 4 * hi; }
+
+
+}
diff --git a/diffusionhandles_amd/csrc/debug_api.cpp b/diffusionhandles_amd/csrc/debug_api.cpp
--- a/diffusionhandles_amd/csrc/debug_api.cpp
+++ b/diffusionhandles_amd/csrc/debug_api.cpp
@@ -138,6 +138,56 @@
   g.A = A; g.lda = lda; g.W = tiled; g.M = M; g.N = N; g.K = K; g.mode = A_DENSE; g.C = C; g.ldc = ldc;
   g.ln_s = ln_s; g.ln_t = ln_t; g.ln_stats = ln_stats; g.ln_eps = ln_eps;
   launch_gemm(dtype, g, (hipStream_t)stream);
+  DH_LAUNCH_CHECK();
+  return DH_OK;
+}
+extern "C" int dh_dbg_gemm_xattn(int dtype, const void* A, long lda, const void* W, int M, int N, int K, const float* bias,
+                                 const float* ln_s, const float* ln_t, float* ln_stats, float ln_eps, void* q, const void* k,
+                                 const void* v, long ldk, void* o, float* lse, int B, int Nk, int save, int* carried, void* stream) {
+  DH_REQUIRE(A && W && q && k && v && o && lse && K % 64 == 0 && N % 64 == 0 && B > 0 && M % B == 0 && Nk > 0, "bad arguments");
+  DH_REQUIRE(!ln_s || (ln_t && ln_stats), "the folded LayerNorm needs ln_s, ln_t and ln_stats");
+  static void* tiled = nullptr;
+  static size_t tiled_cap = 0;
+  const size_t need = (size_t)N * K * 2;
+  if (need > tiled_cap) {
+    if (tiled) (void)hipFree(tiled);
+    DH_CHECK_HIP(hipMalloc(&tiled, need));
+    tiled_cap = need;
+  }
+  launch_tile_weights(dtype, W, tiled, N, K, (hipStream_t)stream);
+  GemmArgs g;
+  g.A = A; g.lda = lda; g.W = tiled; g.M = M; g.N = N; g.K = K; g.mode = A_DENSE; g.bias = bias; g.C = q; g.ldc = N;
+  if (ln_s) { g.ln_s = ln_s; g.ln_t = ln_t; g.ln_stats = ln_stats; g.ln_eps = ln_eps; }
+  int have = 0;
+  g.xa_k = k; g.xa_v = v; g.xa_ldk = ldk; g.xa_o = o; g.xa_ldo = N; g.xa_lse = lse; g.xa_H = N / 64; g.xa_Nq = M / B; g.xa_Nk = Nk;
+  g.xa_save = save; g.xa_done = &have;
+  launch_gemm(dtype, g, (hipStream_t)stream);
+  if (!have) launch_attention_fwd(dtype, q, N, k, v, ldk, o, N, lse, B, N / 64, M / B, Nk, (hipStream_t)stream);
+  if (carried) *carried = have;
+  DH_LAUNCH_CHECK();
+  return DH_OK;
+}
+extern "C" int dh_dbg_gemm_xattn_dq(int dtype, const void* A, long lda, const void* W, int M, int N, int K, void* d_o, const void* q,
+                                    const void* k, const void* v, long ldk, const void* o, const float* lse, void* dq, int B, int Nk,
+                                    int* carried, void* stream) {
+  DH_REQUIRE(A && W && d_o && q && k && v && o && lse && dq && K % 64 == 0 && N % 64 == 0 && B > 0 && M % B == 0 && Nk > 0, "bad arguments");
+  static void* tiled = nullptr;
+  static size_t tiled_cap = 0;
+  const size_t need = (size_t)N * K * 2;
+  if (need > tiled_cap) {
+    if (tiled) (void)hipFree(tiled);
+    DH_CHECK_HIP(hipMalloc(&tiled, need));
+    tiled_cap = need;
+  }
+  launch_tile_weights(dtype, W, tiled, N, K, (hipStream_t)stream);
+  GemmArgs g;
+  g.A = A; g.lda = lda; g.W = tiled; g.M = M; g.N = N; g.K = K; g.mode = A_DENSE; g.C = d_o; g.ldc = N;
+  int have = 0;
+  g.xa_k = k; g.xa_v = v; g.xa_ldk = ldk; g.xa_o = const_cast<void*>(o); g.xa_ldo = N; g.xa_lse = const_cast<float*>(lse);
+  g.xa_H = N / 64; g.xa_Nq = M / B; g.xa_Nk = Nk; g.xa_q = q; g.xa_ldq = N; g.xa_dq = dq; g.xa_lddq = N; g.xa_done = &have;
+  launch_gemm(dtype, g, (hipStream_t)stream);
+  if (!have) launch_attention_bwd_dq(dtype, q, N, k, v, ldk, o, N, d_o, N, lse, nullptr, dq, N, B, N / 64, M / B, Nk, (hipStream_t)stream);
+  if (carried) *carried = have;
   DH_LAUNCH_CHECK();
   return DH_OK;
 }
diff --git a/diffusionhandles_amd/csrc/gemm.hip b/diffusionhandles_amd/csrc/gemm.hip
--- a/diffusionhandles_amd/csrc/gemm.hip
+++ b/diffusionhandles_amd/csrc/gemm.hip
@@ -4,6 +4,7 @@
 
 #include <hip/hip_ext.h>
 
+#include "attn_tile.h"
 #include "gemm_k.h"
 
 namespace dh {
@@ -23,6 +24,8 @@
   int bm, bn, kg, stages, mw, splits, pp, gn_epi, reduce_gn;
 };
 static thread_local GemmTileReport g_last_tile;
+static thread_local int g_last_xattn = 0;
+static thread_local long long g_xattn_total = 0;
 #ifdef DH_TUNING
 static unsigned long long* g_gemm_ts = nullptr;
 #endif
@@ -424,6 +427,47 @@
     }
   }
 
+  constexpr bool XA = GLU == EPI_XATTN || GLU == EPI_XATTN_DQ, XB = GLU == EPI_XATTN_DQ;
+  static_assert(!XB || !LNF, "the input-gradient GEMM carries no LayerNorm");
+  static_assert(!XA || xattn_epi_tile(BM, BN, WG, MW, BUF), "the cross-attention epilogue lives on the buffer-staged 64x64 / 128x64 tiles");
+  constexpr int XA_CH = XA_KEYS * 8 / 256;
+  u4v xa_kr[XA ? XA_CH : 1], xa_vr[XA ? XA_CH : 1];
+  if constexpr (XA) {
+    if (KG == 1 || kg == 0) {
+      const int b = div_small(m0, __builtin_amdgcn_rcpf((float)p.xa_Nq));
+      const size_t head = (size_t)b * p.xa_Nk * p.xa_ldk + n0;
+      const T* kp = reinterpret_cast<const T*>(p.xa_k) + head;
+      const T* vp = reinterpret_cast<const T*>(p.xa_v) + head;
+#pragma unroll
+      for (int j = 0; j < XA_CH; ++j) {
+        const int idx = tid + j * 256;
+        int r = idx >> 3;
+        r = r < p.xa_Nk ? r : p.xa_Nk - 1;
+        const size_t off = (size_t)r * p.xa_ldk + (idx & 7) * 8;
+        xa_kr[j] = *reinterpret_cast<const u4v*>(kp + off);
+        xa_vr[j] = *reinterpret_cast<const u4v*>(vp + off);
+      }
+    }
+  }
+  constexpr int XA_WPR = XA ? 4 / (BM / 32) : 1;
+  u4v xb_qf[XB ? 4 : 1], xb_of[XB ? 4 : 1];
+  float xb_lse = 0.f;
+  if constexpr (XB) {
+    if (KG == 1 || kg == 0) {
+      int m = m0 + (wave_s / XA_WPR) * 32 + ln;
+      m = m < p.M ? m : p.M - 1;
+      const T* qp = reinterpret_cast<const T*>(p.xa_q) + (size_t)m * p.xa_ldq + n0 + 8 * hi;
+      const T* op = reinterpret_cast<const T*>(p.xa_o) + (size_t)m * p.xa_ldo + n0 + 8 * hi;
+#pragma unroll
+      for (int kk = 0; kk < 4; ++kk) {
+        xb_qf[kk] = *reinterpret_cast<const u4v*>(qp + 16 * kk);
+        xb_of[kk] = *reinterpret_cast<const u4v*>(op + 16 * kk);
+      }
+      const int b = div_small(m0, __builtin_amdgcn_rcpf((float)p.xa_Nq));
+      xb_lse = p.xa_lse[((size_t)b * p.xa_H + blockIdx.y) * p.xa_Nq + (m - b * p.xa_Nq)] * LOG2E;
+    }
+  }
+
   constexpr int KK = BK / 16 / WG;
   const int kk0 = grp * KK;
   unsigned fa_off[BK / 16], fb_off[BK / 16];
@@ -564,6 +608,162 @@
     }
   }
 
+  if constexpr (XA) {
+    typedef T T4 __attribute__((ext_vector_type(4)));
+    static_assert((BM + 2 * XA_KEYS) * TLD * 2 <= KG * ST * STAGE, "q, K and V tiles fit the idle rings");
+    unsigned short* sq = reinterpret_cast<unsigned short*>(smem_all);
+    unsigned short* sk = sq + BM * TLD;
+    unsigned short* sv = sk + XA_KEYS * TLD;
+    const bool hb = p.bias != nullptr;
+    __syncthreads();
+#pragma unroll
+    for (int i = 0; i < TM; ++i) {
+      const int row = wm * RPW + i * 32 + ln, m = m0 + row;
+      uint2 w[4];
+#pragma unroll
+      for (int g = 0; g < 4; ++g) {
+        float v0 = acc[i][0][4 * g], v1 = acc[i][0][4 * g + 1], v2 = acc[i][0][4 * g + 2], v3 = acc[i][0][4 * g + 3];
+        if (hb) { const float4 b = bpre[0][g]; v0 += b.x; v1 += b.y; v2 += b.z; v3 += b.w; }
+        T4 o;
+        o[0] = from_f32<T>(v0); o[1] = from_f32<T>(v1); o[2] = from_f32<T>(v2); o[3] = from_f32<T>(v3);
+        w[g] = __builtin_bit_cast(uint2, o);
+      }
+      const uint4 ca = half_exchange(w[0], w[1]), cb = half_exchange(w[2], w[3]);
+      if (!XB && p.xa_save && m < p.M) {
+        T* orow = reinterpret_cast<T*>(p.C) + (size_t)m * p.ldc + n0 + wn * CPW + 8 * hi;
+        *reinterpret_cast<uint4*>(orow) = ca;
+        *reinterpret_cast<uint4*>(orow + 16) = cb;
+      }
+      *reinterpret_cast<uint4*>(&sq[row * TLD + wn * CPW + 8 * hi]) = ca;
+      *reinterpret_cast<uint4*>(&sq[row * TLD + wn * CPW + 8 * hi + 16]) = cb;
+    }
+#pragma unroll
+    for (int j = 0; j < XA_CH; ++j) {
+      const int idx = tid + j * 256;
+      *reinterpret_cast<u4v*>(&sk[(idx >> 3) * TLD + (idx & 7) * 8]) = xa_kr[j];
+      *reinterpret_cast<u4v*>(&sv[(idx >> 3) * TLD + (idx & 7) * 8]) = xa_vr[j];
+    }
+    __syncthreads();
+    constexpr int WPR = XA_WPR, NDT = 2 / WPR;
+    const int rb = wave_s / WPR, dt0 = (wave_s % WPR) * NDT;
+    uint4 qf[4];
+#pragma unroll
+    for (int kk = 0; kk < 4; ++kk) qf[kk] = *reinterpret_cast<const uint4*>(&sq[(rb * 32 + ln) * TLD + 16 * kk + 8 * hi]);
+    const int t16 = lane & 15;
+    const int tr_off = (4 * hi + (t16 >> 2)) * TLD + 16 * ((lane >> 4) & 1) + 4 * (t16 & 3);
+    if constexpr (XB) {
+      typedef T T8 __attribute__((ext_vector_type(8)));
+      uint4 sqf[4];
+      float del = 0.f;
+#pragma unroll
+      for (int kk = 0; kk < 4; ++kk) {
+        const T8 ov = __builtin_bit_cast(T8, xb_of[kk]), dv = __builtin_bit_cast(T8, qf[kk]);
+#pragma unroll
+        for (int c = 0; c < 8; ++c) del += to_f32<T>(ov[c]) * to_f32<T>(dv[c]);
+        sqf[kk] = __builtin_bit_cast(uint4, xb_qf[kk]);
+      }
+      del = xor32_sum(del);
+      const unsigned short* kt = sk + tr_off;
+      v16f dqa[NDT];
+#pragma unroll
+      for (int d = 0; d < NDT; ++d) dqa[d] = zero16();
+#pragma unroll
+      for (int kb = 0; kb < XA_KEYS / 32; ++kb) {
+        v16f sc = tile_times_frags<T>(sk, kb * 32, ln, hi, sqf);
+        const v16f dp = tile_times_frags<T>(sv, kb * 32, ln, hi, qf);
+#pragma unroll
+        for (int r = 0; r < 16; ++r) {
+          const float pr = kb * 32 + acc_row(r, hi) < p.xa_Nk ? fast_exp2(__builtin_fmaf(sc[r], CEXP, -xb_lse)) : 0.f;
+          sc[r] = pr * (dp[r] - del);
+        }
+#pragma unroll
+        for (int s2 = 0; s2 < 2; ++s2) {
+          const uint4 dsf = pack8<T>(sc, s2);
+#pragma unroll
+          for (int d = 0; d < NDT; ++d) dqa[d] = Mfma<T>::run(tr_frag(kt, (dt0 + d) * 32, kb * 32 + 16 * s2), dsf, dqa[d]);
+        }
+      }
+      const int m = m0 + rb * 32 + ln;
+      if (m < p.M) {
+        T* orow = reinterpret_cast<T*>(p.xa_dq) + (size_t)m * p.xa_lddq + n0 + 8 * hi;
+#pragma unroll
+        for (int d = 0; d < NDT; ++d) {
+          uint2 w[4];
+#pragma unroll
+          for (int g = 0; g < 4; ++g) {
+            T4 o;
+#pragma unroll
+            for (int c = 0; c < 4; ++c) o[c] = from_f32<T>(dqa[d][4 * g + c] * SCALE);
+            w[g] = __builtin_bit_cast(uint2, o);
+          }
+          const uint4 ca = half_exchange(w[0], w[1]), cb = half_exchange(w[2], w[3]);
+          *reinterpret_cast<uint4*>(orow + (dt0 + d) * 32) = ca;
+          *reinterpret_cast<uint4*>(orow + (dt0 + d) * 32 + 16) = cb;
+        }
+      }
+      return;
+    }
+    v16f sc[XA_KEYS / 32];
+#pragma unroll
+    for (int kb = 0; kb < XA_KEYS / 32; ++kb) {
+      sc[kb] = tile_times_frags<T>(sk, kb * 32, ln, hi, qf);
+#pragma unroll
+      for (int r = 0; r < 16; ++r)
+        if (kb * 32 + acc_row(r, hi) >= p.xa_Nk) sc[kb][r] = -INFINITY;
+    }
+    float mx = sc[0][0];
+#pragma unroll
+    for (int kb = 0; kb < XA_KEYS / 32; ++kb)
+#pragma unroll
+      for (int r = 0; r < 16; ++r) mx = fmaxf(mx, sc[kb][r]);
+    mx = xor32_max(mx);
+    const float mc = mx * CEXP;
+    float l = 0.f;
+#pragma unroll
+    for (int kb = 0; kb < XA_KEYS / 32; ++kb)
+#pragma unroll
+      for (int r = 0; r < 16; ++r) {
+        sc[kb][r] = fast_exp2(__builtin_fmaf(sc[kb][r], CEXP, -mc));
+        l += sc[kb][r];
+      }
+    l = xor32_sum(l);
+    const unsigned short* vt = sv + tr_off;
+    v16f oa[NDT];
+#pragma unroll
+    for (int d = 0; d < NDT; ++d) oa[d] = zero16();
+#pragma unroll
+    for (int kb = 0; kb < XA_KEYS / 32; ++kb)
+#pragma unroll
+      for (int s2 = 0; s2 < 2; ++s2) {
+        const uint4 pf = pack8<T>(sc[kb], s2);
+#pragma unroll
+        for (int d = 0; d < NDT; ++d) oa[d] = Mfma<T>::run(tr_frag(vt, (dt0 + d) * 32, kb * 32 + 16 * s2), pf, oa[d]);
+      }
+    const int m = m0 + rb * 32 + ln;
+    if (m < p.M) {
+      const float inv_l = 1.f / l;
+      T* orow = reinterpret_cast<T*>(p.xa_o) + (size_t)m * p.xa_ldo + n0 + 8 * hi;
+#pragma unroll
+      for (int d = 0; d < NDT; ++d) {
+        uint2 w[4];
+#pragma unroll
+        for (int g = 0; g < 4; ++g) {
+          T4 o;
+#pragma unroll
+          for (int c = 0; c < 4; ++c) o[c] = from_f32<T>(oa[d][4 * g + c] * inv_l);
+          w[g] = __builtin_bit_cast(uint2, o);
+        }
+        const uint4 ca = half_exchange(w[0], w[1]), cb = half_exchange(w[2], w[3]);
+        *reinterpret_cast<uint4*>(orow + (dt0 + d) * 32) = ca;
+        *reinterpret_cast<uint4*>(orow + (dt0 + d) * 32 + 16) = cb;
+      }
+      if (hi == 0 && dt0 == 0) {
+        const int b = div_small(m0, __builtin_amdgcn_rcpf((float)p.xa_Nq));
+        p.xa_lse[((size_t)b * p.xa_H + blockIdx.y) * p.xa_Nq + (m - b * p.xa_Nq)] = (mc + log2f(l)) * LN2;
+      }
+    }
+    return;
+  }
 
   if constexpr (GLU == 1) {
     typedef T T4 __attribute__((ext_vector_type(4)));
@@ -1111,6 +1311,11 @@
     if (glu == 1) { DH_GEMM_LAUNCH((k_gemm_dma<T, BM, BN, ST, GM_DENSE, 0, WG, KG, MW, false, 1, BUF>)); return; }
     if (glu == 2) { DH_GEMM_LAUNCH((k_gemm_dma<T, BM, BN, ST, GM_DENSE, 0, WG, KG, MW, false, 2, BUF>)); return; }
   }
+  if constexpr (xattn_epi_tile(BM, BN, WG, MW, BUF)) {
+    if (glu == EPI_XATTN && lnf) { DH_GEMM_LAUNCH((k_gemm_dma<T, BM, BN, ST, GM_DENSE, 0, WG, KG, MW, true, EPI_XATTN, BUF>)); return; }
+    if (glu == EPI_XATTN) { DH_GEMM_LAUNCH((k_gemm_dma<T, BM, BN, ST, GM_DENSE, 0, WG, KG, MW, false, EPI_XATTN, BUF>)); return; }
+    if (glu == EPI_XATTN_DQ) { DH_GEMM_LAUNCH((k_gemm_dma<T, BM, BN, ST, GM_DENSE, 0, WG, KG, MW, false, EPI_XATTN_DQ, BUF>)); return; }
+  }
   if (gm == GM_DENSE) {
     if constexpr (WG == 1 && BN != 320 && BN != 160) {
       if (lnf) { DH_GEMM_LAUNCH((k_gemm_dma<T, BM, BN, ST, GM_DENSE, 0, WG, KG, MW, true, 0, BUF>)); return; }
@@ -1137,7 +1342,7 @@
 #endif
 
 template <class T>
-static void gemm_dispatch(GemmK k, size_t partial_elems, hipStream_t st, int* gn_done, int* lnb_done, int dtype) {
+static void gemm_dispatch(GemmK k, size_t partial_elems, hipStream_t st, int* gn_done, int* lnb_done, int* xa_done, int dtype) {
   DH_KNOB(kSplitTiles, "DH_SPLITK_TILES", 200);
   DH_KNOB(kSplitMinK, "DH_SPLITK_MINKT", 32);
   DH_KNOB(kSplitTarget, "DH_SPLITK_TARGET", 256);
@@ -1233,26 +1438,6 @@
 #else
   dim3 grid(tm, tn, splits);
 #endif
-  hipEvent_t e0 = nullptr, e1 = nullptr;
-  if (g_prof.on) {
-    if (g_prof.used + 2 > g_prof.ev.size()) {
-      const size_t old = g_prof.ev.size();
-      g_prof.ev.resize(old + 4096);
-      for (size_t i = old; i < g_prof.ev.size(); ++i) (void)hipEventCreate(&g_prof.ev[i]);
-    }
-    e0 = g_prof.ev[g_prof.used++];
-    e1 = g_prof.ev[g_prof.used++];
-    g_prof.flops += 2.0 * (double)k.M * (double)k.N * (double)k.K;
-    const double esz = 2.0;
-    double a_elems = (double)k.M * k.K;
-    if (k.mode != A_DENSE && k.Hout > 0 && k.Wout > 0) a_elems = (double)k.M / ((double)k.Hout * k.Wout) * k.Hin * k.Win * k.Cin;
-    double c_elems = (double)k.M * k.N * (k.C ? 1.0 : 0.0) + (k.R ? (double)k.M * k.N : 0.0);
-    if (k.glu_y) c_elems += 0.5 * (double)k.M * k.N;
-    if (k.glub_x) c_elems += 4.0 * (double)k.M * k.glub_f - (k.C ? (double)k.M * k.glub_f : 0.0);
-    if (k.gn_epi == 2) c_elems += (double)k.M * k.N;
-    g_prof.bytes += esz * (a_elems + (double)k.N * k.K + c_elems);
-    g_prof.e0 = e0; g_prof.e1 = e1;
-  }
   int gm = GM_GENERIC;
   if (k.mode == A_DENSE) gm = GM_DENSE;
   else if (k.mode == A_CONV3 && k.stride == 1 && k.up == 0 && k.pad == 1) gm = GM_CONV_S1;
@@ -1268,6 +1453,41 @@
         ((size_t)k.A & 15) == 0 && ((size_t)k.W & 15) == 0) {
       k.pp_a_bytes = (unsigned)ab; k.pp_w_bytes = (unsigned)wb;
     }
+  }
+  k.xa = 0;
+  const bool xa_bwd = k.xa_dq != nullptr;
+  if (k.xa_o && xa_done && (g_buf_stage & (xa_bwd ? 32 : 16)) == 0 && splits == 1 && !use_pp && !glu && !t160 && !n320 && !mw2 &&
+      xattn_epi_tile(BM, BN, 1, 1, k.pp_a_bytes != 0) && gm == GM_DENSE && k.xa_Nk >= 1 && k.xa_Nk <= XA_KEYS && k.xa_Nq > 0 &&
+      k.N == 64 * k.xa_H && k.M % k.xa_Nq == 0 && k.M < (1 << 22) && (k.M == k.xa_Nq || k.xa_Nq % BM == 0) && k.C && k.wide_store && k.pre_r &&
+      !k.R && !k.rowvec && !k.act_silu && !k.gn_epi && k.xa_lse && k.xa_ldk % 8 == 0 && k.xa_ldo % 8 == 0 &&
+      (((size_t)k.xa_k | (size_t)k.xa_v | (size_t)k.xa_o) & 15) == 0 &&
+      (!xa_bwd || (!lnf && !k.bias && k.xa_q && k.xa_ldq % 8 == 0 && k.xa_lddq % 8 == 0 && (((size_t)k.xa_q | (size_t)k.xa_dq) & 15) == 0)))
+    k.xa = xa_bwd ? 2 : 1;
+#ifdef DH_TUNING
+  if (force_tile) k.xa = 0;
+#endif
+  const int epi = k.xa == 2 ? EPI_XATTN_DQ : (k.xa ? EPI_XATTN : glu);
+  hipEvent_t e0 = nullptr, e1 = nullptr;
+  if (g_prof.on) {
+    if (g_prof.used + 2 > g_prof.ev.size()) {
+      const size_t old = g_prof.ev.size();
+      g_prof.ev.resize(old + 4096);
+      for (size_t i = old; i < g_prof.ev.size(); ++i) (void)hipEventCreate(&g_prof.ev[i]);
+    }
+    e0 = g_prof.ev[g_prof.used++];
+    e1 = g_prof.ev[g_prof.used++];
+    g_prof.flops += 2.0 * (double)k.M * (double)k.N * (double)k.K;
+    const double esz = 2.0;
+    double a_elems = (double)k.M * k.K;
+    if (k.mode != A_DENSE && k.Hout > 0 && k.Wout > 0) a_elems = (double)k.M / ((double)k.Hout * k.Wout) * k.Hin * k.Win * k.Cin;
+    double c_elems = (double)k.M * k.N * (k.C ? 1.0 : 0.0) + (k.R ? (double)k.M * k.N : 0.0);
+    if (k.glu_y) c_elems += 0.5 * (double)k.M * k.N;
+    if (k.glub_x) c_elems += 4.0 * (double)k.M * k.glub_f - (k.C ? (double)k.M * k.glub_f : 0.0);
+    if (k.gn_epi == 2) c_elems += (double)k.M * k.N;
+    if (k.xa == 1) c_elems += (k.xa_save ? 1.0 : 0.0) * (double)k.M * k.N + 2.0 * (k.M / k.xa_Nq) * (double)k.xa_Nk * k.N;
+    if (k.xa == 2) c_elems += 2.0 * (double)k.M * k.N + 2.0 * (k.M / k.xa_Nq) * (double)k.xa_Nk * k.N;
+    g_prof.bytes += esz * (a_elems + (double)k.N * k.K + c_elems);
+    g_prof.e0 = e0; g_prof.e1 = e1;
   }
 #ifdef DH_TUNING
   static const int kAbl = getenv("DH_GEMM_ABLATE") ? atoi(getenv("DH_GEMM_ABLATE")) : 0;
@@ -1292,14 +1512,16 @@
   else if (mw2) launch_tile<T, 256, 128, 3, 1, 1, 2>(gm, lnf, grid, st, k, glu);
   else if (BM == 128 && BN == 128 && (glu || (kMw128 && tiles_per_split >= kMw128))) launch_tile<T, 128, 128, 4, 1, 1, 2>(gm, lnf, grid, st, k, glu);
   else if (kTwoPerCu && BM == 128 && BN == 64 && tiles * splits > 256 && tiles * splits <= 512)
-    launch_tile<T, 128, 64, 3, 1, 1, 1>(gm, lnf, grid, st, k);
-  else if (BM == 128 && BN == 64 && tiles_per_split >= kKg2MinKt) launch_tile<T, 128, 64, 3, 1, 2, 1>(gm, lnf, grid, st, k);
+    launch_tile<T, 128, 64, 3, 1, 1, 1>(gm, lnf, grid, st, k, epi);
+  else if (BM == 128 && BN == 64 && tiles_per_split >= kKg2MinKt) launch_tile<T, 128, 64, 3, 1, 2, 1>(gm, lnf, grid, st, k, epi);
   else if (BN == 320) launch_tile<T, 128, 320, 2, 1, 1, 2>(gm, false, grid, st, k);
-  else if (BM == 64) launch_tile<T, 64, 64, 4, 1, 1, 1>(gm, lnf, grid, st, k, glu);
+  else if (BM == 64) launch_tile<T, 64, 64, 4, 1, 1, 1>(gm, lnf, grid, st, k, epi);
   else if (BN == 128 && kManyBlocks > 0 && tiles * splits >= kManyBlocks) launch_tile<T, 128, 128, 2, 1, 1, 1>(gm, lnf, grid, st, k);
   else if (BN == 128) launch_tile<T, 128, 128, 4, 1, 1, 1>(gm, lnf, grid, st, k);
-  else launch_tile<T, 128, 64, 5, 1, 1, 1>(gm, lnf, grid, st, k);
+  else launch_tile<T, 128, 64, 5, 1, 1, 1>(gm, lnf, grid, st, k, epi);
   g_prof.e0 = g_prof.e1 = nullptr;
+  g_last_xattn = k.xa;
+  if (k.xa) { ++g_xattn_total; *xa_done = 1; }
   g_last_tile.splits = splits; g_last_tile.pp = use_pp ? 1 : 0; g_last_tile.gn_epi = k.gn_epi;
   if (k.gn_epi) *gn_done = k.gn_S;
   if (splits > 1) {
@@ -1347,10 +1569,14 @@
   } else if (a.glub_x) {
     k.C = nullptr;
   }
+  k.xa = 0; k.xa_k = a.xa_k; k.xa_v = a.xa_v; k.xa_ldk = a.xa_ldk; k.xa_o = a.xa_o; k.xa_ldo = a.xa_ldo; k.xa_lse = a.xa_lse;
+  k.xa_H = a.xa_H; k.xa_Nq = a.xa_Nq; k.xa_Nk = a.xa_Nk; k.xa_save = a.xa_save;
+  k.xa_q = a.xa_q; k.xa_ldq = a.xa_ldq; k.xa_dq = a.xa_dq; k.xa_lddq = a.xa_lddq;
   if (a.gn_done) *a.gn_done = 0;
   if (a.lnb_done) *a.lnb_done = 0;
-  if (dtype == DH_DTYPE_F16) gemm_dispatch<f16>(k, a.partial_elems, st, a.gn_done, a.lnb_done, dtype);
-  else gemm_dispatch<bf16>(k, a.partial_elems, st, a.gn_done, a.lnb_done, dtype);
+  if (a.xa_done) *a.xa_done = 0;
+  if (dtype == DH_DTYPE_F16) gemm_dispatch<f16>(k, a.partial_elems, st, a.gn_done, a.lnb_done, a.xa_done, dtype);
+  else gemm_dispatch<bf16>(k, a.partial_elems, st, a.gn_done, a.lnb_done, a.xa_done, dtype);
   return 2.0 * (double)a.M * (double)a.N * (double)a.K;
 }
 
@@ -1376,6 +1602,12 @@
   const dh::GemmTileReport& r = dh::g_last_tile;
   const int v[9] = {r.bm, r.bn, r.kg, r.stages, r.mw, r.splits, r.pp, r.gn_epi, r.reduce_gn};
   for (int i = 0; i < 9; ++i) out[i] = v[i];
+  return DH_OK;
+}
+
+extern "C" int dh_dbg_gemm_xattn_carried(int* last, long long* total) {
+  if (last) *last = dh::g_last_xattn;
+  if (total) *total = dh::g_xattn_total;
   return DH_OK;
 }
 
diff --git a/diffusionhandles_amd/csrc/gemm_k.h b/diffusionhandles_amd/csrc/gemm_k.h
--- a/diffusionhandles_amd/csrc/gemm_k.h
+++ b/diffusionhandles_amd/csrc/gemm_k.h
@@ -47,12 +47,21 @@
   int glub_f;
   int pp_tm, pp_tn, pp_order, pp_nwork; unsigned pp_a_bytes, pp_w_bytes;
   unsigned long long* pp_ts;
+  int xa, xa_Nq, xa_Nk, xa_H, xa_save;
+  const void *xa_k, *xa_v; long xa_ldk; void* xa_o; long xa_ldo; float* xa_lse;
+  const void* xa_q; long xa_ldq; void* xa_dq; long xa_lddq;
 };
 
 
 __host__ __device__ constexpr bool glub_tile_is_glu(int n0, int glub_f) { return n0 < glub_f; }
 __host__ __device__ constexpr bool glub_split_ok(int BN, int glub_f) { return BN > 0 && glub_f % BN == 0; }
 
+constexpr int EPI_XATTN = 3, EPI_XATTN_DQ = 4;
+constexpr int XA_KEYS = 96;
+__host__ __device__ constexpr bool xattn_epi_tile(int BM, int BN, int WG, int MW, bool BUF) {
+  return BN == 64 && (BM == 64 || BM == 128) && WG == 1 && MW == 1 && BUF;
+}
+
 struct PpPlan { int bm = 0, bn = 0, splits = 1; };
 bool gemm_pp_plan(const GemmK& k, size_t partial_elems, int force, PpPlan* plan);
 void launch_gemm_pp(int dtype, const GemmK& k, const PpPlan& plan, hipStream_t st, hipEvent_t e0, hipEvent_t e1);
diff --git a/diffusionhandles_amd/csrc/unet_engine.cpp b/diffusionhandles_amd/csrc/unet_engine.cpp
--- a/diffusionhandles_amd/csrc/unet_engine.cpp
+++ b/diffusionhandles_amd/csrc/unet_engine.cpp
@@ -56,6 +56,8 @@
   int ln_fold = -1, folded = 0;
   long ln_s_off = -1, ln_t_off = -1;
   int glu_op = -1, glub_op = -1;
+  int xattn_op = -1;
+  int xattn_bwd_op = -1;
 };
 
 struct FfFold {
@@ -294,8 +296,11 @@
     c.out = tensor(N, C);
     c.lse_off = f32_slot((size_t)maxB * heads * N);
     u.ops.push_back(c);
+    u.ops[u.ops.size() - 2].xattn_op = (int)u.ops.size() - 1;
     const int tg = tensor(N, 5 * C, false);
+    const int xop = (int)u.ops.size() - 1;
     int t2 = linear(c.out, b + ".attn2.to_out.0", C, true, t1);
+    u.ops.back().xattn_bwd_op = xop;
     set_view(t2, tg, 4 * C);
     int n3 = ln(t2, b + ".norm3");
     int gg = linear(n3, b + ".ff.net.0.proj", 8 * C, true, -1);
@@ -475,6 +480,7 @@
     rd(o.in0, oi); rd(o.in1, oi); rd(o.res, oi); wr(o.out, oi);
     if (o.ln_fold >= 0) rd(u.ops[o.ln_fold].in0, oi);
     if (o.glu_op >= 0) wr(u.ops[o.glu_op].out, oi);
+    if (o.xattn_op >= 0) wr(u.ops[o.xattn_op].out, oi);
   }
   std::vector<char> written(nt, 0);
   for (const Op& o : u.ops) { if (o.out >= 0) written[root(o.out)] = 1; if (o.glu_op >= 0) written[root(u.ops[o.glu_op].out)] = 1; }
@@ -871,6 +877,7 @@
   const dh_unet_config& c = u->cfg;
   u->flops_fwd = 0;
   int gn_have = 0;
+  int xa_have = 0;
   if (!kv_hit) launch_f32_to_t(dt, u->in_text, u->aptr(u->t_text), (size_t)B * c.text_len * c.cross_attention_dim, st);
   for (int oi = first_op; oi < n_ops; ++oi) {
     const Op& o = u->ops[oi];
@@ -909,6 +916,15 @@
           g.glu_y = u->aptr(ge.out); g.glu_ldy = u->tens[ge.out].ld;
           if (!save) g.C = nullptr;
         }
+        xa_have = 0;
+        if (o.xattn_op >= 0 && o.xattn_op < n_ops) {
+          const Op& at = u->ops[o.xattn_op];
+          const unsigned short* kv = u->aptr(at.in1) + at.kv_col;
+          const int C = u->tens[at.out].C;
+          g.xa_k = kv; g.xa_v = kv + C; g.xa_ldk = u->tens[at.in1].C; g.xa_o = u->aptr(at.out); g.xa_ldo = C;
+          g.xa_lse = u->f32a + at.lse_off; g.xa_H = at.heads; g.xa_Nq = at.Nq; g.xa_Nk = at.Nk; g.xa_save = save ? 1 : 0;
+          g.xa_done = &xa_have;
+        }
         u->flops_fwd += launch_gemm(dt, g, st);
         break;
       }
@@ -935,7 +951,7 @@
           const unsigned short* qkv = u->aptr(o.in0);
           launch_attention_fwd(dt, qkv, tq.C, qkv + C, qkv + 2 * C, tq.C, u->aptr(o.out), C, u->f32a + o.lse_off, B,
                                o.heads, o.Nq, o.Nk, st);
-        } else {
+        } else if (!(oi > 0 && u->ops[oi - 1].xattn_op == oi && xa_have)) {
           const Ten& tkv = u->tens[o.in1];
           const unsigned short* kv = u->aptr(o.in1) + o.kv_col;
           launch_attention_fwd(dt, u->aptr(o.in0), tq.C, kv, kv + C, tkv.C, u->aptr(o.out), C, u->f32a + o.lse_off, B,
@@ -1078,6 +1094,7 @@
   int lnb_have = 0, lnb_for = -1;
   int cat_done = -1;
   int glub_done = -1;
+  int xb_have = 0, xb_for = -1;
   for (int oi = (int)u->ops.size() - 1; oi >= 0; --oi) {
     const Op& o = u->ops[oi];
     if (!want_sample && oi < u->first_cross_op && o.out != u->t_kv) continue;
@@ -1154,6 +1171,17 @@
             gnb_have = 0;
             gnb_for = oi - 1;
           }
+          xb_have = 0;
+          if (o.xattn_bwd_op >= 0 && !bw.need_text && !u->gready[o.in0] && o.in0 == u->ops[o.xattn_bwd_op].out) {
+            const Op& at = u->ops[o.xattn_bwd_op];
+            const unsigned short* kv = u->aptr(at.in1) + at.kv_col;
+            const int C = u->tens[at.out].C, ldq = u->tens[at.in0].C;
+            g.xa_k = kv; g.xa_v = kv + C; g.xa_ldk = u->tens[at.in1].C; g.xa_o = u->aptr(at.out); g.xa_ldo = C;
+            g.xa_lse = u->f32a + at.lse_off; g.xa_H = at.heads; g.xa_Nq = at.Nq; g.xa_Nk = at.Nk;
+            g.xa_q = u->aptr(at.in0); g.xa_ldq = ldq; g.xa_dq = u->gptr(at.in0); g.xa_lddq = ldq;
+            g.xa_done = &xb_have;
+            xb_for = o.xattn_bwd_op;
+          }
           u->flops_bwd += launch_gemm(dt, g, st);
           u->gready[o.in0] = 1;
         } else if (o.up) {
@@ -1247,6 +1275,9 @@
           launch_attention_bwd_dkv(dt, qkv, tq.C, qkv + C, qkv + 2 * C, tq.C, u->gptr(o.out), C, u->f32a + o.lse_off,
                                    delta, dqkv + C, dqkv + 2 * C, tq.C, B, o.heads, o.Nq, o.Nk, st);
           u->flops_bwd += 14.0 * B * o.heads * (double)o.Nq * o.Nk * 64;
+        } else if (xb_have && xb_for == oi) {
+          xb_have = 0;
+          u->flops_bwd += 6.0 * B * o.heads * (double)o.Nq * o.Nk * 64;
         } else {
           const Ten& tkv = u->tens[o.in1];
           const unsigned short* kv = u->aptr(o.in1) + o.kv_col;
diff --git a/diffusionhandles_amd/csrc/unet_kernels.h b/diffusionhandles_amd/csrc/unet_kernels.h
--- a/diffusionhandles_amd/csrc/unet_kernels.h
+++ b/diffusionhandles_amd/csrc/unet_kernels.h
@@ -47,6 +47,9 @@
   void* lnb_dx = nullptr; int* lnb_done = nullptr;
   void* glu_y = nullptr; long glu_ldy = 0;
   const void* glub_x = nullptr; void* glub_dx = nullptr; int glub_f = 0;
+  const void *xa_k = nullptr, *xa_v = nullptr; long xa_ldk = 0; void* xa_o = nullptr; long xa_ldo = 0; float* xa_lse = nullptr;
+  int xa_H = 0, xa_Nq = 0, xa_Nk = 0, xa_save = 1; int* xa_done = nullptr;
+  const void* xa_q = nullptr; long xa_ldq = 0; void* xa_dq = nullptr; long xa_lddq = 0;
 };
 void launch_splitk_reduce_ln_bwd(int dtype, const float* partial, int splits, const void* x, const float* gamma,
                                  const float* stats, const void* add, void* dx, int rows, int C, hipStream_t st, long ldx = 0);
```

Result: faster. 38.48 steps/s, median of 6 (+2.1%).
